# pyg-team/pytorch_geometric

Hardware: NVIDIA H100
Metric: edges/sec (GCNConv fwd+bwd) (higher is better)
Workload: dtype f32

## Files before the change

include/b200mp.h:

```cpp
#ifndef B200MP_H_
#define B200MP_H_

#include <stdint.h>

#ifdef __cplusplus
extern "C" {
#endif

#define B200MP_VERSION "0.1.0"

enum { B200MP_F32 = 0, B200MP_BF16 = 1 };
enum { B200MP_I32 = 0, B200MP_I64 = 1 };
enum { B200MP_SUM = 0, B200MP_MEAN = 1, B200MP_MIN = 2, B200MP_MAX = 3, B200MP_MUL = 4 };
enum {
    B200MP_OK = 0,
    B200MP_ERR_INVALID_ARG = -1,
    B200MP_ERR_UNSUPPORTED = -2,
    B200MP_ERR_CUDA = -3,
    B200MP_ERR_WORKSPACE = -4
};

const char* b200mp_version(void);
const char* b200mp_last_error(void);
int b200mp_device_info(int* sm_count, int* cc_major, int* cc_minor, int64_t* l2_bytes);
int b200mp_set_option(const char* name, int value);


int b200mp_degree(const void* index, int64_t n_index, int64_t n_nodes, void* deg, int idx_dtype,
                  void* stream);
int b200mp_index2ptr(const void* index_sorted, int64_t n_index, int64_t n_nodes, void* ptr,
                     int idx_dtype, void* stream);
int b200mp_ptr2index(const void* ptr, int64_t n_nodes, int64_t n_index, void* index,
                     int idx_dtype, void* stream);
int b200mp_index_stats(const void* index, int64_t n_index, int64_t* stats, int idx_dtype,
                       void* stream);
int64_t b200mp_sort_workspace_bytes(int64_t n_index, int64_t n_nodes, int idx_dtype);
int b200mp_sort_by_key(const void* keys, int64_t n_index, int64_t n_nodes, void* keys_sorted,
                       void* perm, void* ptr, void* workspace, int64_t workspace_bytes,
                       int idx_dtype, void* stream);
int b200mp_permute(const void* in, const void* perm, void* out, int64_t n, int elem_bytes,
                   int idx_dtype, void* stream);
int b200mp_convert_index(const void* in, int in_dtype, void* out, int out_dtype, int64_t n,
                         void* stream);
int64_t b200mp_self_loops_workspace_bytes(int64_t n_edges, int64_t n_nodes, int idx_dtype);
int b200mp_self_loops(const void* row, const void* col, const float* w_in, int64_t n_edges,
                      int64_t n_nodes, float fill_value, int mode, void* row_out, void* col_out,
                      float* w_out, int64_t* n_out_dev, void* workspace, int64_t workspace_bytes,
                      int idx_dtype, void* stream);
int b200mp_gcn_norm_csr(const void* rowptr, const void* src, const float* w, int64_t n_nodes,
                        int64_t n_edges, float* deg_inv_sqrt, float* w_out, int idx_dtype,
                        void* stream);

int b200mp_csr_plan_count(const void* rowptr, int64_t n_rows, int64_t chunk, int64_t* counts_dev,
                          int idx_dtype, void* stream);
int64_t b200mp_csr_plan_workspace_bytes(int64_t n_rows, int64_t n_long_rows, int idx_dtype);
int b200mp_csr_plan_fill(const void* rowptr, int64_t n_rows, int64_t chunk, int64_t n_long_rows,
                         int64_t* long_rows, int64_t* chunk_ptr, void* workspace,
                         int64_t workspace_bytes, int idx_dtype, void* stream);

int b200mp_spmm_csr(const void* rowptr, const void* col, const float* val, const void* x,
                    void* out, int64_t n_rows, int64_t n_cols, int64_t feat, int reduce,
                    const int64_t* long_rows, const int64_t* chunk_ptr, int64_t n_long_rows,
                    int64_t n_chunks, int64_t chunk, float* partials, const float* bias,
                    const void* x_halo, int64_t n_local_cols, int flags, const void* peer_ptrs,
                    int64_t peer_rows, const void* relu_mask, int idx_dtype, int val_dtype, void* stream);

int b200mp_segment_csr(const void* ptr, const void* src, void* out, int64_t n_rows, int64_t n_src,
                       int64_t feat, int reduce, const int64_t* long_rows, const int64_t* chunk_ptr,
                       int64_t n_long_rows, int64_t n_chunks, int64_t chunk, float* partials,
                       int idx_dtype, int val_dtype, void* stream);

int b200mp_minmax_ties(const void* rowptr, const void* col, const float* val, const void* x,
                       const void* out, float* ties, int64_t n_rows, int64_t feat,
                       int count_self_zero, int idx_dtype, int val_dtype, void* stream);
int b200mp_minmax_backward(const void* rowptr_t, const void* col_t, const float* val_t,
                           const void* x, const void* out, const void* grad_out, const float* ties,
                           void* grad_x, int64_t n_src, int64_t feat, int idx_dtype,
                           int val_dtype, void* stream);

int b200mp_sddmm_csr(const void* rowptr, const void* col, const void* a, const void* b, float* dot,
                     int64_t n_rows, int64_t feat, int idx_dtype, int val_dtype, void* stream);

int b200mp_edge_relu_csr(const void* rowptr, const void* col, const void* perm, const void* x,
                         const void* edge_rows, void* out, void* mask, int64_t n_rows, int64_t n_cols,
                         int64_t n_edges, int64_t feat, int reduce, const int64_t* long_rows,
                         const int64_t* chunk_ptr, int64_t n_long_rows, int64_t n_chunks, int64_t chunk,
                         float* partials, int idx_dtype, int val_dtype, void* stream);
int b200mp_edge_relu_backward_x(const void* rowptr_t, const void* col_t, const void* t2csr,
                                const float* val_t, const void* grad_out, const void* mask, void* grad_x,
                                int64_t n_src, int64_t feat, const int64_t* long_rows,
                                const int64_t* chunk_ptr, int64_t n_long_rows, int64_t n_chunks,
                                int64_t chunk, float* partials, int idx_dtype, int val_dtype, void* stream);
int b200mp_edge_relu_backward_edge(const void* rowptr, const void* perm, const void* grad_out,
                                   const void* mask, void* grad_edge_rows, int64_t n_rows, int64_t feat,
                                   int reduce, const int64_t* long_rows, const int64_t* chunk_ptr,
                                   int64_t n_long_rows, int64_t n_chunks, int64_t chunk, int idx_dtype,
                                   int val_dtype, void* stream);

int b200mp_gated_csr(const void* rowptr, const void* col, const void* k, const void* q, const void* v,
                     void* out, int64_t n_rows, int64_t n_cols, int64_t n_edges, int64_t feat, int64_t ld,
                     int reduce, const int64_t* long_rows, const int64_t* chunk_ptr, int64_t n_long_rows,
                     int64_t n_chunks, int64_t chunk, float* partials, int idx_dtype, int val_dtype,
                     void* stream);
int b200mp_gated_backward_dst(const void* rowptr, const void* col, const void* k, const void* q,
                              const void* v, const void* grad_out, void* grad_k, int64_t n_rows,
                              int64_t n_cols, int64_t n_edges, int64_t feat, int64_t ld, int reduce,
                              const int64_t* long_rows, const int64_t* chunk_ptr, int64_t n_long_rows,
                              int64_t n_chunks, int64_t chunk, float* partials, int idx_dtype,
                              int val_dtype, void* stream);
int b200mp_gated_backward_src(const void* rowptr_t, const void* col_t, const float* val_t, const void* k,
                              const void* q, const void* v, const void* grad_out, void* grad_q,
                              void* grad_v, int64_t n_src, int64_t n_dst, int64_t n_edges, int64_t feat,
                              int64_t ld, const int64_t* long_rows, const int64_t* chunk_ptr,
                              int64_t n_long_rows, int64_t n_chunks, int64_t chunk, float* partials,
                              int idx_dtype, int val_dtype, void* stream);

int b200mp_cg_csr(const void* rowptr, const void* col, const void* perm, const void* u, const void* v,
                  const void* c, void* out, int64_t n_rows, int64_t n_cols, int64_t n_edges, int64_t feat,
                  int64_t ld_u, int64_t ld_v, int reduce, const int64_t* long_rows,
                  const int64_t* chunk_ptr, int64_t n_long_rows, int64_t n_chunks, int64_t chunk,
                  float* partials, int idx_dtype, int val_dtype, void* stream);
int b200mp_cg_backward_dst(const void* rowptr, const void* col, const void* perm, const void* u,
                           const void* v, const void* c, const void* grad_out, void* grad_u, void* grad_c,
                           int64_t n_rows, int64_t n_cols, int64_t n_edges, int64_t feat, int64_t ld_u,
                           int64_t ld_v, int reduce, const int64_t* long_rows, const int64_t* chunk_ptr,
                           int64_t n_long_rows, int64_t n_chunks, int64_t chunk, float* partials,
                           int idx_dtype, int val_dtype, void* stream);
int b200mp_cg_backward_src(const void* rowptr_t, const void* col_t, const void* perm_t, const float* val_t,
                           const void* u, const void* v, const void* c, const void* grad_out, void* grad_v,
                           int64_t n_src, int64_t n_dst, int64_t n_edges, int64_t feat, int64_t ld_u,
                           int64_t ld_v, const int64_t* long_rows, const int64_t* chunk_ptr,
                           int64_t n_long_rows, int64_t n_chunks, int64_t chunk, float* partials,
                           int idx_dtype, int val_dtype, void* stream);

int b200mp_softmax_aggr_csr(const void* rowptr, const void* col, const void* perm, const void* x,
                            const void* edge_rows, const float* t, void* out, float* lse, int64_t n_rows,
                            int64_t n_cols, int64_t n_edges, int64_t feat, int message, float eps, int t_mode,
                            const int64_t* long_rows, const int64_t* chunk_ptr, int64_t n_long_rows,
                            int64_t n_chunks, int64_t chunk, float* partials, int idx_dtype, int val_dtype,
                            void* stream);
int64_t b200mp_softmax_aggr_workspace(int64_t n_rows, int64_t n_chunks, int64_t feat);
int b200mp_softmax_aggr_backward_dst(const void* rowptr, const void* col, const void* perm, const void* x,
                                     const void* edge_rows, const float* t, const void* out, const float* lse,
                                     const void* grad_out, void* grad_edge_rows, float* grad_t, float* workspace,
                                     int64_t n_rows, int64_t n_cols, int64_t n_edges, int64_t feat, int message,
                                     float eps, int t_mode, int semi_grad, const int64_t* long_rows,
                                     const int64_t* chunk_ptr, int64_t n_long_rows, int64_t n_chunks, int64_t chunk,
                                     int idx_dtype, int val_dtype, void* stream);
int b200mp_softmax_aggr_backward_src(const void* rowptr_t, const void* col_t, const void* perm_t, const void* x,
                                     const void* edge_rows, const float* t, const void* out, const float* lse,
                                     const void* grad_out, void* grad_x, int64_t n_src, int64_t n_dst,
                                     int64_t n_edges, int64_t feat, int message, float eps, int t_mode,
                                     int semi_grad, const int64_t* long_rows, const int64_t* chunk_ptr,
                                     int64_t n_long_rows, int64_t n_chunks, int64_t chunk, float* partials,
                                     int idx_dtype, int val_dtype, void* stream);

int b200mp_scatter_coo(const float* src, const void* index, float* out, float* count,
                       int64_t n_src, int64_t n_rows, int64_t feat, int reduce, int idx_dtype,
                       void* stream);
int b200mp_index_add_rows(const float* src, const void* index, float* out, int64_t n_src,
                          int64_t feat, int idx_dtype, void* stream);
int b200mp_gather_rows(const void* x, const void* index, const float* scale, void* out,
                       int64_t n_out, int64_t feat, int idx_dtype, int val_dtype, void* stream);

int b200mp_softmax_csr(const void* ptr, const float* src, float* out, int64_t n_rows,
                       int64_t n_src, int64_t heads, int idx_dtype, void* stream);
int b200mp_softmax_csr_backward(const void* ptr, const float* out, const float* grad_out,
                                float* grad_src, int64_t n_rows, int64_t n_src, int64_t heads,
                                int idx_dtype, void* stream);
int b200mp_softmax_edge_op(int op, const float* a, const float* b, const float* row, const void* dst_of_edge,
                           float* out, int64_t n_src, int64_t heads, int idx_dtype, void* stream);


int64_t b200mp_column_sum_parts(int64_t n_rows);
int b200mp_column_sum(const void* x, float* out, float* partials, int64_t n_parts, int64_t n_rows, int64_t feat,
                      int val_dtype, void* stream);

int b200mp_multi_aggr_mask_supported(int64_t feat, int val_dtype, int segment_mode);
int b200mp_multi_aggr_csr(const void* rowptr, const void* col, const void* x, void* out_sum, void* out_mean,
                          void* out_min, void* out_max, void* out_var, void* out_std, float* ties_min,
                          float* ties_max, void* hit_mask, int64_t n_rows, int64_t n_src, int64_t feat, int count_self_zero,
                          const int64_t* long_rows, const int64_t* chunk_ptr, int64_t n_long_rows,
                          int64_t n_chunks, int64_t chunk, float* partials, int idx_dtype, int val_dtype,
                          void* stream);
int b200mp_multi_aggr_prepare_backward(const void* rowptr, const void* g_sum, const void* g_mean,
                                       const void* g_var, const void* g_std, const void* g_min,
                                       const void* g_max, const void* mean, const void* std,
                                       const float* ties_min, const float* ties_max, float* term_a,
                                       float* term_b, float* gmin_out, float* gmax_out, int64_t n_rows,
                                       int64_t feat, int semi_grad, int idx_dtype, int val_dtype, void* stream);
int b200mp_multi_aggr_backward(const void* ptr, const void* idx, const void* x, const float* term_a,
                               const float* term_b, const void* out_min, const float* g_min,
                               const void* out_max, const float* g_max, const void* hit_mask, const void* t2csr,
                               void* grad_x, int64_t n_items, int64_t feat, int segment_mode, int idx_dtype,
                               int val_dtype, void* stream);

int b200mp_pna_epilogue(const void* rowptr, const void* x, const void* u, int64_t u_ld, const void* stat_sum,
                        const void* stat_min, const void* stat_max, const void* stat_var, const int32_t* aggr_host,
                        int n_aggr, const int32_t* scaler_host, int n_scaler, const float* avg_deg_lin,
                        const float* avg_deg_log, void* out, int64_t n_rows, int64_t towers, int64_t feat,
                        int stats_dtype, int idx_dtype, int val_dtype, void* stream);
int b200mp_pna_prologue(const void* rowptr, const void* grad_out, const void* u, int64_t u_ld, const void* stat_sum,
                        const void* stat_min, const void* stat_max, const void* stat_var, const float* ties_min,
                        const float* ties_max, const int32_t* aggr_host, int n_aggr, const int32_t* scaler_host,
                        int n_scaler, const float* avg_deg_lin, const float* avg_deg_log, float* term_a, float* term_b,
                        float* gmin, float* gmax, void* grad_u, int64_t gu_ld, void* grad_x, float* avg_part,
                        int64_t n_rows, int64_t towers, int64_t feat, int stats_dtype, int idx_dtype, int val_dtype,
                        void* stream);
int b200mp_pna_edge_stats(const void* rowptr, const void* col, const void* perm, const void* v, int64_t v_ld,
                          const void* c, float* stat_sum, float* stat_min, float* stat_max, float* stat_var,
                          float* ties_min, float* ties_max, int64_t n_rows, int64_t n_cols, int64_t n_edges,
                          int64_t width, const int64_t* long_rows, const int64_t* chunk_ptr, int64_t n_long_rows,
                          int64_t n_chunks, int64_t chunk, float* partials, int idx_dtype, int val_dtype, void* stream);
int b200mp_pna_edge_backward(const void* rowptr_t, const void* col_t, const void* perm_t, const void* v, int64_t v_ld,
                             const void* c, const float* term_a, const float* term_b, const float* stat_min,
                             const float* gmin, const float* stat_max, const float* gmax, void* grad_v, int64_t gv_ld,
                             void* grad_c, int64_t n_src, int64_t n_dst, int64_t n_edges, int64_t width, int idx_dtype,
                             int val_dtype, void* stream);

int b200mp_head_dot_supported(int64_t heads, int64_t chan, int val_dtype);
int64_t b200mp_head_dot_parts(int64_t n_rows, int64_t heads, int64_t chan, int val_dtype);
int b200mp_head_dot(const void* x, const float* att_a, const float* att_b, float* s_a, float* s_b, int64_t n_rows,
                    int64_t heads, int64_t chan, int val_dtype, void* stream);
int b200mp_head_dot_backward(const void* x, const float* att_a, const float* att_b, const float* g_a, const float* g_b,
                             const void* add, void* grad_x, float* part_a, float* part_b, int64_t n_parts,
                             int64_t n_rows, int64_t heads, int64_t chan, int val_dtype, void* stream);

int b200mp_gat_fused_csr(const void* rowptr, const void* col, const void* dst_of_edge, const void* xh,
                         const float* a_src, const float* a_dst, void* out, float* row_max,
                         float* row_den, float* alpha_out, int64_t n_rows, int64_t n_edges,
                         int64_t heads, int64_t chan, float slope, const int64_t* long_rows,
                         const int64_t* chunk_ptr, int64_t n_long_rows, int64_t n_chunks, int64_t chunk,
                         float* part_acc, float* part_ms, int idx_dtype, int val_dtype, void* stream);
int b200mp_gat_fused_csr_backward(const void* rowptr, const void* col, const void* dst_of_edge,
                                  const void* rowptr_t, const void* col_t, const void* t2csr,
                                  const void* xh, const float* a_src, const float* a_dst,
                                  const float* row_max, const float* row_den, const void* out,
                                  const void* grad_out, float* grad_pre, float* rowdot, void* grad_xh,
                                  float* grad_a_src, float* grad_a_dst, int64_t n_rows, int64_t n_src,
                                  int64_t n_edges, int64_t heads, int64_t chan, float slope,
                                  const int64_t* long_rows, const int64_t* chunk_ptr,
                                  int64_t n_long_rows, int64_t n_chunks, int64_t chunk, float* partials,
                                  int idx_dtype, int val_dtype, void* stream);

int b200mp_scatter_arg(const float* src, const void* index, const float* out, int64_t* arg, int64_t n_src,
                       int64_t n_rows, int64_t feat, int idx_dtype, void* stream);
int b200mp_spmm_csr_arg(const void* rowptr, const void* col, const float* val, const float* x, const float* out,
                        int64_t* arg, int64_t n_rows, int64_t feat, int64_t nnz, int idx_dtype, void* stream);

int b200mp_attn_supported(int64_t heads, int64_t chan, int val_dtype);
int b200mp_attn_csr_forward(int mode, const void* rowptr, const void* col, const void* v, const void* k,
                            const void* q, const float* s_src, const float* s_dst, const float* att,
                            const float* s_edge, int64_t v_stride, int64_t k_stride, int64_t q_stride,
                            void* out, float* row_max, float* row_den, float* alpha_out, int64_t n_rows,
                            int64_t n_edges, int64_t heads, int64_t chan, float slope, float scale,
                            const int64_t* long_rows, const int64_t* chunk_ptr, int64_t n_long_rows,
                            int64_t n_chunks, int64_t chunk, float* part_acc, float* part_ms, float dropout_p,
                            unsigned long long dropout_seed, const void* edge_feat, int idx_dtype, int val_dtype,
                            void* stream);
int64_t b200mp_attn_backward_partial_width(int mode, int64_t heads, int64_t chan, int transposed);
int64_t b200mp_attn_gatt_rows(void);
int b200mp_attn_csr_backward(int mode, const void* rowptr, const void* col, const void* rowptr_t,
                             const void* col_t, const void* t2csr, const void* v, const void* k, const void* q,
                             const float* s_src, const float* s_dst, const float* att, const float* s_edge,
                             int64_t v_stride, int64_t k_stride, int64_t q_stride, const float* row_max,
                             const float* row_den, const void* out, const void* grad_out, float* pair,
                             void* grad_v, void* grad_k, void* grad_q, float* grad_s_src, float* grad_s_dst,
                             float* grad_att, float* gatt_part, int64_t n_rows, int64_t n_src, int64_t n_edges,
                             int64_t heads, int64_t chan, float slope, float scale, const int64_t* long_rows,
                             const int64_t* chunk_ptr, int64_t n_long_rows, int64_t n_chunks, int64_t chunk,
                             float* partials, const int64_t* long_rows_t, const int64_t* chunk_ptr_t,
                             int64_t n_long_rows_t, int64_t n_chunks_t, float* partials_t, float dropout_p,
                             unsigned long long dropout_seed, const void* edge_feat, void* grad_edge_feat, int idx_dtype,
                             int val_dtype, void* stream);

int b200mp_split_tf32(const float* w, float* w_hi, float* w_lo, int64_t n, void* stream);
int b200mp_split_tf32_transposed(const float* w, float* wt_hi, float* wt_lo, int64_t rows, int64_t cols, void* stream);
int b200mp_linear_tf32x3(const float* x, const float* w_hi, const float* w_lo, float* y, int64_t m,
                         int64_t n, int64_t k, void* stream);
int b200mp_linear_grad_input_tf32x3(const float* g, const float* w_hi, const float* w_lo, float* gx,
                                    int64_t m, int64_t n, int64_t k, void* stream);
int64_t b200mp_linear_grad_weight_workspace_bytes(int64_t m, int64_t n, int64_t k);
int b200mp_linear_grad_weight_tf32x3(const float* g, const float* x, float* gw, int64_t m, int64_t n,
                                     int64_t k, void* workspace, int64_t workspace_bytes,
                                     void* stream);

int b200mp_gemm_pair_tf32x3(const float* a1, int64_t k1, const float* a2, int64_t k2, const float* b_hi,
                            const float* b_lo, int b_layout, const float* bias, int relu, float* c1, int64_t n1,
                            float* c2, int64_t n2, int64_t m, void* stream);

int b200mp_segment_matmul_tf32x3(const float* a, const int64_t* ptr, int64_t n_seg, const float* b_hi,
                                 const float* b_lo, int b_layout, float* c, int64_t m, int64_t k, int64_t n,
                                 void* stream);

#ifdef __cplusplus
}
#endif
#endif
```

pytorch_geometric_b200/_lib.py:

```python
from __future__ import annotations

import ctypes
import os
import re

from . import _build

_I64 = ctypes.c_int64
_INT = ctypes.c_int
_P = ctypes.c_void_p
_F = ctypes.c_float
_U64 = ctypes.c_uint64

_SIGS = {
    "b200mp_version": (ctypes.c_char_p, []),
    "b200mp_last_error": (ctypes.c_char_p, []),
    "b200mp_device_info": (_INT, [_P, _P, _P, _P]),
    "b200mp_set_option": (_INT, [ctypes.c_char_p, _INT]),
    "b200mp_degree": (_INT, [_P, _I64, _I64, _P, _INT, _P]),
    "b200mp_index2ptr": (_INT, [_P, _I64, _I64, _P, _INT, _P]),
    "b200mp_ptr2index": (_INT, [_P, _I64, _I64, _P, _INT, _P]),
    "b200mp_index_stats": (_INT, [_P, _I64, _P, _INT, _P]),
    "b200mp_sort_workspace_bytes": (_I64, [_I64, _I64, _INT]),
    "b200mp_sort_by_key": (_INT, [_P, _I64, _I64, _P, _P, _P, _P, _I64, _INT, _P]),
    "b200mp_permute": (_INT, [_P, _P, _P, _I64, _INT, _INT, _P]),
    "b200mp_convert_index": (_INT, [_P, _INT, _P, _INT, _I64, _P]),
    "b200mp_self_loops_workspace_bytes": (_I64, [_I64, _I64, _INT]),
    "b200mp_self_loops": (_INT, [_P, _P, _P, _I64, _I64, _F, _INT, _P, _P, _P, _P, _P, _I64, _INT, _P]),
    "b200mp_gcn_norm_csr": (_INT, [_P, _P, _P, _I64, _I64, _P, _P, _INT, _P]),
    "b200mp_csr_plan_count": (_INT, [_P, _I64, _I64, _P, _INT, _P]),
    "b200mp_csr_plan_workspace_bytes": (_I64, [_I64, _I64, _INT]),
    "b200mp_csr_plan_fill": (_INT, [_P, _I64, _I64, _I64, _P, _P, _P, _I64, _INT, _P]),
    "b200mp_spmm_csr": (_INT, [_P, _P, _P, _P, _P, _I64, _I64, _I64, _INT, _P, _P, _I64, _I64, _I64, _P,
                               _P, _P, _I64, _INT, _P, _I64, _P, _INT, _INT, _P]),
    "b200mp_segment_csr": (_INT, [_P, _P, _P, _I64, _I64, _I64, _INT, _P, _P, _I64, _I64, _I64, _P, _INT, _INT, _P]),
    "b200mp_minmax_ties": (_INT, [_P, _P, _P, _P, _P, _P, _I64, _I64, _INT, _INT, _INT, _P]),
    "b200mp_minmax_backward": (_INT, [_P, _P, _P, _P, _P, _P, _P, _P, _I64, _I64, _INT, _INT, _P]),
    "b200mp_sddmm_csr": (_INT, [_P, _P, _P, _P, _P, _I64, _I64, _INT, _INT, _P]),
    "b200mp_edge_relu_csr": (_INT, [_P] * 7 + [_I64] * 4 + [_INT, _P, _P, _I64, _I64, _I64, _P, _INT, _INT, _P]),
    "b200mp_edge_relu_backward_x": (_INT, [_P] * 7 + [_I64, _I64, _P, _P, _I64, _I64, _I64, _P, _INT, _INT, _P]),
    "b200mp_edge_relu_backward_edge": (_INT, [_P] * 5 + [_I64, _I64, _INT, _P, _P, _I64, _I64, _I64, _INT, _INT, _P]),
    "b200mp_gated_csr": (_INT, [_P] * 6 + [_I64] * 5 + [_INT, _P, _P, _I64, _I64, _I64, _P, _INT, _INT, _P]),
    "b200mp_gated_backward_dst": (_INT, [_P] * 7 + [_I64] * 5 + [_INT, _P, _P, _I64, _I64, _I64, _P, _INT, _INT, _P]),
    "b200mp_gated_backward_src": (_INT, [_P] * 9 + [_I64] * 5 + [_P, _P, _I64, _I64, _I64, _P, _INT, _INT, _P]),
    "b200mp_cg_csr": (_INT, [_P] * 7 + [_I64] * 6 + [_INT, _P, _P, _I64, _I64, _I64, _P, _INT, _INT, _P]),
    "b200mp_cg_backward_dst": (_INT, [_P] * 9 + [_I64] * 6 + [_INT, _P, _P, _I64, _I64, _I64, _P, _INT, _INT, _P]),
    "b200mp_cg_backward_src": (_INT, [_P] * 9 + [_I64] * 6 + [_P, _P, _I64, _I64, _I64, _P, _INT, _INT, _P]),
    "b200mp_softmax_aggr_csr": (_INT, [_P] * 8 + [_I64] * 4 + [_INT, _F, _INT, _P, _P, _I64, _I64, _I64, _P, _INT, _INT,
                                                                _P]),
    "b200mp_softmax_aggr_workspace": (_I64, [_I64, _I64, _I64]),
    "b200mp_softmax_aggr_backward_dst": (_INT, [_P] * 12 + [_I64] * 4 + [_INT, _F, _INT, _INT, _P, _P, _I64, _I64, _I64,
                                                                           _INT, _INT, _P]),
    "b200mp_softmax_aggr_backward_src": (_INT, [_P] * 10 + [_I64] * 4 + [_INT, _F, _INT, _INT, _P, _P, _I64, _I64, _I64,
                                                                           _P, _INT, _INT, _P]),
    "b200mp_scatter_coo": (_INT, [_P, _P, _P, _P, _I64, _I64, _I64, _INT, _INT, _P]),
    "b200mp_split_tf32": (_INT, [_P, _P, _P, _I64, _P]),
    "b200mp_split_tf32_transposed": (_INT, [_P, _P, _P, _I64, _I64, _P]),
    "b200mp_linear_tf32x3": (_INT, [_P, _P, _P, _P, _I64, _I64, _I64, _P]),
    "b200mp_linear_grad_input_tf32x3": (_INT, [_P, _P, _P, _P, _I64, _I64, _I64, _P]),
    "b200mp_linear_grad_weight_workspace_bytes": (_I64, [_I64, _I64, _I64]),
    "b200mp_linear_grad_weight_tf32x3": (_INT, [_P, _P, _P, _I64, _I64, _I64, _P, _I64, _P]),
    "b200mp_gemm_pair_tf32x3": (_INT, [_P, _I64, _P, _I64, _P, _P, _INT, _P, _INT, _P, _I64, _P, _I64, _I64, _P]),
    "b200mp_segment_matmul_tf32x3": (_INT, [_P, _P, _I64, _P, _P, _INT, _P, _I64, _I64, _I64, _P]),
    "b200mp_index_add_rows": (_INT, [_P, _P, _P, _I64, _I64, _INT, _P]),
    "b200mp_gather_rows": (_INT, [_P, _P, _P, _P, _I64, _I64, _INT, _INT, _P]),
    "b200mp_softmax_csr": (_INT, [_P, _P, _P, _I64, _I64, _I64, _INT, _P]),
    "b200mp_softmax_csr_backward": (_INT, [_P, _P, _P, _P, _I64, _I64, _I64, _INT, _P]),
    "b200mp_gat_fused_csr": (_INT, [_P] * 10 + [_I64, _I64, _I64, _I64, _F, _P, _P, _I64, _I64, _I64, _P, _P, _INT, _INT, _P]),
    "b200mp_gat_fused_csr_backward": (_INT, [_P] * 18 + [_I64, _I64, _I64, _I64, _I64, _F, _P, _P, _I64, _I64, _I64, _P,
                                              _INT, _INT, _P]),
    "b200mp_scatter_arg": (_INT, [_P, _P, _P, _P, _I64, _I64, _I64, _INT, _P]),
    "b200mp_spmm_csr_arg": (_INT, [_P, _P, _P, _P, _P, _P, _I64, _I64, _I64, _INT, _P]),
    "b200mp_attn_supported": (_INT, [_I64, _I64, _INT]),
    "b200mp_attn_csr_forward": (_INT, [_INT] + [_P] * 9 + [_I64] * 3 + [_P] * 4 + [_I64] * 4 + [_F, _F, _P, _P, _I64, _I64, _I64,
                                       _P, _P, _F, _U64, _P, _INT, _INT, _P]),
    "b200mp_attn_backward_partial_width": (_I64, [_INT, _I64, _I64, _INT]),
    "b200mp_attn_gatt_rows": (_I64, []),
    "b200mp_attn_csr_backward": (_INT, [_INT] + [_P] * 12 + [_I64] * 3 + [_P] * 12 + [_I64] * 5 + [_F, _F, _P, _P, _I64, _I64,
                                        _I64, _P, _P, _P, _I64, _I64, _P, _F, _U64, _P, _P, _INT, _INT, _P]),
    "b200mp_column_sum_parts": (_I64, [_I64]),
    "b200mp_column_sum": (_INT, [_P, _P, _P, _I64, _I64, _I64, _INT, _P]),
    "b200mp_softmax_edge_op": (_INT, [_INT, _P, _P, _P, _P, _P, _I64, _I64, _INT, _P]),
    "b200mp_multi_aggr_csr": (_INT, [_P] * 12 + [_I64, _I64, _I64, _INT, _P, _P, _I64, _I64, _I64, _P, _INT, _INT, _P]),
    "b200mp_multi_aggr_mask_supported": (_INT, [_I64, _INT, _INT]),
    "b200mp_head_dot_supported": (_INT, [_I64, _I64, _INT]),
    "b200mp_head_dot_parts": (_I64, [_I64, _I64, _I64, _INT]),
    "b200mp_head_dot": (_INT, [_P] * 5 + [_I64, _I64, _I64, _INT, _P]),
    "b200mp_head_dot_backward": (_INT, [_P] * 9 + [_I64, _I64, _I64, _I64, _INT, _P]),
    "b200mp_multi_aggr_prepare_backward": (_INT, [_P] * 15 + [_I64, _I64, _INT, _INT, _INT, _P]),
    "b200mp_multi_aggr_backward": (_INT, [_P] * 12 + [_I64, _I64, _INT, _INT, _INT, _P]),
    "b200mp_pna_epilogue": (_INT, [_P, _P, _P, _I64] + [_P] * 4 + [_P, _INT, _P, _INT, _P, _P, _P, _I64, _I64, _I64,
                                                                   _INT, _INT, _INT, _P]),
    "b200mp_pna_prologue": (_INT, [_P, _P, _P, _I64] + [_P] * 6 + [_P, _INT, _P, _INT] + [_P] * 7 + [_I64, _P, _P,
                                                                                               _I64, _I64, _I64,
                                                                                               _INT, _INT, _INT, _P]),
    "b200mp_pna_edge_stats": (_INT, [_P, _P, _P, _P, _I64] + [_P] * 7 + [_I64] * 4 + [_P, _P, _I64, _I64, _I64, _P, _INT,
                                                                                    _INT, _P]),
    "b200mp_pna_edge_backward": (_INT, [_P, _P, _P, _P, _I64] + [_P] * 8 + [_I64, _P] + [_I64] * 4 + [_INT, _INT, _P]),
}

_lib = None


def header_symbols() -> list[str]:
    with open(os.path.join(_build.INCLUDE, "b200mp.h")) as f:
        text = f.read()
    text = re.sub(r"/\*.*?\*/", "", text, flags=re.S)
    return sorted(set(re.findall(r"\b(b200mp_[a-z0-9_]+)\s*\(", text)))


def lib() -> ctypes.CDLL:
    global _lib
    if _lib is None:
        path = _build.LIB
        if _build.needs_build():
            try:
                path = _build.build()
            except Exception as exc:
                state = "is missing" if not os.path.exists(_build.LIB) else "is stale (sources changed since it was built)"
                raise RuntimeError(
                    f"pytorch_geometric_b200: libb200mp.so {state} and could not be rebuilt ({exc}); "
                    "there is no CPU / eager fallback.") from exc
        l = ctypes.CDLL(path)
        for name, (res, args) in _SIGS.items():
            fn = getattr(l, name)
            fn.restype = res
            fn.argtypes = args
        _lib = l
    return _lib


class B200MPError(RuntimeError):
    pass


def check(rc: int, what: str = "") -> None:
    if rc != 0:
        msg = lib().b200mp_last_error().decode()
        raise B200MPError(f"{what or 'b200mp'} failed (code {rc}): {msg}")
```

pytorch_geometric_b200/csrc/common.cuh:

```cuda
#pragma once

#include <cuda_bf16.h>
#include <cuda_runtime.h>
#include <stdint.h>

#include <cstdio>
#include <type_traits>

#include "../../include/b200mp.h"

namespace b200mp {

void set_error(const char* fmt, ...);

#define B200MP_CHECK_ARG(cond)                                                          \
    do {                                                                                \
        if (!(cond)) {                                                                  \
            ::b200mp::set_error("%s:%d: invalid argument: %s", __FILE__, __LINE__, #cond); \
            return B200MP_ERR_INVALID_ARG;                                              \
        }                                                                               \
    } while (0)

#define B200MP_CUDA(call)                                                                       \
    do {                                                                                        \
        cudaError_t e__ = (call);                                                               \
        if (e__ != cudaSuccess) {                                                               \
            ::b200mp::set_error("%s:%d: %s: %s", __FILE__, __LINE__, #call, cudaGetErrorString(e__)); \
            (void)cudaGetLastError();  \
            return B200MP_ERR_CUDA;                                                             \
        }                                                                                       \
    } while (0)

#define B200MP_LAUNCH_CHECK() B200MP_CUDA(cudaGetLastError())

constexpr int kSMs = 132;

inline int num_sms() {
    static int n = 0;
    if (n == 0) {
        int dev = 0;
        if (cudaGetDevice(&dev) != cudaSuccess ||
            cudaDeviceGetAttribute(&n, cudaDevAttrMultiProcessorCount, dev) != cudaSuccess || n <= 0)
            n = kSMs;
    }
    return n;
}

inline int64_t ceil_div(int64_t a, int64_t b) { return (a + b - 1) / b; }

template <typename F>
int dispatch_val_idx(int val_dtype, int idx_dtype, const char* what, F&& fn) {
    if (val_dtype == B200MP_F32 && idx_dtype == B200MP_I32) return fn(float{}, int32_t{});
    if (val_dtype == B200MP_F32 && idx_dtype == B200MP_I64) return fn(float{}, int64_t{});
    if (val_dtype == B200MP_BF16 && idx_dtype == B200MP_I32) return fn(__nv_bfloat16{}, int32_t{});
    if (val_dtype == B200MP_BF16 && idx_dtype == B200MP_I64) return fn(__nv_bfloat16{}, int64_t{});
    set_error("%s: unsupported dtype combination val=%d idx=%d", what, val_dtype, idx_dtype);
    return B200MP_ERR_UNSUPPORTED;
}

template <int MAX_VPL, typename F>
void lane_group_shape(int n_vec, F&& launch) {
    static_assert(MAX_VPL == 1 || MAX_VPL == 2 || MAX_VPL == 4, "VPL is 1, 2 or 4");
    using std::integral_constant;
    if (n_vec <= 1) launch(integral_constant<int, 1>{}, integral_constant<int, 1>{});
    else if (n_vec <= 2) launch(integral_constant<int, 2>{}, integral_constant<int, 1>{});
    else if (n_vec <= 4) launch(integral_constant<int, 4>{}, integral_constant<int, 1>{});
    else if (n_vec <= 8) launch(integral_constant<int, 8>{}, integral_constant<int, 1>{});
    else if (n_vec <= 16) launch(integral_constant<int, 16>{}, integral_constant<int, 1>{});
    else if constexpr (MAX_VPL == 1) launch(integral_constant<int, 32>{}, integral_constant<int, 1>{});
    else if (n_vec <= 32) launch(integral_constant<int, 32>{}, integral_constant<int, 1>{});
    else if constexpr (MAX_VPL == 2) launch(integral_constant<int, 32>{}, integral_constant<int, 2>{});
    else if (n_vec <= 64) launch(integral_constant<int, 32>{}, integral_constant<int, 2>{});
    else launch(integral_constant<int, 32>{}, integral_constant<int, 4>{});
}

template <int VPL>
constexpr int unroll_for_vpl() { return VPL >= 4 ? 1 : 4 / VPL; }

struct __align__(16) Vec16 {
    uint32_t w[4];
};

__device__ __forceinline__ Vec16 ldg_row16(const void* p) {
    Vec16 v;
    asm volatile("ld.global.nc.L1::no_allocate.v4.u32 {%0,%1,%2,%3}, [%4];"
                 : "=r"(v.w[0]), "=r"(v.w[1]), "=r"(v.w[2]), "=r"(v.w[3])
                 : "l"(p));
    return v;
}
__device__ __forceinline__ Vec16 ldg_stream16(const void* p) {
    Vec16 v;
    asm volatile("ld.global.cs.v4.u32 {%0,%1,%2,%3}, [%4];"
                 : "=r"(v.w[0]), "=r"(v.w[1]), "=r"(v.w[2]), "=r"(v.w[3])
                 : "l"(p));
    return v;
}
__device__ __forceinline__ void cp_async16(void* smem, const void* gmem) {
    asm volatile("cp.async.cg.shared.global [%0], [%1], 16;" ::"r"(static_cast<uint32_t>(__cvta_generic_to_shared(smem))), "l"(gmem) : "memory");
}
__device__ __forceinline__ void cp_async8(void* smem, const void* gmem) {
    asm volatile("cp.async.ca.shared.global [%0], [%1], 8;" ::"r"(static_cast<uint32_t>(__cvta_generic_to_shared(smem))), "l"(gmem) : "memory");
}
__device__ __forceinline__ void cp_async4(void* smem, const void* gmem) {
    asm volatile("cp.async.ca.shared.global [%0], [%1], 4;" ::"r"(static_cast<uint32_t>(__cvta_generic_to_shared(smem))), "l"(gmem) : "memory");
}
__device__ __forceinline__ void cp_async_commit() { asm volatile("cp.async.commit_group;" ::: "memory"); }
template <int N>
__device__ __forceinline__ void cp_async_wait() { asm volatile("cp.async.wait_group %0;" ::"n"(N) : "memory"); }
__device__ __forceinline__ void stg_stream16(void* p, const Vec16& v) {
    asm volatile("st.global.cs.v4.u32 [%0], {%1,%2,%3,%4};" ::"l"(p), "r"(v.w[0]), "r"(v.w[1]),
                 "r"(v.w[2]), "r"(v.w[3])
                 : "memory");
}

template <typename T>
struct ElemTraits;
template <>
struct ElemTraits<float> {
    static constexpr int kPerVec = 4;
    __device__ static __forceinline__ void unpack(const Vec16& v, float (&f)[4]) {
#pragma unroll
        for (int i = 0; i < 4; ++i) f[i] = __uint_as_float(v.w[i]);
    }
    __device__ static __forceinline__ Vec16 pack(const float (&f)[4]) {
        Vec16 v;
#pragma unroll
        for (int i = 0; i < 4; ++i) v.w[i] = __float_as_uint(f[i]);
        return v;
    }
    __device__ static __forceinline__ float to_float(float x) { return x; }
    __device__ static __forceinline__ float from_float(float x) { return x; }
};
template <>
struct ElemTraits<__nv_bfloat16> {
    static constexpr int kPerVec = 8;
    __device__ static __forceinline__ void unpack(const Vec16& v, float (&f)[8]) {
#pragma unroll
        for (int i = 0; i < 4; ++i) {
            f[2 * i] = __uint_as_float(v.w[i] << 16);
            f[2 * i + 1] = __uint_as_float(v.w[i] & 0xffff0000u);
        }
    }
    __device__ static __forceinline__ Vec16 pack(const float (&f)[8]) {
        Vec16 v;
#pragma unroll
        for (int i = 0; i < 4; ++i) {
            __nv_bfloat162 p = __floats2bfloat162_rn(f[2 * i], f[2 * i + 1]);
            v.w[i] = *reinterpret_cast<uint32_t*>(&p);
        }
        return v;
    }
    __device__ static __forceinline__ float to_float(__nv_bfloat16 x) { return __bfloat162float(x); }
    __device__ static __forceinline__ __nv_bfloat16 from_float(float x) { return __float2bfloat16_rn(x); }
};

template <typename T>
__device__ __forceinline__ float round_to(float v) {
    return ElemTraits<T>::to_float(ElemTraits<T>::from_float(v));
}

template <int EPV>
__device__ __forceinline__ void store_partial(float* p, const float (&acc)[EPV]) {
#pragma unroll
    for (int q = 0; q < EPV / 4; ++q)
        *reinterpret_cast<float4*>(p + 4 * q) = make_float4(acc[4 * q], acc[4 * q + 1], acc[4 * q + 2], acc[4 * q + 3]);
}

template <int RED>
__device__ __forceinline__ float red_identity() {
    if (RED == B200MP_MIN) return __int_as_float(0x7f800000);
    if (RED == B200MP_MAX) return __int_as_float(0xff800000);
    if (RED == B200MP_MUL) return 1.0f;
    return 0.0f;
}
template <int RED>
__device__ __forceinline__ float red_combine(float acc, float v) {
    if (RED == B200MP_MIN) return (v < acc || v != v) ? v : acc;
    if (RED == B200MP_MAX) return (v > acc || v != v) ? v : acc;
    if (RED == B200MP_MUL) return __fmul_rn(acc, v);
    return __fadd_rn(acc, v);
}

template <typename I>
__device__ __forceinline__ I ldg_idx(const I* p) {
    return __ldg(p);
}

inline bool aligned16(const void* p) { return (reinterpret_cast<uintptr_t>(p) & 15u) == 0; }

}
```

pytorch_geometric_b200/csrc/csr_dispatch.cuh:

```cuda
#pragma once

#include "csr_reduce.cuh"
#include "csr_tma.cuh"

namespace b200mp {

int get_option_spmm_impl();

template <typename T, typename I, int RED, bool GATHER>
int csr_reduce_variant(const I* rowptr, const I* col, const float* val, const T* x, T* out, int64_t n_rows,
                       int64_t feat, bool is_mean, bool inf_to_zero, LongRowPlan plan, const float* bias,
                       cudaStream_t stream) {
    if (n_rows == 0 || feat == 0) return B200MP_OK;
    const size_t row_bytes = static_cast<size_t>(feat) * sizeof(T);
    const bool tma_ok = row_bytes % 16 == 0 && row_bytes >= 512 && row_bytes <= 2048 && aligned16(x) &&
                        aligned16(plan.x2) && aligned16(out) && (plan.n_chunks == 0 || aligned16(plan.partials));
    const int impl = get_option_spmm_impl();
    if (tma_ok && impl == 2 && !plan.accumulate && !plan.peers)
        return csr_tma_launch<T, I, RED, GATHER>(rowptr, col, val, x, out, n_rows, feat, is_mean, inf_to_zero, plan,
                                                 bias, stream);
    return csr_reduce_dispatch<T, I, RED, GATHER>(rowptr, col, val, x, out, n_rows, feat, is_mean, inf_to_zero, plan,
                                                  bias, stream);
}

template <typename T, typename I, bool GATHER>
int csr_reduce_auto(const I* rowptr, const I* col, const float* val, const T* x, T* out, int64_t n_rows,
                    int64_t feat, int reduce, bool inf_to_zero, LongRowPlan plan, const float* bias,
                    cudaStream_t stream) {
    switch (reduce) {
        case B200MP_SUM:
            return csr_reduce_variant<T, I, B200MP_SUM, GATHER>(rowptr, col, val, x, out, n_rows, feat, false, false, plan, bias, stream);
        case B200MP_MEAN:
            return csr_reduce_variant<T, I, B200MP_SUM, GATHER>(rowptr, col, val, x, out, n_rows, feat, true, false, plan, bias, stream);
        case B200MP_MIN:
            return csr_reduce_variant<T, I, B200MP_MIN, GATHER>(rowptr, col, val, x, out, n_rows, feat, false, inf_to_zero, plan, bias, stream);
        case B200MP_MAX:
            return csr_reduce_variant<T, I, B200MP_MAX, GATHER>(rowptr, col, val, x, out, n_rows, feat, false, inf_to_zero, plan, bias, stream);
        default:
            set_error("csr_reduce: unsupported reduce %d", reduce);
            return B200MP_ERR_UNSUPPORTED;
    }
}

}
```

pytorch_geometric_b200/csrc/csr_reduce.cuh:

```cuda
#pragma once

#include "common.cuh"

namespace b200mp {

int get_option_spmm_tune();

struct LongRowPlan {
    const int64_t* long_rows;
    const int64_t* chunk_ptr;
    int64_t n_long;
    int64_t n_chunks;
    int64_t chunk;
    float* partials;
    const void* x2;
    int64_t split;
    int accumulate;
    const unsigned long long* peers;
    int64_t peer_rows;
    const void* relu_mask;
};

inline int make_plan(LongRowPlan& plan, const int64_t* long_rows, const int64_t* chunk_ptr, int64_t n_long_rows,
                     int64_t n_chunks, int64_t chunk, float* partials, bool needs_partials) {
    B200MP_CHECK_ARG(n_long_rows >= 0 && n_chunks >= 0);
    B200MP_CHECK_ARG(n_long_rows == 0 || (long_rows && chunk_ptr && chunk > 0 && (partials || !needs_partials)));
    plan = LongRowPlan{long_rows, chunk_ptr, n_long_rows, n_long_rows ? n_chunks : 0, chunk, partials,
                       nullptr, 0, 0, nullptr, 0, nullptr};
    return B200MP_OK;
}

__device__ __forceinline__ const char* row_base(const LongRowPlan& plan, const char* xb, const char* xb2, int64_t split,
                                                size_t row_bytes, int64_t c) {
    if (plan.peers) {
        const int64_t r = c / plan.peer_rows;
        return reinterpret_cast<const char*>(__ldg(plan.peers + r)) + static_cast<size_t>(c - r * plan.peer_rows) * row_bytes;
    }
    return (c < split ? xb : xb2) + static_cast<size_t>(c) * row_bytes;
}

template <typename I>
__device__ __forceinline__ bool decode_item(int64_t item, const I* __restrict__ rowptr, int64_t n_rows,
                                            const LongRowPlan& plan, int64_t& row, int64_t& begin,
                                            int64_t& end, bool& is_chunk) {
    if (item < plan.n_chunks) {
        int64_t lo = 0, hi = plan.n_long;
        while (hi - lo > 1) {
            const int64_t mid = (lo + hi) >> 1;
            if (__ldg(plan.chunk_ptr + mid) <= item) lo = mid; else hi = mid;
        }
        row = __ldg(plan.long_rows + lo);
        const int64_t k = item - __ldg(plan.chunk_ptr + lo);
        begin = static_cast<int64_t>(__ldg(rowptr + row)) + k * plan.chunk;
        const int64_t row_end = static_cast<int64_t>(__ldg(rowptr + row + 1));
        end = begin + plan.chunk < row_end ? begin + plan.chunk : row_end;
        is_chunk = true;
        return true;
    }
    row = item - plan.n_chunks;
    if (row >= n_rows) return false;
    begin = static_cast<int64_t>(__ldg(rowptr + row));
    end = static_cast<int64_t>(__ldg(rowptr + row + 1));
    is_chunk = false;
    if (plan.n_long > 0 && end - begin > plan.chunk) return false;
    return true;
}

template <int RED>
__device__ __forceinline__ float finalize(float acc, int64_t deg, bool is_mean, bool inf_to_zero) {
    if (RED == B200MP_SUM) {
        if (is_mean) acc = __fdiv_rn(acc, static_cast<float>(deg < 1 ? 1 : deg));
    } else if (RED == B200MP_MIN || RED == B200MP_MAX) {
        if (deg == 0) acc = 0.0f;
        if (inf_to_zero && isinf(acc)) acc = 0.0f;
    }
    return acc;
}

template <typename T, typename I, int G, int VPL, int RED, bool GATHER, int UNR_OVR = 0, int BLOCK = 256,
          int MINB = 1>
__global__ void __launch_bounds__(BLOCK, MINB)
csr_reduce_kernel(const I* __restrict__ rowptr, const I* __restrict__ col,
                  const float* __restrict__ val, const T* __restrict__ x, T* __restrict__ out,
                  int64_t n_rows, int n_vec, bool is_mean, bool inf_to_zero, LongRowPlan plan,
                  const float* __restrict__ bias) {
    constexpr int EPV = ElemTraits<T>::kPerVec;
    constexpr int UNR = UNR_OVR ? UNR_OVR : (VPL == 1 ? 8 : (VPL == 2 ? 4 : 2));
    const int lig = threadIdx.x & (G - 1);
    const int64_t item = (static_cast<int64_t>(blockIdx.x) * blockDim.x + threadIdx.x) / G;
    int64_t row, begin, end;
    bool is_chunk;
    const bool active = decode_item(item, rowptr, n_rows, plan, row, begin, end, is_chunk);
    if (G < 32 && !active) return;
    if (G == 32 && !active) return;
    const size_t row_bytes = static_cast<size_t>(n_vec) * 16;
    const char* xb = reinterpret_cast<const char*>(x);
    const char* xb2 = plan.x2 ? reinterpret_cast<const char*>(plan.x2) - static_cast<size_t>(plan.split) * row_bytes : xb;
    const int64_t split = plan.x2 ? plan.split : INT64_MAX;

    for (int vbase = 0; vbase < n_vec; vbase += G * VPL) {
        float acc[VPL][EPV];
#pragma unroll
        for (int k = 0; k < VPL; ++k)
#pragma unroll
            for (int i = 0; i < EPV; ++i) acc[k][i] = red_identity<RED>();
        bool vvalid[VPL];
#pragma unroll
        for (int k = 0; k < VPL; ++k) vvalid[k] = (vbase + lig + k * G) < n_vec;
        const size_t voff = static_cast<size_t>(vbase + lig) * 16;

        if (G == 32) {
            for (int64_t e0 = begin; e0 < end; e0 += 32) {
                const int n = static_cast<int>(end - e0 < 32 ? end - e0 : 32);
                int64_t c_l = 0;
                float w_l = 1.0f;
                if (lig < n) {
                    c_l = GATHER ? static_cast<int64_t>(ldg_idx(col + e0 + lig)) : (e0 + lig);
                    if (val) w_l = __ldg(val + e0 + lig);
                    c_l = static_cast<int64_t>(reinterpret_cast<uintptr_t>(row_base(plan, xb, xb2, split, row_bytes, c_l)));
                }
                for (int j = 0; j < n; j += UNR) {
                    Vec16 buf[UNR][VPL];
                    float w[UNR];
#pragma unroll
                    for (int u = 0; u < UNR; ++u) {
                        const int64_t c = __shfl_sync(0xffffffffu, c_l, (j + u) & 31);
                        w[u] = __shfl_sync(0xffffffffu, w_l, (j + u) & 31);
                        if (j + u < n) {
                            const char* p = reinterpret_cast<const char*>(static_cast<uintptr_t>(c)) + voff;
#pragma unroll
                            for (int k = 0; k < VPL; ++k)
                                if (vvalid[k]) buf[u][k] = ldg_row16(p + static_cast<size_t>(k) * G * 16);
                        }
                    }
#pragma unroll
                    for (int u = 0; u < UNR; ++u) {
                        if (j + u < n) {
#pragma unroll
                            for (int k = 0; k < VPL; ++k) {
                                if (vvalid[k]) {
                                    float f[EPV];
                                    ElemTraits<T>::unpack(buf[u][k], f);
#pragma unroll
                                    for (int i = 0; i < EPV; ++i) {
                                        const float m = val ? __fmul_rn(w[u], f[i]) : f[i];
                                        acc[k][i] = red_combine<RED>(acc[k][i], m);
                                    }
                                }
                            }
                        }
                    }
                }
            }
        } else {
            for (int64_t e = begin; e < end; e += UNR) {
                Vec16 buf[UNR][VPL];
                float w[UNR];
#pragma unroll
                for (int u = 0; u < UNR; ++u) {
                    w[u] = 1.0f;
                    if (e + u < end) {
                        const int64_t c = GATHER ? static_cast<int64_t>(ldg_idx(col + e + u)) : (e + u);
                        if (val) w[u] = __ldg(val + e + u);
                        if (vvalid[0]) buf[u][0] = ldg_row16(row_base(plan, xb, xb2, split, row_bytes, c) + voff);
                    }
                }
#pragma unroll
                for (int u = 0; u < UNR; ++u) {
                    if (e + u < end && vvalid[0]) {
                        float f[EPV];
                        ElemTraits<T>::unpack(buf[u][0], f);
#pragma unroll
                        for (int i = 0; i < EPV; ++i) {
                            const float m = val ? __fmul_rn(w[u], f[i]) : f[i];
                            acc[0][i] = red_combine<RED>(acc[0][i], m);
                        }
                    }
                }
            }
        }

        if (is_chunk) {
            float* pbase = plan.partials + static_cast<size_t>(item) * n_vec * EPV;
#pragma unroll
            for (int k = 0; k < VPL; ++k)
                if (vvalid[k]) store_partial<EPV>(pbase + static_cast<size_t>(vbase + lig + k * G) * EPV, acc[k]);
        } else {
            const int64_t deg = end - begin;
            char* ob = reinterpret_cast<char*>(out) + static_cast<size_t>(row) * row_bytes;
#pragma unroll
            for (int k = 0; k < VPL; ++k) {
                if (!vvalid[k]) continue;
                float f[EPV];
#pragma unroll
                for (int i = 0; i < EPV; ++i) f[i] = finalize<RED>(acc[k][i], deg, is_mean, inf_to_zero);
                if (bias) {
                    const float* bp = bias + static_cast<size_t>(vbase + lig + k * G) * EPV;
#pragma unroll
                    for (int i = 0; i < EPV; ++i) f[i] = __fadd_rn(f[i], __ldg(bp + i));
                }
                if (plan.accumulate) {
                    if (deg == 0 && !plan.relu_mask) continue;
                    float o[EPV];
                    ElemTraits<T>::unpack(*reinterpret_cast<const Vec16*>(ob + static_cast<size_t>(vbase + lig + k * G) * 16), o);
#pragma unroll
                    for (int i = 0; i < EPV; ++i) f[i] = deg == 0 ? o[i] : __fadd_rn(o[i], f[i]);
                    if (plan.relu_mask) {
                        float mk[EPV];
                        ElemTraits<T>::unpack(ldg_stream16(static_cast<const char*>(plan.relu_mask) + static_cast<size_t>(row) * row_bytes +
                                                           static_cast<size_t>(vbase + lig + k * G) * 16), mk);
#pragma unroll
                        for (int i = 0; i < EPV; ++i) f[i] = mk[i] > 0.0f ? f[i] : 0.0f;
                    }
                }
                stg_stream16(ob + static_cast<size_t>(vbase + lig + k * G) * 16, ElemTraits<T>::pack(f));
            }
        }
    }
}

template <typename T, typename I, int RED>
__global__ void __launch_bounds__(256)
csr_combine_kernel(const I* __restrict__ rowptr, T* __restrict__ out, int64_t feat, bool is_mean,
                   bool inf_to_zero, LongRowPlan plan, const float* __restrict__ bias) {
    const int64_t j = blockIdx.x;
    if (j >= plan.n_long) return;
    const int64_t row = plan.long_rows[j];
    const int64_t c0 = plan.chunk_ptr[j], c1 = plan.chunk_ptr[j + 1];
    const int64_t deg = static_cast<int64_t>(rowptr[row + 1]) - static_cast<int64_t>(rowptr[row]);
    for (int64_t f = threadIdx.x; f < feat; f += blockDim.x) {
        float acc = red_identity<RED>();
        for (int64_t c = c0; c < c1; ++c) acc = red_combine<RED>(acc, plan.partials[c * feat + f]);
        acc = finalize<RED>(acc, deg, is_mean, inf_to_zero);
        if (bias) acc = __fadd_rn(acc, bias[f]);
        if (plan.accumulate) acc = __fadd_rn(ElemTraits<T>::to_float(out[row * feat + f]), acc);
        if (plan.relu_mask && !(ElemTraits<T>::to_float(static_cast<const T*>(plan.relu_mask)[row * feat + f]) > 0.0f)) acc = 0.0f;
        out[row * feat + f] = ElemTraits<T>::from_float(acc);
    }
}

template <typename T, typename I, int RED, bool GATHER>
__global__ void __launch_bounds__(256)
csr_reduce_scalar_kernel(const I* __restrict__ rowptr, const I* __restrict__ col,
                         const float* __restrict__ val, const T* __restrict__ x, T* __restrict__ out,
                         int64_t n_rows, int64_t feat, int g, bool is_mean, bool inf_to_zero,
                         LongRowPlan plan, const float* __restrict__ bias) {
    const int lig = threadIdx.x & (g - 1);
    const int64_t item = (static_cast<int64_t>(blockIdx.x) * blockDim.x + threadIdx.x) / g;
    int64_t row, begin, end;
    bool is_chunk;
    if (!decode_item(item, rowptr, n_rows, plan, row, begin, end, is_chunk)) return;
    for (int64_t f = lig; f < feat; f += g) {
        float acc = red_identity<RED>();
        for (int64_t e = begin; e < end; e += 4) {
            float v[4], w[4];
#pragma unroll
            for (int u = 0; u < 4; ++u) {
                w[u] = 1.0f;
                v[u] = 0.0f;
                if (e + u < end) {
                    const int64_t c = GATHER ? static_cast<int64_t>(ldg_idx(col + e + u)) : (e + u);
                    if (val) w[u] = __ldg(val + e + u);
                    v[u] = ElemTraits<T>::to_float((plan.x2 && c >= plan.split)
                                                       ? static_cast<const T*>(plan.x2)[(c - plan.split) * feat + f]
                                                       : x[c * feat + f]);
                }
            }
#pragma unroll
            for (int u = 0; u < 4; ++u)
                if (e + u < end) acc = red_combine<RED>(acc, val ? __fmul_rn(w[u], v[u]) : v[u]);
        }
        if (is_chunk)
            plan.partials[item * feat + f] = acc;
        else {
            acc = finalize<RED>(acc, end - begin, is_mean, inf_to_zero);
            if (bias) acc = __fadd_rn(acc, bias[f]);
            if (plan.accumulate) {
                if (end == begin && !plan.relu_mask) continue;
                const float o = ElemTraits<T>::to_float(out[row * feat + f]);
                acc = end == begin ? o : __fadd_rn(o, acc);
                if (plan.relu_mask && !(ElemTraits<T>::to_float(static_cast<const T*>(plan.relu_mask)[row * feat + f]) > 0.0f)) acc = 0.0f;
            }
            out[row * feat + f] = ElemTraits<T>::from_float(acc);
        }
    }
}

template <typename T, typename I, int RED, bool GATHER, int G, int VPL>
inline void launch_vec(const I* rowptr, const I* col, const float* val, const T* x, T* out,
                       int64_t n_rows, int n_vec, bool is_mean, bool inf_to_zero,
                       const LongRowPlan& plan, const float* bias, cudaStream_t stream) {
    const int64_t items = plan.n_chunks + n_rows;
    if (items == 0) return;
#define B200MP_LAUNCH_TUNED(UNR_, BLOCK_, MINB_)                                                           \
    csr_reduce_kernel<T, I, G, VPL, RED, GATHER, UNR_, BLOCK_, MINB_>                                      \
        <<<static_cast<unsigned>(ceil_div(items, BLOCK_ / G)), BLOCK_, 0, stream>>>(                       \
            rowptr, col, val, x, out, n_rows, n_vec, is_mean, inf_to_zero, plan, bias)
    if (G == 32 && VPL == 2 && RED == B200MP_SUM && GATHER) {
        switch (get_option_spmm_tune()) {
            case 1: B200MP_LAUNCH_TUNED(4, 256, 1); return;
            case 2: B200MP_LAUNCH_TUNED(4, 256, 4); return;
            case 3: B200MP_LAUNCH_TUNED(1, 256, 8); return;
            default: break;
        }
    }
    if (sizeof(T) == 4) B200MP_LAUNCH_TUNED(unroll_for_vpl<VPL>(), 128, 12);
    else B200MP_LAUNCH_TUNED(unroll_for_vpl<VPL>(), 128, 8);
#undef B200MP_LAUNCH_TUNED
}

template <typename T, typename I, int RED, bool GATHER>
int csr_reduce_dispatch(const I* rowptr, const I* col, const float* val, const T* x, T* out,
                        int64_t n_rows, int64_t feat, bool is_mean, bool inf_to_zero,
                        LongRowPlan plan, const float* bias, cudaStream_t stream) {
    if (n_rows == 0 || feat == 0) return B200MP_OK;
    const size_t row_bytes = static_cast<size_t>(feat) * sizeof(T);
    const bool vec_ok = (row_bytes % 16 == 0) && aligned16(x) && aligned16(out) && aligned16(plan.x2) &&
                        aligned16(plan.relu_mask) && (plan.n_chunks == 0 || aligned16(plan.partials));
    if (vec_ok) {
        const int n_vec = static_cast<int>(row_bytes / 16);
        lane_group_shape<4>(n_vec, [&](auto G, auto VPL) {
            launch_vec<T, I, RED, GATHER, G(), VPL()>(rowptr, col, val, x, out, n_rows, n_vec, is_mean, inf_to_zero,
                                                      plan, bias, stream);
        });
    } else {
        int g = 1;
        while (g < 32 && g < feat) g <<= 1;
        const int64_t items = plan.n_chunks + n_rows;
        const int64_t blocks = ceil_div(items, 256 / g);
        csr_reduce_scalar_kernel<T, I, RED, GATHER><<<static_cast<unsigned>(blocks), 256, 0, stream>>>(
            rowptr, col, val, x, out, n_rows, feat, g, is_mean, inf_to_zero, plan, bias);
    }
    B200MP_LAUNCH_CHECK();
    if (plan.n_long > 0) {
        csr_combine_kernel<T, I, RED><<<static_cast<unsigned>(plan.n_long), 256, 0, stream>>>(
            rowptr, out, feat, is_mean, inf_to_zero, plan, bias);
        B200MP_LAUNCH_CHECK();
    }
    return B200MP_OK;
}

template <typename T, typename I, bool GATHER>
int csr_reduce_by_op(const I* rowptr, const I* col, const float* val, const T* x, T* out,
                     int64_t n_rows, int64_t feat, int reduce, bool inf_to_zero, LongRowPlan plan,
                     const float* bias, cudaStream_t stream) {
    switch (reduce) {
        case B200MP_SUM:
            return csr_reduce_dispatch<T, I, B200MP_SUM, GATHER>(rowptr, col, val, x, out, n_rows, feat, false, false, plan, bias, stream);
        case B200MP_MEAN:
            return csr_reduce_dispatch<T, I, B200MP_SUM, GATHER>(rowptr, col, val, x, out, n_rows, feat, true, false, plan, bias, stream);
        case B200MP_MIN:
            return csr_reduce_dispatch<T, I, B200MP_MIN, GATHER>(rowptr, col, val, x, out, n_rows, feat, false, inf_to_zero, plan, bias, stream);
        case B200MP_MAX:
            return csr_reduce_dispatch<T, I, B200MP_MAX, GATHER>(rowptr, col, val, x, out, n_rows, feat, false, inf_to_zero, plan, bias, stream);
        default:
            set_error("csr_reduce: unsupported reduce %d", reduce);
            return B200MP_ERR_UNSUPPORTED;
    }
}

}
```

pytorch_geometric_b200/csrc/spmm.cu:

```cuda
#include "csr_dispatch.cuh"

namespace b200mp {

template <typename T, typename I>
__global__ void __launch_bounds__(256)
minmax_ties_kernel(const I* __restrict__ rowptr, const I* __restrict__ col,
                   const float* __restrict__ val, const T* __restrict__ x, const T* __restrict__ out,
                   float* __restrict__ ties, int64_t n_rows, int64_t feat, int g, bool count_self_zero) {
    const int lig = threadIdx.x & (g - 1);
    const int64_t row = (static_cast<int64_t>(blockIdx.x) * blockDim.x + threadIdx.x) / g;
    if (row >= n_rows) return;
    const int64_t begin = rowptr[row], end = rowptr[row + 1];
    for (int64_t f = lig; f < feat; f += g) {
        const float o = ElemTraits<T>::to_float(out[row * feat + f]);
        float cnt = (count_self_zero && o == 0.0f) ? 1.0f : 0.0f;
        for (int64_t e = begin; e < end; e += 4) {
            float v[4];
#pragma unroll
            for (int u = 0; u < 4; ++u) {
                v[u] = 0.f;
                if (e + u < end) {
                    const int64_t c = col[e + u];
                    const float xv = ElemTraits<T>::to_float(x[c * feat + f]);
                    v[u] = ElemTraits<T>::to_float(ElemTraits<T>::from_float(val ? __fmul_rn(__ldg(val + e + u), xv) : xv));
                }
            }
#pragma unroll
            for (int u = 0; u < 4; ++u)
                if (e + u < end && v[u] == o) cnt += 1.0f;
        }
        ties[row * feat + f] = cnt;
    }
}

template <typename T, typename I>
__global__ void __launch_bounds__(256)
minmax_backward_kernel(const I* __restrict__ rowptr_t, const I* __restrict__ col_t,
                       const float* __restrict__ val_t, const T* __restrict__ x,
                       const T* __restrict__ out, const T* __restrict__ grad_out,
                       const float* __restrict__ ties, T* __restrict__ grad_x, int64_t n_src,
                       int64_t feat, int g) {
    const int lig = threadIdx.x & (g - 1);
    const int64_t j = (static_cast<int64_t>(blockIdx.x) * blockDim.x + threadIdx.x) / g;
    if (j >= n_src) return;
    const int64_t begin = rowptr_t[j], end = rowptr_t[j + 1];
    for (int64_t f = lig; f < feat; f += g) {
        const float xv = ElemTraits<T>::to_float(x[j * feat + f]);
        float acc = 0.0f;
        for (int64_t e = begin; e < end; ++e) {
            const int64_t d = col_t[e];
            const float w = val_t ? __ldg(val_t + e) : 1.0f;
            const float m = ElemTraits<T>::to_float(ElemTraits<T>::from_float(val_t ? __fmul_rn(w, xv) : xv));
            const float o = ElemTraits<T>::to_float(out[d * feat + f]);
            if (m == o) {
                const float gd = __fdiv_rn(ElemTraits<T>::to_float(grad_out[d * feat + f]), ties[d * feat + f]);
                acc = __fadd_rn(acc, val_t ? __fmul_rn(w, gd) : gd);
            }
        }
        grad_x[j * feat + f] = ElemTraits<T>::from_float(acc);
    }
}

template <typename T, typename I>
__global__ void __launch_bounds__(256)
sddmm_kernel(const I* __restrict__ rowptr, const I* __restrict__ col, const T* __restrict__ a,
             const T* __restrict__ b, float* __restrict__ dot, int64_t n_rows, int64_t feat) {
    const int lane = threadIdx.x & 31;
    const int64_t row = (static_cast<int64_t>(blockIdx.x) * blockDim.x + threadIdx.x) >> 5;
    if (row >= n_rows) return;
    const int64_t begin = rowptr[row], end = rowptr[row + 1];
    const T* ar = a + row * feat;
    for (int64_t e = begin; e < end; e += 2) {
        const bool has1 = e + 1 < end;
        const T* b0 = b + static_cast<int64_t>(col[e]) * feat;
        const T* b1 = has1 ? b + static_cast<int64_t>(col[e + 1]) * feat : b0;
        float s0 = 0.f, s1 = 0.f;
        for (int64_t f = lane; f < feat; f += 32) {
            const float av = ElemTraits<T>::to_float(ar[f]);
            s0 = fmaf(av, ElemTraits<T>::to_float(b0[f]), s0);
            s1 = fmaf(av, ElemTraits<T>::to_float(b1[f]), s1);
        }
#pragma unroll
        for (int o = 16; o > 0; o >>= 1) {
            s0 += __shfl_xor_sync(0xffffffffu, s0, o);
            s1 += __shfl_xor_sync(0xffffffffu, s1, o);
        }
        if (lane == 0) {
            dot[e] = s0;
            if (has1) dot[e + 1] = s1;
        }
    }
}

inline int group_width(int64_t feat) {
    int g = 1;
    while (g < 32 && g < feat) g <<= 1;
    return g;
}

}

using namespace b200mp;

extern "C" int b200mp_spmm_csr(const void* rowptr, const void* col, const float* val, const void* x,
                               void* out, int64_t n_rows, int64_t n_cols, int64_t feat, int reduce,
                               const int64_t* long_rows, const int64_t* chunk_ptr,
                               int64_t n_long_rows, int64_t n_chunks, int64_t chunk, float* partials,
                               const float* bias, const void* x_halo, int64_t n_local_cols, int flags,
                               const void* peer_ptrs, int64_t peer_rows, const void* relu_mask, int idx_dtype,
                               int val_dtype, void* stream) {
    B200MP_CHECK_ARG(n_rows >= 0 && n_cols >= 0 && feat >= 0);
    B200MP_CHECK_ARG((flags & ~1) == 0 && (!(flags & 1) || (reduce == B200MP_SUM && !bias)));
    B200MP_CHECK_ARG(!relu_mask || (flags & 1));
    LongRowPlan plan;
    if (int rc = make_plan(plan, long_rows, chunk_ptr, n_long_rows, n_chunks, chunk, partials, true)) return rc;
    if (n_rows == 0 || feat == 0) return B200MP_OK;
    B200MP_CHECK_ARG(rowptr && out);
    B200MP_CHECK_ARG(x || n_cols == 0 || peer_ptrs);
    B200MP_CHECK_ARG(!peer_ptrs || (peer_rows > 0 && !x_halo && (feat * (val_dtype == B200MP_BF16 ? 2 : 4)) % 16 == 0));
    B200MP_CHECK_ARG(!peer_ptrs || (aligned16(x) && aligned16(out) && aligned16(relu_mask) &&
                                    (n_long_rows == 0 || aligned16(partials))));
    B200MP_CHECK_ARG(!x_halo || (n_local_cols >= 0 && n_local_cols <= n_cols));
    plan.x2 = x_halo;
    plan.split = x_halo ? n_local_cols : 0;
    plan.accumulate = flags & 1;
    plan.peers = static_cast<const unsigned long long*>(peer_ptrs);
    plan.peer_rows = peer_ptrs ? peer_rows : 0;
    plan.relu_mask = relu_mask;
    return dispatch_val_idx(val_dtype, idx_dtype, "spmm_csr", [&](auto tv, auto ti) {
        using T = decltype(tv);
        using I = decltype(ti);
        return csr_reduce_auto<T, I, true>(static_cast<const I*>(rowptr), static_cast<const I*>(col), val,
                                            static_cast<const T*>(x), static_cast<T*>(out), n_rows, feat, reduce,
                                            false, plan, bias, static_cast<cudaStream_t>(stream));
    });
}

extern "C" int b200mp_minmax_ties(const void* rowptr, const void* col, const float* val, const void* x,
                                  const void* out, float* ties, int64_t n_rows, int64_t feat,
                                  int count_self_zero, int idx_dtype, int val_dtype, void* stream) {
    B200MP_CHECK_ARG(n_rows >= 0 && feat >= 0);
    if (n_rows == 0 || feat == 0) return B200MP_OK;
    B200MP_CHECK_ARG(rowptr && out && ties);
    return dispatch_val_idx(val_dtype, idx_dtype, "minmax_ties", [&](auto tv, auto ti) {
        using T = decltype(tv);
        using I = decltype(ti);
        const int g = group_width(feat);
        minmax_ties_kernel<T, I><<<static_cast<unsigned>(ceil_div(n_rows, 256 / g)), 256, 0,
                                   static_cast<cudaStream_t>(stream)>>>(
            static_cast<const I*>(rowptr), static_cast<const I*>(col), val, static_cast<const T*>(x),
            static_cast<const T*>(out), ties, n_rows, feat, g, count_self_zero != 0);
        B200MP_LAUNCH_CHECK();
        return B200MP_OK;
    });
}

extern "C" int b200mp_minmax_backward(const void* rowptr_t, const void* col_t, const float* val_t,
                                      const void* x, const void* out, const void* grad_out,
                                      const float* ties, void* grad_x, int64_t n_src, int64_t feat,
                                      int idx_dtype, int val_dtype, void* stream) {
    B200MP_CHECK_ARG(n_src >= 0 && feat >= 0);
    if (n_src == 0 || feat == 0) return B200MP_OK;
    B200MP_CHECK_ARG(rowptr_t && x && grad_x);
    return dispatch_val_idx(val_dtype, idx_dtype, "minmax_backward", [&](auto tv, auto ti) {
        using T = decltype(tv);
        using I = decltype(ti);
        const int g = group_width(feat);
        minmax_backward_kernel<T, I><<<static_cast<unsigned>(ceil_div(n_src, 256 / g)), 256, 0,
                                       static_cast<cudaStream_t>(stream)>>>(
            static_cast<const I*>(rowptr_t), static_cast<const I*>(col_t), val_t, static_cast<const T*>(x),
            static_cast<const T*>(out), static_cast<const T*>(grad_out), ties, static_cast<T*>(grad_x), n_src,
            feat, g);
        B200MP_LAUNCH_CHECK();
        return B200MP_OK;
    });
}

extern "C" int b200mp_sddmm_csr(const void* rowptr, const void* col, const void* a, const void* b,
                                float* dot, int64_t n_rows, int64_t feat, int idx_dtype, int val_dtype,
                                void* stream) {
    B200MP_CHECK_ARG(n_rows >= 0 && feat >= 0);
    if (n_rows == 0) return B200MP_OK;
    B200MP_CHECK_ARG(rowptr && dot);
    return dispatch_val_idx(val_dtype, idx_dtype, "sddmm_csr", [&](auto tv, auto ti) {
        using T = decltype(tv);
        using I = decltype(ti);
        sddmm_kernel<T, I><<<static_cast<unsigned>(ceil_div(n_rows, 8)), 256, 0, static_cast<cudaStream_t>(stream)>>>(
            static_cast<const I*>(rowptr), static_cast<const I*>(col), static_cast<const T*>(a),
            static_cast<const T*>(b), dot, n_rows, feat);
        B200MP_LAUNCH_CHECK();
        return B200MP_OK;
    });
}
```

pytorch_geometric_b200/csrc/structure.cu:

```cuda
#include <cub/cub.cuh>
#include <thrust/iterator/counting_iterator.h>

#include "common.cuh"

namespace b200mp {

constexpr int kThreads = 256;
inline unsigned grid_for(int64_t n, int per_block = kThreads) {
    int64_t b = ceil_div(n, per_block);
    return static_cast<unsigned>(b < 1 ? 1 : b);
}

template <typename I>
__global__ void degree_kernel(const I* __restrict__ index, int64_t n, I* __restrict__ deg) {
    const int64_t e = static_cast<int64_t>(blockIdx.x) * blockDim.x + threadIdx.x;
    if (e >= n) return;
    if (sizeof(I) == 8)
        atomicAdd(reinterpret_cast<unsigned long long*>(deg + index[e]), 1ull);
    else
        atomicAdd(reinterpret_cast<unsigned int*>(deg + index[e]), 1u);
}

template <typename I>
__global__ void index2ptr_kernel(const I* __restrict__ index, int64_t n, int64_t n_nodes, I* __restrict__ ptr) {
    const int64_t e = static_cast<int64_t>(blockIdx.x) * blockDim.x + threadIdx.x;
    if (e > n) return;
    const int64_t prev = e == 0 ? -1 : static_cast<int64_t>(index[e - 1]);
    const int64_t cur = e == n ? n_nodes : static_cast<int64_t>(index[e]);
    for (int64_t i = prev + 1; i <= cur; ++i) ptr[i] = static_cast<I>(e);
}

template <typename I>
__device__ __forceinline__ int64_t row_of_edge(const I* __restrict__ ptr, int64_t n_nodes, int64_t e) {
    int64_t lo = 0, hi = n_nodes;
    while (hi - lo > 1) {
        const int64_t mid = (lo + hi) >> 1;
        if (static_cast<int64_t>(__ldg(ptr + mid)) <= e) lo = mid; else hi = mid;
    }
    return lo;
}

template <typename I>
__global__ void ptr2index_kernel(const I* __restrict__ ptr, int64_t n_nodes, int64_t n, I* __restrict__ index) {
    const int64_t e = static_cast<int64_t>(blockIdx.x) * blockDim.x + threadIdx.x;
    if (e >= n) return;
    index[e] = static_cast<I>(row_of_edge(ptr, n_nodes, e));
}

template <typename I>
__global__ void index_stats_kernel(const I* __restrict__ index, int64_t n, long long* __restrict__ stats) {
    long long mn = LLONG_MAX, mx = LLONG_MIN;
    int unsorted = 0;
    for (int64_t e = static_cast<int64_t>(blockIdx.x) * blockDim.x + threadIdx.x; e < n;
         e += static_cast<int64_t>(gridDim.x) * blockDim.x) {
        const long long v = index[e];
        mn = v < mn ? v : mn;
        mx = v > mx ? v : mx;
        if (e > 0 && static_cast<long long>(index[e - 1]) > v) unsorted = 1;
    }
    typedef cub::BlockReduce<long long, kThreads> BR;
    __shared__ typename BR::TempStorage tmp;
    mn = BR(tmp).Reduce(mn, cub::Min());
    __syncthreads();
    mx = BR(tmp).Reduce(mx, cub::Max());
    __syncthreads();
    const long long us = BR(tmp).Reduce(static_cast<long long>(unsorted), cub::Max());
    if (threadIdx.x == 0) {
        atomicMin(stats + 0, mn);
        atomicMax(stats + 1, mx);
        if (us) atomicMin(stats + 2, 0ll);
    }
}
__global__ void index_stats_init(long long* stats, int64_t n) {
    stats[0] = n ? LLONG_MAX : 0;
    stats[1] = n ? LLONG_MIN : -1;
    stats[2] = 1;
}

template <typename I>
__global__ void iota_kernel(I* __restrict__ out, int64_t n) {
    const int64_t i = static_cast<int64_t>(blockIdx.x) * blockDim.x + threadIdx.x;
    if (i < n) out[i] = static_cast<I>(i);
}

template <typename E, typename I>
__global__ void permute_kernel(const E* __restrict__ in, const I* __restrict__ perm, E* __restrict__ out, int64_t n) {
    const int64_t i = static_cast<int64_t>(blockIdx.x) * blockDim.x + threadIdx.x;
    if (i < n) out[i] = in[perm[i]];
}

template <typename A, typename B>
__global__ void convert_kernel(const A* __restrict__ in, B* __restrict__ out, int64_t n) {
    const int64_t i = static_cast<int64_t>(blockIdx.x) * blockDim.x + threadIdx.x;
    if (i < n) out[i] = static_cast<B>(in[i]);
}

inline int bits_for(int64_t n_nodes) {
    int b = 1;
    while (b < 63 && (int64_t(1) << b) < n_nodes) ++b;
    return b;
}
inline size_t align_up(size_t x, size_t a = 256) { return (x + a - 1) / a * a; }

template <typename I>
size_t sort_temp_bytes(int64_t n, int64_t n_nodes) {
    size_t t = 0;
    cub::DeviceRadixSort::SortPairs(nullptr, t, static_cast<const I*>(nullptr), static_cast<I*>(nullptr),
                                    static_cast<const I*>(nullptr), static_cast<I*>(nullptr), n, 0,
                                    bits_for(n_nodes));
    return t;
}

template <typename I>
int sort_typed(const void* keys, int64_t n, int64_t n_nodes, void* keys_sorted, void* perm, void* ptr,
               void* workspace, int64_t ws_bytes, cudaStream_t stream) {
    const size_t arr = align_up(sizeof(I) * static_cast<size_t>(n));
    size_t temp = sort_temp_bytes<I>(n, n_nodes);
    const size_t need = arr * 2 + align_up(temp);
    if (static_cast<size_t>(ws_bytes) < need) {
        set_error("sort_by_key: workspace %lld < %zu", static_cast<long long>(ws_bytes), need);
        return B200MP_ERR_WORKSPACE;
    }
    char* ws = static_cast<char*>(workspace);
    I* iota = reinterpret_cast<I*>(ws);
    I* kout = keys_sorted ? static_cast<I*>(keys_sorted) : reinterpret_cast<I*>(ws + arr);
    void* tmp = ws + 2 * arr;
    if (n > 0) {
        iota_kernel<I><<<grid_for(n), kThreads, 0, stream>>>(iota, n);
        B200MP_LAUNCH_CHECK();
        B200MP_CUDA(cub::DeviceRadixSort::SortPairs(tmp, temp, static_cast<const I*>(keys), kout, iota,
                                                    static_cast<I*>(perm), n, 0, bits_for(n_nodes), stream));
    }
    if (ptr) {
        index2ptr_kernel<I><<<grid_for(n + 1), kThreads, 0, stream>>>(kout, n, n_nodes, static_cast<I*>(ptr));
        B200MP_LAUNCH_CHECK();
    }
    return B200MP_OK;
}

template <typename I>
struct NotLoop {
    const I* row;
    const I* col;
    __device__ __forceinline__ bool operator()(const int64_t& e) const { return row[e] != col[e]; }
};

template <typename I>
__global__ void self_loops_write_kernel(const I* __restrict__ row, const I* __restrict__ col,
                                        const float* __restrict__ w_in, const int64_t* __restrict__ kept,
                                        const int64_t* __restrict__ n_kept_dev, int64_t n_nodes,
                                        float fill, I* __restrict__ row_out, I* __restrict__ col_out,
                                        float* __restrict__ w_out, int64_t* __restrict__ n_out_dev) {
    const int64_t n_kept = *n_kept_dev;
    const int64_t i = static_cast<int64_t>(blockIdx.x) * blockDim.x + threadIdx.x;
    if (i == 0) *n_out_dev = n_kept + n_nodes;
    if (i < n_kept) {
        const int64_t e = kept[i];
        row_out[i] = row[e];
        col_out[i] = col[e];
        if (w_in) w_out[i] = w_in[e];
    } else if (i < n_kept + n_nodes) {
        const int64_t v = i - n_kept;
        row_out[i] = static_cast<I>(v);
        col_out[i] = static_cast<I>(v);
        if (w_in) w_out[i] = fill;
    }
}
template <typename I>
__global__ void loop_last_edge_kernel(const I* __restrict__ row, const I* __restrict__ col, int64_t n_edges,
                                      long long* __restrict__ last) {
    const int64_t e = static_cast<int64_t>(blockIdx.x) * blockDim.x + threadIdx.x;
    if (e < n_edges && row[e] == col[e]) atomicMax(last + row[e], static_cast<long long>(e));
}
__global__ void fill_ll_kernel(long long* p, int64_t n, long long v) {
    const int64_t i = static_cast<int64_t>(blockIdx.x) * blockDim.x + threadIdx.x;
    if (i < n) p[i] = v;
}
__global__ void loop_weight_kernel(const float* __restrict__ w_in, const long long* __restrict__ last,
                                   const int64_t* __restrict__ n_kept_dev, int64_t n_nodes,
                                   float* __restrict__ w_out) {
    const int64_t v = static_cast<int64_t>(blockIdx.x) * blockDim.x + threadIdx.x;
    if (v < n_nodes && last[v] >= 0) w_out[*n_kept_dev + v] = w_in[last[v]];
}

template <typename I>
size_t select_temp_bytes(int64_t n) {
    size_t t = 0;
    thrust::counting_iterator<int64_t> it(0);
    NotLoop<I> pred{nullptr, nullptr};
    cub::DeviceSelect::If(nullptr, t, it, static_cast<int64_t*>(nullptr), static_cast<int64_t*>(nullptr), n, pred);
    return t;
}

template <typename I>
int self_loops_typed(const void* row_, const void* col_, const float* w_in, int64_t n_edges, int64_t n_nodes,
                     float fill, int mode, void* row_out, void* col_out, float* w_out, int64_t* n_out_dev,
                     void* workspace, int64_t ws_bytes, cudaStream_t stream) {
    const I* row = static_cast<const I*>(row_);
    const I* col = static_cast<const I*>(col_);
    size_t temp = select_temp_bytes<I>(n_edges);
    const size_t kept_b = align_up(sizeof(int64_t) * static_cast<size_t>(n_edges));
    const size_t last_b = align_up(sizeof(long long) * static_cast<size_t>(n_nodes));
    const size_t need = kept_b + last_b + 256 + align_up(temp);
    if (static_cast<size_t>(ws_bytes) < need) {
        set_error("self_loops: workspace %lld < %zu", static_cast<long long>(ws_bytes), need);
        return B200MP_ERR_WORKSPACE;
    }
    char* ws = static_cast<char*>(workspace);
    int64_t* kept = reinterpret_cast<int64_t*>(ws);
    long long* last = reinterpret_cast<long long*>(ws + kept_b);
    int64_t* n_kept = reinterpret_cast<int64_t*>(ws + kept_b + last_b);
    void* tmp = ws + kept_b + last_b + 256;
    thrust::counting_iterator<int64_t> it(0);
    NotLoop<I> pred{row, col};
    B200MP_CUDA(cub::DeviceSelect::If(tmp, temp, it, kept, n_kept, n_edges, pred, stream));
    self_loops_write_kernel<I><<<grid_for(n_edges + n_nodes), kThreads, 0, stream>>>(
        row, col, w_in, kept, n_kept, n_nodes, fill, static_cast<I*>(row_out), static_cast<I*>(col_out), w_out,
        n_out_dev);
    B200MP_LAUNCH_CHECK();
    if (w_in && mode == 0 && n_nodes > 0) {
        fill_ll_kernel<<<grid_for(n_nodes), kThreads, 0, stream>>>(last, n_nodes, -1ll);
        if (n_edges > 0) loop_last_edge_kernel<I><<<grid_for(n_edges), kThreads, 0, stream>>>(row, col, n_edges, last);
        loop_weight_kernel<<<grid_for(n_nodes), kThreads, 0, stream>>>(w_in, last, n_kept, n_nodes, w_out);
        B200MP_LAUNCH_CHECK();
    }
    return B200MP_OK;
}

template <typename I>
__global__ void gcn_deg_kernel(const I* __restrict__ rowptr, const float* __restrict__ w, int64_t n_nodes,
                               float* __restrict__ dinv) {
    const int64_t i = static_cast<int64_t>(blockIdx.x) * blockDim.x + threadIdx.x;
    if (i >= n_nodes) return;
    const int64_t b = rowptr[i], e = rowptr[i + 1];
    float deg;
    if (w) {
        deg = 0.0f;
        for (int64_t k = b; k < e; ++k) deg = __fadd_rn(deg, __ldg(w + k));
    } else {
        deg = static_cast<float>(e - b);
    }
    float d = powf(deg, -0.5f);
    if (isinf(d)) d = 0.0f;
    dinv[i] = d;
}
template <typename I>
__global__ void gcn_weight_kernel(const I* __restrict__ rowptr, const I* __restrict__ src,
                                  const float* __restrict__ w, const float* __restrict__ dinv, int64_t n_nodes,
                                  int64_t n_edges, float* __restrict__ w_out) {
    const int64_t e = static_cast<int64_t>(blockIdx.x) * blockDim.x + threadIdx.x;
    if (e >= n_edges) return;
    const int64_t dst = row_of_edge(rowptr, n_nodes, e);
    const float we = w ? w[e] : 1.0f;
    w_out[e] = __fmul_rn(__fmul_rn(dinv[src[e]], we), dinv[dst]);
}

template <typename I>
__global__ void plan_count_kernel(const I* __restrict__ rowptr, int64_t n_rows, int64_t chunk,
                                  unsigned long long* __restrict__ counts) {
    const int64_t i = static_cast<int64_t>(blockIdx.x) * blockDim.x + threadIdx.x;
    if (i >= n_rows) return;
    const int64_t deg = static_cast<int64_t>(rowptr[i + 1]) - static_cast<int64_t>(rowptr[i]);
    if (deg > chunk) {
        atomicAdd(counts + 0, 1ull);
        atomicAdd(counts + 1, static_cast<unsigned long long>((deg + chunk - 1) / chunk));
    }
}
template <typename I>
struct IsLong {
    const I* rowptr;
    int64_t chunk;
    __device__ __forceinline__ bool operator()(const int64_t& i) const {
        return static_cast<int64_t>(rowptr[i + 1]) - static_cast<int64_t>(rowptr[i]) > chunk;
    }
};
template <typename I>
__global__ void plan_chunks_kernel(const I* __restrict__ rowptr, const int64_t* __restrict__ long_rows,
                                   int64_t n_long, int64_t chunk, int64_t* __restrict__ nchunks) {
    const int64_t j = static_cast<int64_t>(blockIdx.x) * blockDim.x + threadIdx.x;
    if (j > n_long) return;
    if (j == n_long) { nchunks[j] = 0; return; }
    const int64_t r = long_rows[j];
    const int64_t deg = static_cast<int64_t>(rowptr[r + 1]) - static_cast<int64_t>(rowptr[r]);
    nchunks[j] = (deg + chunk - 1) / chunk;
}

}

using namespace b200mp;

#define IDX_DISPATCH(EXPR32, EXPR64)                                        \
    do {                                                                    \
        if (idx_dtype == B200MP_I32) { EXPR32; }                            \
        else if (idx_dtype == B200MP_I64) { EXPR64; }                       \
        else { set_error("bad idx_dtype %d", idx_dtype); return B200MP_ERR_UNSUPPORTED; } \
    } while (0)

extern "C" int b200mp_degree(const void* index, int64_t n_index, int64_t n_nodes, void* deg, int idx_dtype,
                             void* stream) {
    B200MP_CHECK_ARG(n_index >= 0 && n_nodes >= 0);
    B200MP_CHECK_ARG(deg || n_nodes == 0);
    cudaStream_t s = static_cast<cudaStream_t>(stream);
    const size_t isz = idx_dtype == B200MP_I64 ? 8 : 4;
    if (n_nodes) B200MP_CUDA(cudaMemsetAsync(deg, 0, isz * n_nodes, s));
    if (n_index == 0) return B200MP_OK;
    B200MP_CHECK_ARG(index);
    IDX_DISPATCH((degree_kernel<int32_t><<<grid_for(n_index), kThreads, 0, s>>>(static_cast<const int32_t*>(index), n_index, static_cast<int32_t*>(deg))),
                 (degree_kernel<int64_t><<<grid_for(n_index), kThreads, 0, s>>>(static_cast<const int64_t*>(index), n_index, static_cast<int64_t*>(deg))));
    B200MP_LAUNCH_CHECK();
    return B200MP_OK;
}

extern "C" int b200mp_index2ptr(const void* index_sorted, int64_t n_index, int64_t n_nodes, void* ptr,
                                int idx_dtype, void* stream) {
    B200MP_CHECK_ARG(n_index >= 0 && n_nodes >= 0 && ptr);
    cudaStream_t s = static_cast<cudaStream_t>(stream);
    IDX_DISPATCH((index2ptr_kernel<int32_t><<<grid_for(n_index + 1), kThreads, 0, s>>>(static_cast<const int32_t*>(index_sorted), n_index, n_nodes, static_cast<int32_t*>(ptr))),
                 (index2ptr_kernel<int64_t><<<grid_for(n_index + 1), kThreads, 0, s>>>(static_cast<const int64_t*>(index_sorted), n_index, n_nodes, static_cast<int64_t*>(ptr))));
    B200MP_LAUNCH_CHECK();
    return B200MP_OK;
}

extern "C" int b200mp_ptr2index(const void* ptr, int64_t n_nodes, int64_t n_index, void* index, int idx_dtype,
                                void* stream) {
    B200MP_CHECK_ARG(n_index >= 0 && n_nodes >= 0 && ptr);
    if (n_index == 0) return B200MP_OK;
    B200MP_CHECK_ARG(index);
    cudaStream_t s = static_cast<cudaStream_t>(stream);
    IDX_DISPATCH((ptr2index_kernel<int32_t><<<grid_for(n_index), kThreads, 0, s>>>(static_cast<const int32_t*>(ptr), n_nodes, n_index, static_cast<int32_t*>(index))),
                 (ptr2index_kernel<int64_t><<<grid_for(n_index), kThreads, 0, s>>>(static_cast<const int64_t*>(ptr), n_nodes, n_index, static_cast<int64_t*>(index))));
    B200MP_LAUNCH_CHECK();
    return B200MP_OK;
}

extern "C" int b200mp_index_stats(const void* index, int64_t n_index, int64_t* stats, int idx_dtype,
                                  void* stream) {
    B200MP_CHECK_ARG(n_index >= 0 && stats);
    cudaStream_t s = static_cast<cudaStream_t>(stream);
    long long* st = reinterpret_cast<long long*>(stats);
    index_stats_init<<<1, 1, 0, s>>>(st, n_index);
    if (n_index > 0) {
        B200MP_CHECK_ARG(index);
        int64_t blocks = ceil_div(n_index, kThreads);
        if (blocks > num_sms() * 8) blocks = num_sms() * 8;
        IDX_DISPATCH((index_stats_kernel<int32_t><<<static_cast<unsigned>(blocks), kThreads, 0, s>>>(static_cast<const int32_t*>(index), n_index, st)),
                     (index_stats_kernel<int64_t><<<static_cast<unsigned>(blocks), kThreads, 0, s>>>(static_cast<const int64_t*>(index), n_index, st)));
    }
    B200MP_LAUNCH_CHECK();
    return B200MP_OK;
}

extern "C" int64_t b200mp_sort_workspace_bytes(int64_t n_index, int64_t n_nodes, int idx_dtype) {
    if (n_index < 0 || n_nodes < 0) return B200MP_ERR_INVALID_ARG;
    const size_t isz = idx_dtype == B200MP_I64 ? 8 : 4;
    const size_t arr = align_up(isz * static_cast<size_t>(n_index));
    const size_t temp = idx_dtype == B200MP_I64 ? sort_temp_bytes<int64_t>(n_index, n_nodes)
                                                : sort_temp_bytes<int32_t>(n_index, n_nodes);
    return static_cast<int64_t>(arr * 2 + align_up(temp) + 256);
}

extern "C" int b200mp_sort_by_key(const void* keys, int64_t n_index, int64_t n_nodes, void* keys_sorted,
                                  void* perm, void* ptr, void* workspace, int64_t workspace_bytes,
                                  int idx_dtype, void* stream) {
    B200MP_CHECK_ARG(n_index >= 0 && n_nodes >= 0);
    B200MP_CHECK_ARG(n_index == 0 || (keys && perm && workspace));
    cudaStream_t s = static_cast<cudaStream_t>(stream);
    if (idx_dtype == B200MP_I32)
        return sort_typed<int32_t>(keys, n_index, n_nodes, keys_sorted, perm, ptr, workspace, workspace_bytes, s);
    if (idx_dtype == B200MP_I64)
        return sort_typed<int64_t>(keys, n_index, n_nodes, keys_sorted, perm, ptr, workspace, workspace_bytes, s);
    set_error("bad idx_dtype %d", idx_dtype);
    return B200MP_ERR_UNSUPPORTED;
}

extern "C" int b200mp_permute(const void* in, const void* perm, void* out, int64_t n, int elem_bytes,
                              int idx_dtype, void* stream) {
    B200MP_CHECK_ARG(n >= 0);
    if (n == 0) return B200MP_OK;
    B200MP_CHECK_ARG(in && perm && out);
    B200MP_CHECK_ARG(elem_bytes == 4 || elem_bytes == 8);
    cudaStream_t s = static_cast<cudaStream_t>(stream);
    if (elem_bytes == 4) {
        IDX_DISPATCH((permute_kernel<uint32_t, int32_t><<<grid_for(n), kThreads, 0, s>>>(static_cast<const uint32_t*>(in), static_cast<const int32_t*>(perm), static_cast<uint32_t*>(out), n)),
                     (permute_kernel<uint32_t, int64_t><<<grid_for(n), kThreads, 0, s>>>(static_cast<const uint32_t*>(in), static_cast<const int64_t*>(perm), static_cast<uint32_t*>(out), n)));
    } else {
        IDX_DISPATCH((permute_kernel<uint64_t, int32_t><<<grid_for(n), kThreads, 0, s>>>(static_cast<const uint64_t*>(in), static_cast<const int32_t*>(perm), static_cast<uint64_t*>(out), n)),
                     (permute_kernel<uint64_t, int64_t><<<grid_for(n), kThreads, 0, s>>>(static_cast<const uint64_t*>(in), static_cast<const int64_t*>(perm), static_cast<uint64_t*>(out), n)));
    }
    B200MP_LAUNCH_CHECK();
    return B200MP_OK;
}

extern "C" int b200mp_convert_index(const void* in, int in_dtype, void* out, int out_dtype, int64_t n,
                                    void* stream) {
    B200MP_CHECK_ARG(n >= 0);
    if (n == 0) return B200MP_OK;
    B200MP_CHECK_ARG(in && out);
    cudaStream_t s = static_cast<cudaStream_t>(stream);
    if (in_dtype == B200MP_I64 && out_dtype == B200MP_I32)
        convert_kernel<int64_t, int32_t><<<grid_for(n), kThreads, 0, s>>>(static_cast<const int64_t*>(in), static_cast<int32_t*>(out), n);
    else if (in_dtype == B200MP_I32 && out_dtype == B200MP_I64)
        convert_kernel<int32_t, int64_t><<<grid_for(n), kThreads, 0, s>>>(static_cast<const int32_t*>(in), static_cast<int64_t*>(out), n);
    else if (in_dtype == out_dtype && (in_dtype == B200MP_I32 || in_dtype == B200MP_I64))
        B200MP_CUDA(cudaMemcpyAsync(out, in, (in_dtype == B200MP_I64 ? 8 : 4) * static_cast<size_t>(n), cudaMemcpyDeviceToDevice, s));
    else {
        set_error("convert_index: bad dtypes %d -> %d", in_dtype, out_dtype);
        return B200MP_ERR_UNSUPPORTED;
    }
    B200MP_LAUNCH_CHECK();
    return B200MP_OK;
}

extern "C" int64_t b200mp_self_loops_workspace_bytes(int64_t n_edges, int64_t n_nodes, int idx_dtype) {
    if (n_edges < 0 || n_nodes < 0) return B200MP_ERR_INVALID_ARG;
    const size_t temp = idx_dtype == B200MP_I64 ? select_temp_bytes<int64_t>(n_edges) : select_temp_bytes<int32_t>(n_edges);
    return static_cast<int64_t>(align_up(8 * static_cast<size_t>(n_edges)) + align_up(8 * static_cast<size_t>(n_nodes)) + 256 + align_up(temp) + 256);
}

extern "C" int b200mp_self_loops(const void* row, const void* col, const float* w_in, int64_t n_edges,
                                 int64_t n_nodes, float fill_value, int mode, void* row_out, void* col_out,
                                 float* w_out, int64_t* n_out_dev, void* workspace, int64_t workspace_bytes,
                                 int idx_dtype, void* stream) {
    B200MP_CHECK_ARG(n_edges >= 0 && n_nodes >= 0 && n_out_dev && workspace);
    B200MP_CHECK_ARG(n_edges == 0 || (row && col));
    B200MP_CHECK_ARG(n_edges + n_nodes == 0 || (row_out && col_out));
    B200MP_CHECK_ARG(!w_in || w_out);
    B200MP_CHECK_ARG(mode == 0 || mode == 1);
    cudaStream_t s = static_cast<cudaStream_t>(stream);
    if (idx_dtype == B200MP_I32)
        return self_loops_typed<int32_t>(row, col, w_in, n_edges, n_nodes, fill_value, mode, row_out, col_out, w_out, n_out_dev, workspace, workspace_bytes, s);
    if (idx_dtype == B200MP_I64)
        return self_loops_typed<int64_t>(row, col, w_in, n_edges, n_nodes, fill_value, mode, row_out, col_out, w_out, n_out_dev, workspace, workspace_bytes, s);
    set_error("bad idx_dtype %d", idx_dtype);
    return B200MP_ERR_UNSUPPORTED;
}

extern "C" int b200mp_gcn_norm_csr(const void* rowptr, const void* src, const float* w, int64_t n_nodes,
                                   int64_t n_edges, float* deg_inv_sqrt, float* w_out, int idx_dtype,
                                   void* stream) {
    B200MP_CHECK_ARG(n_nodes >= 0 && n_edges >= 0);
    if (n_nodes == 0) return B200MP_OK;
    B200MP_CHECK_ARG(rowptr && deg_inv_sqrt);
    B200MP_CHECK_ARG(n_edges == 0 || (src && w_out));
    cudaStream_t s = static_cast<cudaStream_t>(stream);
    IDX_DISPATCH(({
                     gcn_deg_kernel<int32_t><<<grid_for(n_nodes), kThreads, 0, s>>>(static_cast<const int32_t*>(rowptr), w, n_nodes, deg_inv_sqrt);
                     if (n_edges) gcn_weight_kernel<int32_t><<<grid_for(n_edges), kThreads, 0, s>>>(static_cast<const int32_t*>(rowptr), static_cast<const int32_t*>(src), w, deg_inv_sqrt, n_nodes, n_edges, w_out);
                 }),
                 ({
                     gcn_deg_kernel<int64_t><<<grid_for(n_nodes), kThreads, 0, s>>>(static_cast<const int64_t*>(rowptr), w, n_nodes, deg_inv_sqrt);
                     if (n_edges) gcn_weight_kernel<int64_t><<<grid_for(n_edges), kThreads, 0, s>>>(static_cast<const int64_t*>(rowptr), static_cast<const int64_t*>(src), w, deg_inv_sqrt, n_nodes, n_edges, w_out);
                 }));
    B200MP_LAUNCH_CHECK();
    return B200MP_OK;
}

extern "C" int b200mp_csr_plan_count(const void* rowptr, int64_t n_rows, int64_t chunk, int64_t* counts_dev,
                                     int idx_dtype, void* stream) {
    B200MP_CHECK_ARG(n_rows >= 0 && chunk > 0 && counts_dev);
    cudaStream_t s = static_cast<cudaStream_t>(stream);
    B200MP_CUDA(cudaMemsetAsync(counts_dev, 0, 16, s));
    if (n_rows == 0) return B200MP_OK;
    B200MP_CHECK_ARG(rowptr);
    unsigned long long* c = reinterpret_cast<unsigned long long*>(counts_dev);
    IDX_DISPATCH((plan_count_kernel<int32_t><<<grid_for(n_rows), kThreads, 0, s>>>(static_cast<const int32_t*>(rowptr), n_rows, chunk, c)),
                 (plan_count_kernel<int64_t><<<grid_for(n_rows), kThreads, 0, s>>>(static_cast<const int64_t*>(rowptr), n_rows, chunk, c)));
    B200MP_LAUNCH_CHECK();
    return B200MP_OK;
}

namespace b200mp {
template <typename I>
size_t plan_temp_bytes(int64_t n_rows, int64_t n_long) {
    size_t t1 = 0, t2 = 0;
    thrust::counting_iterator<int64_t> it(0);
    IsLong<I> pred{nullptr, 1};
    cub::DeviceSelect::If(nullptr, t1, it, static_cast<int64_t*>(nullptr), static_cast<int64_t*>(nullptr), n_rows, pred);
    cub::DeviceScan::ExclusiveSum(nullptr, t2, static_cast<int64_t*>(nullptr), static_cast<int64_t*>(nullptr), n_long + 1);
    return t1 > t2 ? t1 : t2;
}
template <typename I>
int plan_fill_typed(const void* rowptr_, int64_t n_rows, int64_t chunk, int64_t n_long, int64_t* long_rows,
                    int64_t* chunk_ptr, void* workspace, int64_t ws_bytes, cudaStream_t s) {
    const I* rowptr = static_cast<const I*>(rowptr_);
    size_t temp = plan_temp_bytes<I>(n_rows, n_long);
    const size_t nch_b = align_up(8 * static_cast<size_t>(n_long + 1));
    if (static_cast<size_t>(ws_bytes) < nch_b + 256 + align_up(temp)) {
        set_error("csr_plan_fill: workspace too small");
        return B200MP_ERR_WORKSPACE;
    }
    char* ws = static_cast<char*>(workspace);
    int64_t* nchunks = reinterpret_cast<int64_t*>(ws);
    int64_t* n_sel = reinterpret_cast<int64_t*>(ws + nch_b);
    void* tmp = ws + nch_b + 256;
    thrust::counting_iterator<int64_t> it(0);
    IsLong<I> pred{rowptr, chunk};
    size_t t = temp;
    B200MP_CUDA(cub::DeviceSelect::If(tmp, t, it, long_rows, n_sel, n_rows, pred, s));
    plan_chunks_kernel<I><<<grid_for(n_long + 1), kThreads, 0, s>>>(rowptr, long_rows, n_long, chunk, nchunks);
    B200MP_LAUNCH_CHECK();
    t = temp;
    B200MP_CUDA(cub::DeviceScan::ExclusiveSum(tmp, t, nchunks, chunk_ptr, n_long + 1, s));
    return B200MP_OK;
}
}

extern "C" int64_t b200mp_csr_plan_workspace_bytes(int64_t n_rows, int64_t n_long_rows, int idx_dtype) {
    if (n_rows < 0 || n_long_rows < 0) return B200MP_ERR_INVALID_ARG;
    const size_t temp = idx_dtype == B200MP_I64 ? plan_temp_bytes<int64_t>(n_rows, n_long_rows)
                                                : plan_temp_bytes<int32_t>(n_rows, n_long_rows);
    return static_cast<int64_t>(align_up(8 * static_cast<size_t>(n_long_rows + 1)) + 256 + align_up(temp) + 256);
}

extern "C" int b200mp_csr_plan_fill(const void* rowptr, int64_t n_rows, int64_t chunk, int64_t n_long_rows,
                                    int64_t* long_rows, int64_t* chunk_ptr, void* workspace,
                                    int64_t workspace_bytes, int idx_dtype, void* stream) {
    B200MP_CHECK_ARG(n_rows >= 0 && chunk > 0 && n_long_rows >= 0);
    if (n_long_rows == 0) return B200MP_OK;
    B200MP_CHECK_ARG(rowptr && long_rows && chunk_ptr && workspace);
    cudaStream_t s = static_cast<cudaStream_t>(stream);
    if (idx_dtype == B200MP_I32)
        return plan_fill_typed<int32_t>(rowptr, n_rows, chunk, n_long_rows, long_rows, chunk_ptr, workspace, workspace_bytes, s);
    if (idx_dtype == B200MP_I64)
        return plan_fill_typed<int64_t>(rowptr, n_rows, chunk, n_long_rows, long_rows, chunk_ptr, workspace, workspace_bytes, s);
    set_error("bad idx_dtype %d", idx_dtype);
    return B200MP_ERR_UNSUPPORTED;
}
```

pytorch_geometric_b200/functional.py:

```python
from __future__ import annotations

from typing import Optional

import torch
from torch import Tensor

from . import ops
from .graph import CSRGraph


class _Aggregate(torch.autograd.Function):
    @staticmethod
    def forward(ctx, x: Tensor, edge_weight: Optional[Tensor], graph: CSRGraph, reduce: str):
        val = graph.val
        if edge_weight is not None:
            val = graph.to_csr_order(edge_weight.detach().float().contiguous().view(-1))
        out = ops.spmm_csr(graph.rowptr, graph.col, val, x, graph.num_dst, reduce, graph.plan)
        ctx.graph, ctx.reduce = graph, reduce
        ctx.has_ew = edge_weight is not None
        need_x = reduce in ("min", "max") or (ctx.has_ew and edge_weight.requires_grad)
        ctx.save_for_backward(x if need_x else None, out if reduce in ("min", "max") else None, val)
        return out

    @staticmethod
    def backward(ctx, grad_out: Tensor):
        graph, reduce = ctx.graph, ctx.reduce
        x, out, val = ctx.saved_tensors
        grad_out = grad_out.contiguous()
        graph.build_transpose()
        gx = gw = None
        val_t = None
        if val is not None:
            val_t = graph.val_t if (not ctx.has_ew and graph.val_t is not None) else \
                graph.to_csc_order(graph.from_csr_order(val))
        if ctx.needs_input_grad[0]:
            if reduce in ("sum", "add"):
                gx = ops.spmm_csr(graph.rowptr_t, graph.col_t, val_t, grad_out, graph.num_src, "sum", graph.plan_t)
            elif reduce == "mean":
                mv = graph.mean_val_t()
                if val_t is not None:
                    mv = mv * val_t
                gx = ops.spmm_csr(graph.rowptr_t, graph.col_t, mv, grad_out, graph.num_src, "sum", graph.plan_t)
            else:
                ties = ops.minmax_ties(graph.rowptr, graph.col, val, x, out, count_self_zero=True)
                gx = ops.minmax_backward(graph.rowptr_t, graph.col_t, val_t, x, out, grad_out, ties)
        if ctx.has_ew and ctx.needs_input_grad[1]:
            if reduce not in ("sum", "add", "mean"):
                raise NotImplementedError("gradient wrt edge_weight is implemented for sum/mean only")
            g = grad_out
            dot = ops.sddmm_csr(graph.rowptr, graph.col, g, x)
            if reduce == "mean":
                inv = 1.0 / graph.in_degree().clamp(min=1).to(torch.float32)
                dot = dot * ops.gather_rows(inv.view(-1, 1), graph.dst_csr).view(-1)
            gw = graph.from_csr_order(dot)
        return gx, gw, None, None


def aggregate(graph: CSRGraph, x: Tensor, reduce: str = "sum", edge_weight: Optional[Tensor] = None) -> Tensor:
    if reduce not in ("sum", "add", "mean", "min", "max"):
        raise ValueError(f"Encountered invalid `reduce` argument '{reduce}'")
    if x.dim() == 1:
        return aggregate(graph, x.view(-1, 1), reduce, edge_weight).view(-1)
    if x.dim() > 2:
        shape = x.shape[1:]
        return aggregate(graph, x.reshape(x.size(0), -1), reduce, edge_weight).view((graph.num_dst, ) + shape)
    if x.size(0) != graph.num_src:
        raise ValueError(f"x has {x.size(0)} rows but the graph has {graph.num_src} source nodes")
    return _Aggregate.apply(x, edge_weight, graph, reduce)


class _AggregateEdgeReLU(torch.autograd.Function):

    @staticmethod
    def forward(ctx, x: Tensor, edge_rows: Tensor, graph: CSRGraph, reduce: str):
        want_mask = ctx.needs_input_grad[0] or ctx.needs_input_grad[1]
        out, mask = ops.edge_relu_csr(graph.rowptr, graph.col, graph.perm, x, edge_rows, graph.num_dst, reduce,
                                      graph.plan, want_mask=want_mask)
        ctx.graph, ctx.reduce = graph, reduce
        ctx.save_for_backward(mask)
        return out

    @staticmethod
    def backward(ctx, grad_out: Tensor):
        mask, = ctx.saved_tensors
        graph, reduce = ctx.graph, ctx.reduce
        gx = ga = None
        if ctx.needs_input_grad[0]:
            graph.build_transpose()
            val_t = graph.mean_val_t() if reduce == "mean" else None
            gx = ops.edge_relu_backward_x(graph.rowptr_t, graph.col_t, graph.t2csr, val_t, grad_out, mask, graph.num_src,
                                          graph.plan_t)
        if ctx.needs_input_grad[1]:
            ga = ops.edge_relu_backward_edge(graph.rowptr, graph.perm, grad_out, mask, graph.num_edges, reduce, graph.plan)
        return gx, ga, None, None


def aggregate_edge_relu(graph: CSRGraph, x: Tensor, edge_rows: Tensor, reduce: str = "sum") -> Tensor:
    if reduce not in ("sum", "add", "mean"):
        raise ValueError(f"aggregate_edge_relu reduces by sum or mean, got '{reduce}'")
    if edge_rows.dtype != x.dtype:
        raise TypeError(f"edge_rows ({edge_rows.dtype}) and x ({x.dtype}) must share a dtype")
    if tuple(edge_rows.shape) != (graph.num_edges, ) + tuple(x.shape[1:]):
        raise ValueError(f"edge_rows must have shape {(graph.num_edges, ) + tuple(x.shape[1:])}, "
                         f"got {tuple(edge_rows.shape)}")
    if x.dim() == 1:
        return aggregate_edge_relu(graph, x.view(-1, 1), edge_rows.view(-1, 1), reduce).view(-1)
    if x.size(0) != graph.num_src:
        raise ValueError(f"x has {x.size(0)} rows but the graph has {graph.num_src} source nodes")
    shape = x.shape[1:]
    x2 = x.reshape(x.size(0), -1)
    out = _AggregateEdgeReLU.apply(x2, edge_rows.reshape(graph.num_edges, x2.size(1)), graph,
                                   "mean" if reduce == "mean" else "sum")
    return out.view((graph.num_dst, ) + tuple(shape))


class _AggregateGated(torch.autograd.Function):

    @staticmethod
    def forward(ctx, k: Tensor, q: Tensor, v: Optional[Tensor], graph: CSRGraph, reduce: str):
        F = k.size(1)
        qq, vv = (q, v) if v is not None else (q[:, :F], q[:, F:])
        out = ops.gated_csr(graph.rowptr, graph.col, k, qq, vv, graph.num_dst, reduce, graph.plan)
        ctx.graph, ctx.reduce, ctx.split = graph, reduce, v is None
        ctx.save_for_backward(k, q, v)
        return out

    @staticmethod
    def backward(ctx, grad_out: Tensor):
        k, q, v = ctx.saved_tensors
        graph, reduce = ctx.graph, ctx.reduce
        F = k.size(1)
        qq, vv = (q[:, :F], q[:, F:]) if ctx.split else (q, v)
        gk = gq = gv = None
        if ctx.needs_input_grad[0]:
            gk = ops.gated_backward_dst(graph.rowptr, graph.col, k, qq, vv, grad_out, reduce, graph.plan)
        if ctx.needs_input_grad[1] or ctx.needs_input_grad[2]:
            graph.build_transpose()
            val_t = graph.mean_val_t() if reduce == "mean" else None
            gq = torch.empty_like(q)
            gv = None if ctx.split else torch.empty_like(v)
            ops.gated_backward_src(graph.rowptr_t, graph.col_t, val_t, k, qq, vv, grad_out,
                                   gq[:, :F] if ctx.split else gq, gq[:, F:] if ctx.split else gv, graph.plan_t)
        return gk, gq, gv, None, None


def _gated_check(graph: CSRGraph, k: Tensor, q: Tensor, reduce: str, name: str) -> None:
    if reduce not in ("sum", "add", "mean"):
        raise ValueError(f"{name} reduces by sum or mean, got '{reduce}'")
    if q.dtype != k.dtype:
        raise TypeError(f"q ({q.dtype}) and k ({k.dtype}) must share a dtype")
    if k.size(0) != graph.num_dst:
        raise ValueError(f"k has {k.size(0)} rows but the graph has {graph.num_dst} destination nodes")
    if q.size(0) != graph.num_src:
        raise ValueError(f"q has {q.size(0)} rows but the graph has {graph.num_src} source nodes")


def aggregate_gated(graph: CSRGraph, k: Tensor, q: Tensor, v: Tensor, reduce: str = "sum") -> Tensor:
    _gated_check(graph, k, q, reduce, "aggregate_gated")
    if v.dtype != k.dtype:
        raise TypeError(f"v ({v.dtype}) and k ({k.dtype}) must share a dtype")
    if q.shape[1:] != k.shape[1:] or v.shape != q.shape:
        raise ValueError(f"q and v must have shape {(graph.num_src, ) + tuple(k.shape[1:])}, "
                         f"got {tuple(q.shape)} and {tuple(v.shape)}")
    if k.dim() == 1:
        return aggregate_gated(graph, k.view(-1, 1), q.view(-1, 1), v.view(-1, 1), reduce).view(-1)
    shape = k.shape[1:]
    k2 = k.reshape(k.size(0), -1).contiguous()
    q2 = q.reshape(q.size(0), -1).contiguous()
    v2 = v.reshape(v.size(0), -1).contiguous()
    out = _AggregateGated.apply(k2, q2, v2, graph, "mean" if reduce == "mean" else "sum")
    return out.view((graph.num_dst, ) + tuple(shape))


def aggregate_gated_qv(graph: CSRGraph, k: Tensor, qv: Tensor, reduce: str = "sum") -> Tensor:
    _gated_check(graph, k, qv, reduce, "aggregate_gated_qv")
    if k.dim() != 2 or qv.dim() != 2 or qv.size(1) != 2 * k.size(1):
        raise ValueError(f"k must be [num_dst, F] and qv [num_src, 2F], got {tuple(k.shape)} and {tuple(qv.shape)}")
    return _AggregateGated.apply(k.contiguous(), qv.contiguous(), None, graph, "mean" if reduce == "mean" else "sum")


class _AggregateCG(torch.autograd.Function):

    @staticmethod
    def forward(ctx, u: Tensor, v: Optional[Tensor], c: Optional[Tensor], graph: CSRGraph, reduce: str):
        W = u.size(1) // (2 if v is None else 1)
        uu, vv = (u, v) if v is not None else (u[:, :W], u[:, W:])
        out = ops.cg_csr(graph.rowptr, graph.col, graph.perm, uu, vv, c, graph.num_dst, reduce, graph.plan)
        ctx.graph, ctx.reduce, ctx.packed = graph, reduce, v is None
        ctx.save_for_backward(u, v, c)
        return out

    @staticmethod
    def backward(ctx, grad_out: Tensor):
        u, v, c = ctx.saved_tensors
        graph, reduce, packed = ctx.graph, ctx.reduce, ctx.packed
        W = u.size(1) // (2 if packed else 1)
        uu, vv = (u[:, :W], u[:, W:]) if packed else (u, v)
        need_u, need_c = ctx.needs_input_grad[0], ctx.needs_input_grad[2]
        need_v = need_u if packed else ctx.needs_input_grad[1]
        grad_out = grad_out.contiguous()
        gu = gv = gc = None
        gu_dst = gv_dst = None
        if packed:
            if need_u or need_c:
                full = torch.empty_like(u)
                gu_dst, gv_dst = full[:, :W], full[:, W:]
                gu = full if need_u else None
        else:
            if need_u or need_c:
                gu_dst = torch.empty_like(u)
                gu = gu_dst if need_u else None
        if need_u or need_c:
            gc = ops.cg_backward_dst(graph.rowptr, graph.col, graph.perm, uu, vv, c, grad_out, gu_dst, need_c, reduce,
                                     graph.plan)
        if need_v:
            graph.build_transpose()
            if gc is not None:
                sums = ops.spmm_csr(graph.rowptr_t, graph.perm_t, None, gc, graph.num_src, "sum", graph.plan_t)
                if packed:
                    gv_dst.copy_(sums)
                else:
                    gv = sums
            else:
                if not packed:
                    gv = gv_dst = torch.empty_like(v)
                val_t = graph.mean_val_t() if reduce == "mean" else None
                ops.cg_backward_src(graph.rowptr_t, graph.col_t, graph.perm_t, val_t, uu, vv, c, grad_out, gv_dst,
                                    graph.plan_t)
        return gu, gv, gc, None, None


def _cg_check(graph: CSRGraph, u: Tensor, c: Optional[Tensor], reduce: str, width: int, name: str) -> None:
    if reduce not in ("sum", "add", "mean"):
        raise ValueError(f"{name} reduces by sum or mean, got '{reduce}'")
    if u.dim() != 2 or u.size(1) % width:
        raise ValueError(f"{name}: u must be a [num_dst, {width}F] tensor, got {tuple(u.shape)}")
    if u.size(0) != graph.num_dst:
        raise ValueError(f"u has {u.size(0)} rows but the graph has {graph.num_dst} destination nodes")
    F = u.size(1) // width
    if c is not None and (tuple(c.shape) != (graph.num_edges, 2 * F) or c.dtype != u.dtype):
        raise ValueError(f"c must be a [{graph.num_edges}, {2 * F}] tensor of u's dtype, got {tuple(c.shape)} {c.dtype}")


def aggregate_cg(graph: CSRGraph, u: Tensor, v: Tensor, c: Optional[Tensor] = None, reduce: str = "sum") -> Tensor:
    _cg_check(graph, u, c, reduce, 2, "aggregate_cg")
    if v.dtype != u.dtype or v.shape != (graph.num_src, u.size(1)):
        raise ValueError(f"v must be a [{graph.num_src}, {u.size(1)}] tensor of u's dtype, got {tuple(v.shape)} {v.dtype}")
    return _AggregateCG.apply(u.contiguous(), v.contiguous(), None if c is None else c.contiguous(), graph,
                              "mean" if reduce == "mean" else "sum")


def aggregate_cg_uv(graph: CSRGraph, uv: Tensor, c: Optional[Tensor] = None, reduce: str = "sum") -> Tensor:
    _cg_check(graph, uv, c, reduce, 4, "aggregate_cg_uv")
    if graph.num_src != graph.num_dst:
        raise ValueError(f"aggregate_cg_uv needs as many sources as destinations, got {graph.num_src} and {graph.num_dst}")
    return _AggregateCG.apply(uv.contiguous(), None, None if c is None else c.contiguous(), graph,
                              "mean" if reduce == "mean" else "sum")


class _SoftmaxAggregate(torch.autograd.Function):

    @staticmethod
    def forward(ctx, x, a, t, where, eps: float, message: str, semi_grad: bool, want_lse: bool):
        rowptr, col, perm, plan, n_edges, _ = where
        out, lse = ops.softmax_aggr_csr(rowptr, col, perm, x, a, t, rowptr.numel() - 1, n_edges, message, eps, plan,
                                        want_lse)
        ctx.where, ctx.eps, ctx.message, ctx.semi = where, eps, message, semi_grad
        ctx.save_for_backward(x, a, t, out, lse)
        return out

    @staticmethod
    def backward(ctx, grad_out: Tensor):
        x, a, t, out, lse = ctx.saved_tensors
        rowptr, col, perm, plan, n_edges, graph = ctx.where
        need_x, need_a, need_t = ctx.needs_input_grad[:3]
        need_t = need_t and not ctx.semi
        gx = ga = gt = None
        if need_a or need_t:
            ga, gt = ops.softmax_aggr_backward_dst(rowptr, col, perm, x, a, t, out, lse, grad_out, n_edges, ctx.message,
                                                   ctx.eps, ctx.semi, need_a, need_t, plan)
            if gt is not None:
                gt = gt.sum().view(1) if t.numel() == 1 else gt
        if need_x:
            graph.build_transpose()
            if ga is not None:
                gx = ops.spmm_csr(graph.rowptr_t, graph.perm_t, None, ga, graph.num_src, "sum", graph.plan_t)
            else:
                gx = ops.softmax_aggr_backward_src(graph.rowptr_t, graph.col_t, graph.perm_t, x, a, t, out, lse,
                                                   grad_out, ctx.message, ctx.eps, ctx.semi, graph.plan_t)
        return gx, ga, gt, None, None, None, None, None


def softmax_aggregate(graph, x: Optional[Tensor], a: Optional[Tensor] = None, t=1.0, eps: float = 0.0,
                      message: str = "identity", semi_grad: bool = False) -> Tensor:
    if isinstance(graph, CSRGraph):
        where = (graph.rowptr, graph.col, graph.perm, graph.plan, graph.num_edges, graph)
        if x is not None and x.size(0) != graph.num_src:
            raise ValueError(f"x has {x.size(0)} rows but the graph has {graph.num_src} source nodes")
    else:
        if x is not None:
            raise ValueError("a (ptr, plan) message layout takes the messages as `a`, not x")
        ptr, plan = graph
        where = (ptr, None, None, plan, a.size(0), None)
    ref = x if x is not None else a
    if ref is None or ref.dim() != 2:
        raise ValueError("softmax_aggregate takes two-dimensional x or a")
    if isinstance(t, Tensor):
        tt = t.reshape(-1).float().contiguous()
        if tt.numel() not in (1, ref.size(1)):
            raise ValueError(f"t must have 1 or {ref.size(1)} elements, got {t.numel()}")
    elif float(t) == 1.0:
        tt = None
    else:
        tt = torch.full((1, ), float(t), dtype=torch.float32, device=ref.device)
    x = None if x is None else x.contiguous()
    a = None if a is None else a.contiguous()
    want_lse = torch.is_grad_enabled() and any(v is not None and v.requires_grad for v in (x, a, tt))
    return _SoftmaxAggregate.apply(x, a, tt, where, float(eps), message, bool(semi_grad), want_lse)


class _PNAAggregate(torch.autograd.Function):

    @staticmethod
    def forward(ctx, x: Tensor, uv: Tensor, c: Optional[Tensor], avg_lin: Tensor, avg_log: Tensor, graph: CSRGraph,
                aggrs: tuple, scalers: tuple):
        N, T, F = x.shape
        W = T * F
        u, v = uv[:, :W], uv[:, W:]
        lin32 = avg_lin.detach().reshape(1).float().contiguous()
        log32 = avg_log.detach().reshape(1).float().contiguous()
        need_grad = any(ctx.needs_input_grad[:5])
        vv = None
        if c is None:
            vv = v.contiguous()
            res = ops.multi_aggr_csr(graph.rowptr, graph.col, vv, graph.num_dst, ops._pna_need(aggrs), graph.plan,
                                     with_ties=need_grad, count_self_zero=False)
        else:
            res = ops.pna_edge_stats(graph.rowptr, graph.col, graph.perm, v, c, graph.num_dst, aggrs, graph.plan,
                                     with_ties=need_grad)
        out = ops.pna_epilogue(graph.rowptr, x.reshape(N, W), u, res, aggrs, scalers, lin32, log32, T)
        ctx.graph, ctx.aggrs, ctx.scalers, ctx.shape = graph, aggrs, scalers, (N, T, F)
        ctx.keys, ctx.avg_dtypes = tuple(res), (avg_lin.dtype, avg_log.dtype)
        ctx.save_for_backward(uv, vv, c, lin32, log32, *res.values())
        return out

# ... 381 lines not shown
```

pytorch_geometric_b200/graph.py:

```python
from __future__ import annotations

from typing import Optional

import torch
from torch import Tensor

from . import ops

DEFAULT_CHUNK = 512
_INT32_MAX = 2**31 - 1


class CSRGraph:
    def __init__(self, src: Tensor, dst: Tensor, num_src: int, num_dst: int,
                 edge_weight: Optional[Tensor] = None, chunk: int = DEFAULT_CHUNK,
                 idx_dtype: Optional[torch.dtype] = None):
        if not src.is_cuda:
            raise RuntimeError("CSRGraph lives on a CUDA device (no CPU fallback)")
        E = src.numel()
        if idx_dtype is None:
            idx_dtype = torch.int32 if max(num_src, num_dst, E) < _INT32_MAX else torch.int64
        self.idx_dtype = idx_dtype
        self.num_src, self.num_dst, self.num_edges = int(num_src), int(num_dst), int(E)
        self.chunk = int(chunk)
        self.device = src.device
        self._src = ops.convert_index(src.contiguous(), idx_dtype)
        self._dst = ops.convert_index(dst.contiguous(), idx_dtype)
        _, self.perm, self.rowptr = ops.sort_by_key(self._dst, self.num_dst, want_sorted=False)
        self.col = ops.permute(self._src, self.perm)
        self.val = None if edge_weight is None else ops.permute(edge_weight.detach().float().contiguous(), self.perm)
        self.plan = ops.LongRowPlan(self.rowptr, self.chunk)
        self._t_built = False
        self.perm_t = self.rowptr_t = self.col_t = self.val_t = self.plan_t = None
        self._mean_val_t = None
        self._inv_perm = None
        self._inv_perm_t = None
        self._dst_csr = None
        self._t2csr = None

    @classmethod
    def from_edge_index(cls, edge_index: Tensor, num_nodes: Optional[int] = None,
                        edge_weight: Optional[Tensor] = None, num_src: Optional[int] = None,
                        num_dst: Optional[int] = None, **kw) -> "CSRGraph":
        if edge_index.dim() != 2 or edge_index.size(0) != 2:
            raise ValueError("edge_index must have shape [2, E]")
        if num_nodes is None and (num_src is None or num_dst is None):
            _, mx, _ = ops.index_stats(edge_index.reshape(-1)) if edge_index.numel() else (0, -1, True)
            num_nodes = mx + 1
        return cls(edge_index[0], edge_index[1], num_src if num_src is not None else num_nodes,
                   num_dst if num_dst is not None else num_nodes, edge_weight, **kw)

    @classmethod
    def from_csr(cls, rowptr: Tensor, col: Tensor, num_src: int, edge_weight: Optional[Tensor] = None,
                 transposed: Optional[tuple] = None, chunk: int = DEFAULT_CHUNK,
                 idx_dtype: Optional[torch.dtype] = None, bounded_degree: bool = False) -> "CSRGraph":
        if not rowptr.is_cuda:
            raise RuntimeError("CSRGraph lives on a CUDA device (no CPU fallback)")
        g = object.__new__(cls)
        E, n_dst = col.numel(), rowptr.numel() - 1
        if idx_dtype is None:
            idx_dtype = torch.int32 if max(num_src, n_dst, E) < _INT32_MAX else torch.int64
        g.idx_dtype = idx_dtype
        g.num_src, g.num_dst, g.num_edges = int(num_src), int(n_dst), int(E)
        g.chunk, g.device = int(chunk), rowptr.device
        g.rowptr = ops.convert_index(rowptr.contiguous(), idx_dtype)
        g.col = ops.convert_index(col.contiguous(), idx_dtype)
        g.perm = None
        g._src, g._dst = g.col, None
        g.val = None if edge_weight is None else edge_weight.detach().float().contiguous()
        g._bounded = bool(bounded_degree)
        g.plan = ops.LongRowPlan.empty(g.chunk) if bounded_degree else ops.LongRowPlan(g.rowptr, g.chunk)
        g._t_built = False
        g.perm_t = g.rowptr_t = g.col_t = g.val_t = g.plan_t = None
        g._mean_val_t = g._inv_perm = g._inv_perm_t = g._dst_csr = g._t2csr = None
        if transposed is not None:
            rowptr_t, col_t, perm_t = transposed
            g.rowptr_t = ops.convert_index(rowptr_t.contiguous(), idx_dtype)
            g.col_t = ops.convert_index(col_t.contiguous(), idx_dtype)
            g.perm_t = ops.convert_index(perm_t.contiguous(), idx_dtype)
            g.plan_t = ops.LongRowPlan(g.rowptr_t, g.chunk)
            g._t_built = True
            if g.val is not None:
                g.val_t = ops.permute(g.val, g.perm_t)
        return g

    def build_transpose(self) -> None:
        if self._t_built:
            return
        if self._dst is None:
            self._dst = self.dst_csr
        _, self.perm_t, self.rowptr_t = ops.sort_by_key(self._src, self.num_src, want_sorted=False)
        self.col_t = ops.permute(self._dst, self.perm_t)
        self.plan_t = ops.LongRowPlan(self.rowptr_t, self.chunk)
        self._t_built = True
        if self.val is not None:
            self.val_t = self.to_csc_order(self.from_csr_order(self.val))

    def trim(self, num_dst: int, num_src: int, num_edges: int) -> "CSRGraph":
        if self.perm is not None:
            raise ValueError("trim() needs a graph adopted with from_csr (edge order == CSR order)")
        if not (0 <= num_dst <= self.num_dst and 0 <= num_src <= self.num_src and 0 <= num_edges <= self.num_edges):
            raise ValueError("trim(): sizes must not exceed the graph's")
        g = object.__new__(CSRGraph)
        g.idx_dtype, g.chunk, g.device = self.idx_dtype, self.chunk, self.device
        g.num_src, g.num_dst, g.num_edges = int(num_src), int(num_dst), int(num_edges)
        g.rowptr = self.rowptr[:num_dst + 1].clamp(max=num_edges)
        g.col = self.col[:num_edges]
        g.perm = None
        g._src, g._dst = g.col, None
        g.val = None if self.val is None else self.val[:num_edges]
        g._bounded = getattr(self, "_bounded", False)
        g.plan = ops.LongRowPlan.empty(g.chunk) if g._bounded else ops.LongRowPlan(g.rowptr, g.chunk)
        g._t_built = False
        g.perm_t = g.rowptr_t = g.col_t = g.val_t = g.plan_t = None
        g._mean_val_t = g._inv_perm = g._inv_perm_t = g._dst_csr = g._t2csr = None
        return g

    def to_csr_order(self, per_edge: Tensor) -> Tensor:
        if self.perm is None:
            return per_edge.contiguous()
        return ops.permute(per_edge.contiguous(), self.perm)

    def to_csc_order(self, per_edge: Tensor) -> Tensor:
        self.build_transpose()
        return ops.permute(per_edge.contiguous(), self.perm_t)

    def _inverse(self, perm: Tensor) -> Tensor:
        inv = torch.empty_like(perm)
        inv[perm.long()] = torch.arange(perm.numel(), device=perm.device, dtype=perm.dtype)
        return inv

    def from_csr_order(self, per_edge_csr: Tensor) -> Tensor:
        if self.perm is None:
            return per_edge_csr.contiguous()
        if self._inv_perm is None:
            self._inv_perm = self._inverse(self.perm)
        return ops.permute(per_edge_csr.contiguous(), self._inv_perm)

    def from_csc_order(self, per_edge_csc: Tensor) -> Tensor:
        self.build_transpose()
        if self._inv_perm_t is None:
            self._inv_perm_t = self._inverse(self.perm_t)
        return ops.permute(per_edge_csc.contiguous(), self._inv_perm_t)

    def to_csr_order_rows(self, per_edge: Tensor) -> Tensor:
        if self.perm is None:
            return per_edge.contiguous()
        return ops.gather_rows(per_edge.contiguous(), self.perm)

    def from_csr_order_rows(self, per_edge_csr: Tensor) -> Tensor:
        if self.perm is None:
            return per_edge_csr.contiguous()
        if self._inv_perm is None:
            self._inv_perm = self._inverse(self.perm)
        return ops.gather_rows(per_edge_csr.contiguous(), self._inv_perm)

    @property
    def t2csr(self) -> Tensor:
        if getattr(self, "_t2csr", None) is None:
            self.build_transpose()
            if self.perm is None:
                self._t2csr = self.perm_t
            else:
                if self._inv_perm is None:
                    self._inv_perm = self._inverse(self.perm)
                self._t2csr = ops.permute(self._inv_perm, self.perm_t)
        return self._t2csr

    @property
    def dst_csr(self) -> Tensor:
        if self._dst_csr is None:
            self._dst_csr = ops.ptr2index(self.rowptr, self.num_edges)
        return self._dst_csr

    def in_degree(self) -> Tensor:
        return self.rowptr[1:] - self.rowptr[:-1]

    def mean_val_t(self) -> Tensor:
        if self._mean_val_t is None:
            self.build_transpose()
            inv = 1.0 / self.in_degree().clamp(min=1).to(torch.float32)
            self._mean_val_t = ops.gather_rows(inv.view(-1, 1), self.col_t).view(-1)
        return self._mean_val_t

    def with_values(self, val_csr: Optional[Tensor]) -> "CSRGraph":
        g = object.__new__(CSRGraph)
        g.__dict__.update(self.__dict__)
        g.val = val_csr
        g.val_t = None
        if val_csr is not None and self._t_built:
            g.val_t = g.to_csc_order(g.from_csr_order(val_csr))
        return g

    def nbytes(self) -> int:
        n = 0
        for t in (self.rowptr, self.col, self.perm, self.val, self.rowptr_t, self.col_t, self.perm_t, self.val_t,
                  self._src, self._dst):
            if t is not None:
                n += t.numel() * t.element_size()
        return n

    def __repr__(self) -> str:
        return (f"CSRGraph(num_src={self.num_src}, num_dst={self.num_dst}, num_edges={self.num_edges}, "
                f"idx={self.idx_dtype}, long_rows={self.plan.n_long}, chunks={self.plan.n_chunks})")


_GRAPH_CACHE: "dict" = {}
_GRAPH_CACHE_EDGES = 600_000_000


def _cache_put(key, holders, graph) -> None:
    _GRAPH_CACHE[key] = (holders, graph)
    total = sum(g.num_edges for _, g in _GRAPH_CACHE.values())
    while total > _GRAPH_CACHE_EDGES and len(_GRAPH_CACHE) > 1:
        k0 = next(iter(_GRAPH_CACHE))
        total -= _GRAPH_CACHE.pop(k0)[1].num_edges


def cached_graph(edge_index: Tensor, num_src: int, num_dst: int, flow: str = "source_to_target", loops: Optional[str] = None,
                 loop_nodes: Optional[int] = None, edge_type: Optional[Tensor] = None,
                 num_relations: Optional[int] = None) -> CSRGraph:
    if edge_index.dim() != 2 or edge_index.size(0) != 2:
        raise ValueError("edge_index must have shape [2, E]")
    key = (edge_index.data_ptr(), edge_index.numel(), edge_index._version, int(num_src), int(num_dst), flow, loops, loop_nodes,
           None if edge_type is None else (edge_type.data_ptr(), edge_type._version), num_relations)
    hit = _GRAPH_CACHE.get(key)
    if hit is not None:
        return hit[1]
    ei = edge_index
    if loops == "gat":
        from . import utils as U
        ei = U.remove_then_add_self_loops(edge_index, int(loop_nodes if loop_nodes is not None else min(num_src, num_dst)))
    src, dst = (ei[0], ei[1]) if flow == "source_to_target" else (ei[1], ei[0])
    if edge_type is not None:
        dst = dst.to(torch.int64) * int(num_relations) + edge_type.to(torch.int64)
    g = CSRGraph(src, dst, num_src, num_dst)
    _cache_put(key, (edge_index, edge_type), g)
    return g


def clear_graph_cache() -> None:
    _GRAPH_CACHE.clear()
```

pytorch_geometric_b200/nn/conv.py:

```python
from __future__ import annotations

import math
from typing import Optional, Union

import torch
import torch.nn.functional as F
from torch import Tensor

from .. import dense
from .. import functional as Fn
from .. import ops
from .. import utils as U
from ..graph import CSRGraph, cached_graph

Adj = Union[Tensor, CSRGraph]


def glorot_(w: Tensor) -> Tensor:
    a = math.sqrt(6.0 / (w.size(-2) + w.size(-1)))
    with torch.no_grad():
        return w.uniform_(-a, a)


class _Lin(torch.nn.Module):

    def __init__(self, in_channels: int, out_channels: int, bias: bool = True):
        super().__init__()
        self.weight = torch.nn.Parameter(torch.empty(out_channels, in_channels))
        self.bias = torch.nn.Parameter(torch.zeros(out_channels)) if bias else None
        glorot_(self.weight)

    def forward(self, x: Tensor) -> Tensor:
        return dense.linear(x, self.weight, self.bias)


def _w(mod):
    return None if mod is None else mod.weight


class _BiasAggregate(torch.autograd.Function):

    @staticmethod
    def forward(ctx, x: Tensor, bias: Tensor, graph: CSRGraph):
        ctx.graph = graph
        return ops.spmm_csr(graph.rowptr, graph.col, graph.val, x, graph.num_dst, "sum", graph.plan, bias=bias)

    @staticmethod
    def backward(ctx, grad_out: Tensor):
        graph = ctx.graph
        grad_out = grad_out.contiguous()
        gx = gb = None
        if ctx.needs_input_grad[0]:
            graph.build_transpose()
            gx = ops.spmm_csr(graph.rowptr_t, graph.col_t, graph.val_t, grad_out, graph.num_src, "sum", graph.plan_t)
        if ctx.needs_input_grad[1]:
            gb = ops.column_sum(grad_out)
        return gx, gb, None


def gcn_conv(x: Tensor, graph: CSRGraph, weight: Tensor, bias: Optional[Tensor]) -> Tensor:
    xw = dense.linear(x, weight)
    if bias is not None:
        return _BiasAggregate.apply(xw, bias, graph)
    return Fn.aggregate(graph, xw, "sum")


class _SageFused(torch.autograd.Function):

    @staticmethod
    def forward(ctx, x: Tensor, w_l: Tensor, b_l: Optional[Tensor], w_r: Tensor, graph: CSRGraph, aggr: str, relu: bool,
                input_is_relu: bool, grad_masked_by_consumer: bool):
        x = x.contiguous()
        agg = ops.spmm_csr(graph.rowptr, graph.col, graph.val, x, graph.num_dst, aggr, graph.plan)
        w_hi, w_lo = dense.split_tf32(torch.cat([w_l.detach(), w_r.detach()], dim=1))
        y, _ = dense.gemm_pair(agg, x, w_hi, w_lo, 0, w_l.size(0), bias=None if b_l is None else b_l.detach(), relu=relu)
        ctx.graph, ctx.aggr, ctx.relu, ctx.has_bias = graph, aggr, relu, b_l is not None
        ctx.input_is_relu, ctx.premasked = input_is_relu, grad_masked_by_consumer
        ctx.save_for_backward(x, agg, w_hi, w_lo, y if (relu and not grad_masked_by_consumer) else None)
        return y

    @staticmethod
    def backward(ctx, g: Tensor):
        x, agg, w_hi, w_lo, y = ctx.saved_tensors
        graph = ctx.graph
        g = g.contiguous()
        if ctx.relu and not ctx.premasked:
            g = g * (y > 0)
        k = x.size(1)
        gx = gwl = gwr = gb = None
        if ctx.needs_input_grad[0]:
            ga, gx = dense.gemm_pair(g, None, w_hi, w_lo, 1, k, k)
            graph.build_transpose()
            val_t = graph.mean_val_t() if ctx.aggr == "mean" else graph.val_t
            ops.spmm_csr(graph.rowptr_t, graph.col_t, val_t, ga, graph.num_src, "sum", graph.plan_t, out=gx, accumulate=True,
                         relu_mask=x if ctx.input_is_relu else None)
        if ctx.needs_input_grad[1]:
            gwl = dense._mm_tn(g, agg)
        if ctx.needs_input_grad[3]:
            gwr = dense._mm_tn(g, x)
        if ctx.has_bias and ctx.needs_input_grad[2]:
            gb = ops.column_sum(g)
        return gx, gwl, gb, gwr, None, None, None, None, None


def _sage_fusable(x_src: Tensor, x_dst: Optional[Tensor], graph: CSRGraph, aggr: str, w_l: Tensor, w_r: Optional[Tensor]) -> bool:
    k, n = x_src.size(1), w_l.size(0)
    return (x_dst is x_src and w_r is not None and aggr in ("mean", "sum", "add") and graph.val is None
            and graph.num_src == graph.num_dst and x_src.is_cuda and x_src.dtype == torch.float32 and w_l.dtype == torch.float32
            and dense.get_backend() == "tf32x3" and k % 128 == 0 and n % 128 == 0 and w_l.size(1) == k and w_r.size(1) == k
            and x_src.size(0) > 0)


def sage_conv(x_src: Tensor, x_dst: Optional[Tensor], graph: CSRGraph, aggr: str, w_l: Tensor, b_l: Optional[Tensor],
              w_r: Optional[Tensor], normalize: bool = False, relu: bool = False, input_is_relu: bool = False,
              grad_masked_by_consumer: bool = False) -> Tensor:
    if _sage_fusable(x_src, x_dst, graph, aggr, w_l, w_r):
        out = _SageFused.apply(x_src, w_l, b_l, w_r, graph, "sum" if aggr == "add" else aggr, relu, input_is_relu,
                               grad_masked_by_consumer and relu)
    else:
        agg = Fn.aggregate(graph, x_src, aggr)
        if w_r is not None and x_dst is not None:
            out = dense.linear_pair(agg, w_l, x_dst, w_r, b_l, relu=relu)
        else:
            out = dense.linear(agg, w_l, b_l, relu=relu)
    if normalize:
        out = F.normalize(out, p=2.0, dim=-1)
    return out


def graph_conv(x_src: Tensor, x_dst: Optional[Tensor], graph: CSRGraph, aggr: str, w_rel: Tensor, b_rel: Optional[Tensor],
               w_root: Tensor, edge_weight: Optional[Tensor] = None) -> Tensor:
    agg = Fn.aggregate(graph, x_src, aggr, edge_weight)
    if x_dst is not None:
        return dense.linear_pair(agg, w_rel, x_dst, w_root, b_rel)
    return dense.linear(agg, w_rel, b_rel)


def gin_aggregate(x_src: Tensor, x_dst: Optional[Tensor], graph: CSRGraph, eps) -> Tensor:
    out = Fn.aggregate(graph, x_src, "sum")
    if x_dst is not None:
        out = out + (1 + eps) * x_dst
    return out


class _HeadDot(torch.autograd.Function):

    @staticmethod
    def forward(ctx, xh, att_a, att_b, H, C):
        s_a, s_b = ops.head_dot(xh, att_a, att_b, H, C)
        ctx.save_for_backward(xh, att_a, att_b)
        ctx.hc = (H, C)
        return s_a, s_b

    @staticmethod
    def backward(ctx, g_a, g_b):
        xh, att_a, att_b = ctx.saved_tensors
        H, C = ctx.hc
        if g_a is None:
            g_a = torch.zeros(xh.size(0), H, dtype=torch.float32, device=xh.device)
        if att_b is not None and g_b is None:
            g_b = torch.zeros(xh.size(0), H, dtype=torch.float32, device=xh.device)
        gx, ga, gb = ops.head_dot_backward(xh, att_a, att_b, g_a, g_b if att_b is not None else None, None, H, C,
                                           ctx.needs_input_grad[0])
        ga = ga.view_as(att_a).to(att_a.dtype) if ctx.needs_input_grad[1] else None
        gb = gb.view_as(att_b).to(att_b.dtype) if att_b is not None and ctx.needs_input_grad[2] else None
        return gx, ga, gb, None, None


def _head_dot(xh: Tensor, att: Tensor, H: int, C: int, att2: Optional[Tensor] = None):
    if ops.head_dot_supported(xh, H, C):
        s_a, s_b = _HeadDot.apply(xh, att, att2, H, C)
        return s_a if att2 is None else (s_a, s_b)
    x3 = xh.view(-1, H, C).float()
    s_a = (x3 * att.view(1, H, C).float()).sum(dim=-1)
    return s_a if att2 is None else (s_a, (x3 * att2.view(1, H, C).float()).sum(dim=-1))


def _finish_heads(out: Tensor, H: int, C: int, concat: bool, res: Optional[Tensor], bias: Optional[Tensor]) -> Tensor:
    if not concat:
        out = out.view(-1, H, C).mean(dim=1)
    if res is not None:
        out = out + res
    if bias is not None:
        out = out + bias.to(out.dtype)
    return out


def gat_conv(xh_src: Tensor, xh_dst: Optional[Tensor], graph: CSRGraph, att_src: Tensor, att_dst: Optional[Tensor], H: int,
             C: int, negative_slope: float = 0.2, concat: bool = True, res: Optional[Tensor] = None,
             bias: Optional[Tensor] = None, s_edge: Optional[Tensor] = None, return_alpha: bool = False,
             dropout_p: float = 0.0):
    if att_dst is None:
        a_src = _head_dot(xh_src, att_src, H, C)
        a_dst = a_src.new_zeros(graph.num_dst, H)
    elif xh_dst is None:
        a_src, a_dst = _head_dot(xh_src, att_src, H, C, att_dst)
    else:
        a_src = _head_dot(xh_src, att_src, H, C)
        a_dst = _head_dot(xh_dst, att_dst, H, C)
    r = Fn.attention("gat", graph, H, C, v=xh_src, s_src=a_src, s_dst=a_dst, s_edge=s_edge, negative_slope=negative_slope,
                     return_alpha=return_alpha, dropout_p=dropout_p)
    out, alpha = r if return_alpha else (r, None)
    out = _finish_heads(out, H, C, concat, res, bias)
    return (out, alpha) if return_alpha else out


def gatv2_conv(x_l: Tensor, x_r: Tensor, graph: CSRGraph, att: Tensor, H: int, C: int, negative_slope: float = 0.2,
               concat: bool = True, res: Optional[Tensor] = None, bias: Optional[Tensor] = None, return_alpha: bool = False,
               dropout_p: float = 0.0, e_feat: Optional[Tensor] = None):
    r = Fn.attention("gatv2", graph, H, C, v=x_l, q=x_r, att=att.reshape(-1), negative_slope=negative_slope,
                     return_alpha=return_alpha, dropout_p=dropout_p, e_feat=e_feat)
    out, alpha = r if return_alpha else (r, None)
    out = _finish_heads(out, H, C, concat, res, bias)
    return (out, alpha) if return_alpha else out


def transformer_conv(query: Tensor, kv: Tensor, graph: CSRGraph, H: int, C: int, concat: bool = True,
                     x_skip: Optional[Tensor] = None, w_beta: Optional[Tensor] = None, return_alpha: bool = False,
                     dropout_p: float = 0.0, e_feat: Optional[Tensor] = None):
    r = Fn.attention("dot", graph, H, C, q=query, kv=kv, scale=1.0 / math.sqrt(C), return_alpha=return_alpha,
                     dropout_p=dropout_p, e_feat=e_feat)
    out, alpha = r if return_alpha else (r, None)
    if not concat:
        out = out.view(-1, H, C).mean(dim=1)
    if x_skip is not None:
        if w_beta is not None:
            beta = F.linear(torch.cat([out, x_skip, out - x_skip], dim=-1), w_beta).sigmoid()
            out = beta * x_skip + (1 - beta) * out
        else:
            out = out + x_skip
    return (out, alpha) if return_alpha else out


def rgcn_weight(weight: Tensor, comp: Optional[Tensor], num_relations: int, in_channels: int, out_channels: int,
                num_blocks: Optional[int]) -> Tensor:
    if comp is not None:
        return (comp @ weight.view(weight.size(0), -1)).view(num_relations, in_channels, out_channels)
    if num_blocks is not None:
        R, B, ci, co = weight.shape
        return torch.stack([torch.block_diag(*weight[r]) for r in range(R)])
    return weight


def rgcn_conv(x: Tensor, graph: CSRGraph, weight: Tensor, root: Optional[Tensor], bias: Optional[Tensor], aggr: str = "mean"):
    N = x.size(0)
    R, Fi, Fo = weight.shape
    h = Fn.aggregate(graph, x, aggr).view(N, R * Fi)
    w = weight.reshape(R * Fi, Fo)
    if root is not None:
        return dense.matmul_pair(h, w, x, root, bias)
    out = dense.matmul(h, w)
    return out if bias is None else out + bias.to(out.dtype)


def _src_dst(edge_index: Tensor, flow: str):
    return (edge_index[0], edge_index[1]) if flow == "source_to_target" else (edge_index[1], edge_index[0])


def _plain_graph(edge_index: Adj, num_src: int, num_dst: int, flow: str = "source_to_target") -> CSRGraph:
    if isinstance(edge_index, CSRGraph):
        return edge_index
    return cached_graph(edge_index, num_src, num_dst, flow=flow)


class GCNConv(torch.nn.Module):
    def __init__(self, in_channels: int, out_channels: int, improved: bool = False, cached: bool = False,
                 add_self_loops: Optional[bool] = None, normalize: bool = True, bias: bool = True, **kwargs):
        super().__init__()
        if add_self_loops is None:
            add_self_loops = normalize
        if add_self_loops and not normalize:
            raise ValueError(f"'{self.__class__.__name__}' does not support adding self-loops to the graph when no "
                             f"on-the-fly normalization is applied")
        self.in_channels, self.out_channels = in_channels, out_channels
        self.improved, self.cached = improved, cached
        self.add_self_loops, self.normalize = add_self_loops, normalize
        self.flow = kwargs.get("flow", "source_to_target")
        self.lin = _Lin(in_channels, out_channels, bias=False)
        self.bias = torch.nn.Parameter(torch.zeros(out_channels)) if bias else None
        self._cached_graph: Optional[CSRGraph] = None

    def reset_parameters(self):
        glorot_(self.lin.weight)
        if self.bias is not None:
            torch.nn.init.zeros_(self.bias)
        self._cached_graph = None

    def graph_for(self, edge_index: Adj, edge_weight: Optional[Tensor], num_nodes: int) -> CSRGraph:
        if isinstance(edge_index, CSRGraph):
            return edge_index
        if self._cached_graph is not None:
            return self._cached_graph
        if self.normalize:
            g = U.gcn_norm_graph(edge_index, edge_weight, num_nodes, self.improved, self.add_self_loops, self.flow)
        else:
            src, dst = _src_dst(edge_index, self.flow)
            g = CSRGraph(src, dst, num_nodes, num_nodes, edge_weight)
        if self.cached:
            self._cached_graph = g
        return g

    def forward(self, x: Tensor, edge_index: Adj, edge_weight: Optional[Tensor] = None) -> Tensor:
        if isinstance(x, (tuple, list)):
            raise ValueError(f"'{self.__class__.__name__}' received a tuple of node features as input while "
                             "this layer does not support bipartite message passing. Please try other layers "
                             "such as 'SAGEConv' or 'GraphConv' instead")
        return gcn_conv(x, self.graph_for(edge_index, edge_weight, x.size(0)), self.lin.weight, self.bias)

    def __repr__(self) -> str:
        return f"{self.__class__.__name__}({self.in_channels}, {self.out_channels})"


def _pair(x):
    return (x, x) if isinstance(x, Tensor) else (x[0], x[1])


def _num_dst(x, size):
    if x[1] is not None:
        return x[1].size(0)
    return size[1] if size is not None and size[1] is not None else x[0].size(0)


class SAGEConv(torch.nn.Module):
    def __init__(self, in_channels, out_channels: int, aggr: str = "mean", normalize: bool = False,
                 root_weight: bool = True, project: bool = False, bias: bool = True, **kwargs):
        super().__init__()
        if isinstance(in_channels, int):
            in_channels = (in_channels, in_channels)
        if aggr not in ("mean", "sum", "add", "max", "min"):
            raise ValueError(f"aggr='{aggr}' is not on the fused path")
        self.in_channels, self.out_channels = in_channels, out_channels
        self.aggr, self.normalize, self.root_weight, self.project = aggr, normalize, root_weight, project
        self.flow = kwargs.get("flow", "source_to_target")
        if project:
            self.lin = _Lin(in_channels[0], in_channels[0], bias=True)
        self.lin_l = _Lin(in_channels[0], out_channels, bias=bias)
        if root_weight:
            self.lin_r = _Lin(in_channels[1], out_channels, bias=False)

    def forward(self, x, edge_index: Adj, size=None) -> Tensor:
        x = _pair(x)
        if self.project and hasattr(self, "lin"):
            x = (self.lin(x[0]).relu(), x[1])
        graph = _plain_graph(edge_index, x[0].size(0), _num_dst(x, size), self.flow)
        return sage_conv(x[0], x[1], graph, self.aggr, self.lin_l.weight, self.lin_l.bias,
                         self.lin_r.weight if self.root_weight else None, self.normalize)

    def __repr__(self) -> str:
        return f"{self.__class__.__name__}({self.in_channels}, {self.out_channels}, aggr={self.aggr})"


class GraphConv(torch.nn.Module):
    def __init__(self, in_channels, out_channels: int, aggr: str = "add", bias: bool = True, **kwargs):
        super().__init__()
        if isinstance(in_channels, int):
            in_channels = (in_channels, in_channels)
        if aggr not in ("mean", "sum", "add", "max", "min"):
            raise ValueError(f"aggr='{aggr}' is not on the fused path")
        self.in_channels, self.out_channels, self.aggr = in_channels, out_channels, aggr
        self.flow = kwargs.get("flow", "source_to_target")
        self.lin_rel = _Lin(in_channels[0], out_channels, bias=bias)
        self.lin_root = _Lin(in_channels[1], out_channels, bias=False)

    def forward(self, x, edge_index: Adj, edge_weight: Optional[Tensor] = None, size=None) -> Tensor:
        x = _pair(x)
        graph = _plain_graph(edge_index, x[0].size(0), _num_dst(x, size), self.flow)
        return graph_conv(x[0], x[1], graph, self.aggr, self.lin_rel.weight, self.lin_rel.bias, self.lin_root.weight,
                          edge_weight)

    def __repr__(self) -> str:
        return f"{self.__class__.__name__}({self.in_channels[0]}, {self.out_channels})"


class GINConv(torch.nn.Module):
    def __init__(self, nn: torch.nn.Module, eps: float = 0.0, train_eps: bool = False, **kwargs):
        super().__init__()
        self.nn = nn
        self.initial_eps = eps
        self.flow = kwargs.get("flow", "source_to_target")
        if train_eps:
            self.eps = torch.nn.Parameter(torch.full((1, ), float(eps)))
        else:
            self.register_buffer("eps", torch.full((1, ), float(eps)))

    def forward(self, x, edge_index: Adj, size=None) -> Tensor:
        x = _pair(x)
        graph = _plain_graph(edge_index, x[0].size(0), _num_dst(x, size), self.flow)
        return self.nn(gin_aggregate(x[0], x[1], graph, self.eps))

    def __repr__(self) -> str:
        return f"{self.__class__.__name__}(nn={self.nn})"


class GINEConv(torch.nn.Module):

    def __init__(self, nn: torch.nn.Module, eps: float = 0.0, train_eps: bool = False, edge_dim: Optional[int] = None,
                 **kwargs):
        super().__init__()
# ... 542 lines not shown
```

pytorch_geometric_b200/ops.py:

```python
from __future__ import annotations

import ctypes
from typing import Optional, Tuple

import torch
from torch import Tensor

from ._lib import check, lib

F32, BF16 = 0, 1
I32, I64 = 0, 1
REDUCE = {"sum": 0, "add": 0, "mean": 1, "min": 2, "amin": 2, "max": 3, "amax": 3, "mul": 4}


class _Launches:
    count = 0


LAUNCHES = _Launches()


class _Profile:

    def __init__(self):
        self.enabled = False
        self.events = {}

    def reset(self, enabled: bool = False):
        self.enabled = enabled
        self.events = {}

    def begin(self, name: str):
        if not self.enabled:
            return None
        e0 = torch.cuda.Event(enable_timing=True)
        e1 = torch.cuda.Event(enable_timing=True)
        e0.record()
        self.events.setdefault(name, []).append((e0, e1))
        return e1

    def summary(self) -> dict:
        torch.cuda.synchronize()
        out = {}
        for k, v in self.events.items():
            each = [a.elapsed_time(b) for a, b in v]
            out[k] = {"ms_total": sum(each), "calls": len(each), "ms_each": each}
        return out


PROFILE = _Profile()


def _timed(name: str, n_kernels: int, fn, *args):
    LAUNCHES.count += n_kernels
    end = PROFILE.begin(name)
    rc = fn(*args)
    if end is not None:
        end.record()
    check(rc, name)


def _stream() -> int:
    return torch.cuda.current_stream().cuda_stream


def _p(t: Optional[Tensor]):
    return None if t is None else t.data_ptr()


def _cuda(*ts: Optional[Tensor]) -> None:
    for t in ts:
        if t is not None and not t.is_cuda:
            raise RuntimeError("pytorch_geometric_b200 ops run on CUDA tensors only (no CPU fallback); "
                               f"got a tensor on {t.device}")


def _idt(t: Tensor) -> int:
    if t.dtype == torch.int32:
        return I32
    if t.dtype == torch.int64:
        return I64
    raise TypeError(f"index tensors must be int32 or int64, got {t.dtype}")


def _vdt(t: Tensor) -> int:
    if t.dtype == torch.float32:
        return F32
    if t.dtype == torch.bfloat16:
        return BF16
    raise TypeError(f"feature tensors must be float32 or bfloat16, got {t.dtype}")


def _same_idx(*ts: Optional[Tensor]) -> int:
    ds = {t.dtype for t in ts if t is not None}
    if len(ds) != 1:
        raise TypeError(f"index tensors of one call must share a dtype, got {ds}")
    return _idt(next(t for t in ts if t is not None))


def _ws(nbytes: int, device) -> Tensor:
    return torch.empty(max(int(nbytes), 256), dtype=torch.uint8, device=device)


def degree(index: Tensor, num_nodes: int) -> Tensor:
    _cuda(index)
    index = index.contiguous()
    deg = torch.empty(num_nodes, dtype=index.dtype, device=index.device)
    check(lib().b200mp_degree(_p(index), index.numel(), num_nodes, _p(deg), _idt(index), _stream()), "degree")
    return deg


def index2ptr(index: Tensor, size: int) -> Tensor:
    _cuda(index)
    index = index.contiguous()
    ptr = torch.empty(size + 1, dtype=index.dtype, device=index.device)
    check(lib().b200mp_index2ptr(_p(index), index.numel(), size, _p(ptr), _idt(index), _stream()), "index2ptr")
    return ptr


def ptr2index(ptr: Tensor, output_size: Optional[int] = None) -> Tensor:
    _cuda(ptr)
    ptr = ptr.contiguous()
    n = int(ptr[-1]) if output_size is None else int(output_size)
    index = torch.empty(n, dtype=ptr.dtype, device=ptr.device)
    check(lib().b200mp_ptr2index(_p(ptr), ptr.numel() - 1, n, _p(index), _idt(ptr), _stream()), "ptr2index")
    return index


def index_stats(index: Tensor) -> Tuple[int, int, bool]:
    _cuda(index)
    index = index.contiguous()
    st = torch.empty(3, dtype=torch.int64, device=index.device)
    check(lib().b200mp_index_stats(_p(index), index.numel(), _p(st), _idt(index), _stream()), "index_stats")
    mn, mx, srt = st.tolist()
    return mn, mx, bool(srt)


def sort_by_key(keys: Tensor, num_nodes: int, want_sorted: bool = True,
                want_ptr: bool = True) -> Tuple[Optional[Tensor], Tensor, Optional[Tensor]]:
    _cuda(keys)
    keys = keys.contiguous()
    n = keys.numel()
    it = _idt(keys)
    ws = _ws(lib().b200mp_sort_workspace_bytes(n, num_nodes, it), keys.device)
    ks = torch.empty_like(keys) if want_sorted else None
    perm = torch.empty_like(keys)
    ptr = torch.empty(num_nodes + 1, dtype=keys.dtype, device=keys.device) if want_ptr else None
    check(lib().b200mp_sort_by_key(_p(keys), n, num_nodes, _p(ks), _p(perm), _p(ptr), _p(ws), ws.numel(), it,
                                   _stream()), "sort_by_key")
    return ks, perm, ptr


def permute(src: Tensor, perm: Tensor) -> Tensor:
    _cuda(src, perm)
    src, perm = src.contiguous(), perm.contiguous()
    out = torch.empty(perm.numel(), dtype=src.dtype, device=src.device)
    check(lib().b200mp_permute(_p(src), _p(perm), _p(out), perm.numel(), src.element_size(), _idt(perm),
                               _stream()), "permute")
    return out


def convert_index(index: Tensor, dtype: torch.dtype) -> Tensor:
    _cuda(index)
    if index.dtype == dtype:
        return index
    index = index.contiguous()
    out = torch.empty(index.shape, dtype=dtype, device=index.device)
    check(lib().b200mp_convert_index(_p(index), _idt(index), _p(out), _idt(out), index.numel(), _stream()),
          "convert_index")
    return out


def self_loops(row: Tensor, col: Tensor, weight: Optional[Tensor], num_nodes: int, fill_value: float = 1.0,
               mode: int = 0) -> Tuple[Tensor, Tensor, Optional[Tensor]]:
    _cuda(row, col, weight)
    row, col = row.contiguous(), col.contiguous()
    it = _same_idx(row, col)
    E = row.numel()
    if weight is not None:
        weight = weight.contiguous().float()
    ws = _ws(lib().b200mp_self_loops_workspace_bytes(E, num_nodes, it), row.device)
    r2 = torch.empty(E + num_nodes, dtype=row.dtype, device=row.device)
    c2 = torch.empty_like(r2)
    w2 = torch.empty(E + num_nodes, dtype=torch.float32, device=row.device) if weight is not None else None
    n_out = torch.empty(1, dtype=torch.int64, device=row.device)
    check(lib().b200mp_self_loops(_p(row), _p(col), _p(weight), E, num_nodes, float(fill_value), mode, _p(r2),
                                  _p(c2), _p(w2), _p(n_out), _p(ws), ws.numel(), it, _stream()), "self_loops")
    n = int(n_out.item())
    return r2[:n], c2[:n], (w2[:n] if w2 is not None else None)


def gcn_norm_csr(rowptr: Tensor, src: Tensor, weight: Optional[Tensor]) -> Tuple[Tensor, Tensor]:
    _cuda(rowptr, src, weight)
    it = _same_idx(rowptr, src)
    N, E = rowptr.numel() - 1, src.numel()
    dinv = torch.empty(N, dtype=torch.float32, device=rowptr.device)
    w_out = torch.empty(E, dtype=torch.float32, device=rowptr.device)
    check(lib().b200mp_gcn_norm_csr(_p(rowptr), _p(src), _p(weight), N, E, _p(dinv), _p(w_out), it, _stream()),
          "gcn_norm_csr")
    return dinv, w_out


class LongRowPlan:

    __slots__ = ("long_rows", "chunk_ptr", "n_long", "n_chunks", "chunk", "_partials")

    def __init__(self, rowptr: Tensor, chunk: int):
        _cuda(rowptr)
        it = _idt(rowptr)
        n_rows = rowptr.numel() - 1
        counts = torch.empty(2, dtype=torch.int64, device=rowptr.device)
        check(lib().b200mp_csr_plan_count(_p(rowptr), n_rows, chunk, _p(counts), it, _stream()), "csr_plan_count")
        self.n_long, self.n_chunks = (int(v) for v in counts.tolist())
        self.chunk = int(chunk)
        self.long_rows = self.chunk_ptr = None
        self._partials = None
        if self.n_long:
            self.long_rows = torch.empty(self.n_long, dtype=torch.int64, device=rowptr.device)
            self.chunk_ptr = torch.empty(self.n_long + 1, dtype=torch.int64, device=rowptr.device)
            ws = _ws(lib().b200mp_csr_plan_workspace_bytes(n_rows, self.n_long, it), rowptr.device)
            check(lib().b200mp_csr_plan_fill(_p(rowptr), n_rows, chunk, self.n_long, _p(self.long_rows),
                                             _p(self.chunk_ptr), _p(ws), ws.numel(), it, _stream()),
                  "csr_plan_fill")

    @classmethod
    def empty(cls, chunk: int = 512) -> "LongRowPlan":
        p = object.__new__(cls)
        p.n_long = p.n_chunks = 0
        p.chunk = int(chunk)
        p.long_rows = p.chunk_ptr = p._partials = None
        return p

    def partials(self, feat: int, device) -> Optional[Tensor]:
        if not self.n_long:
            return None
        need = self.n_chunks * feat
        if self._partials is None or self._partials.numel() < need:
            self._partials = torch.empty(need, dtype=torch.float32, device=device)
        return self._partials


def spmm_csr(rowptr: Tensor, col: Tensor, val: Optional[Tensor], x: Tensor, n_rows: int, reduce: str = "sum",
             plan: Optional[LongRowPlan] = None, out: Optional[Tensor] = None,
             bias: Optional[Tensor] = None, x_halo: Optional[Tensor] = None, accumulate: bool = False,
             peer_ptrs: Optional[int] = None, peer_rows: int = 0, relu_mask: Optional[Tensor] = None) -> Tensor:
    _cuda(rowptr, col, val, x)
    if x.dim() != 2:
        raise ValueError("spmm_csr expects a 2-D feature matrix")
    x = x.contiguous()
    it = _same_idx(rowptr, col)
    if val is not None and (val.dtype != torch.float32 or not val.is_contiguous()):
        val = val.contiguous().float()
    F = x.size(1)
    if out is None:
        out = torch.empty(n_rows, F, dtype=x.dtype, device=x.device)
    if plan is not None and plan.n_long:
        part = plan.partials(F, x.device)
        args = (_p(plan.long_rows), _p(plan.chunk_ptr), plan.n_long, plan.n_chunks, plan.chunk, _p(part))
    else:
        args = (None, None, 0, 0, 0, None)
    if bias is not None:
        _cuda(bias)
        if bias.dtype != torch.float32 or not bias.is_contiguous():
            bias = bias.detach().float().contiguous()
        if bias.numel() != F:
            raise ValueError("bias must have one entry per feature")
    if relu_mask is not None:
        _cuda(relu_mask)
        if not accumulate or relu_mask.dtype != x.dtype or tuple(relu_mask.shape) != (n_rows, F) or not relu_mask.is_contiguous():
            raise ValueError("relu_mask needs accumulate=True and a contiguous [n_rows, F] tensor of x's dtype")
    n_cols, n_local = x.size(0), 0
    if x_halo is not None:
        _cuda(x_halo)
        if x_halo.dtype != x.dtype or x_halo.dim() != 2 or x_halo.size(1) != F or not x_halo.is_contiguous():
            raise ValueError("x_halo must be a contiguous [n_halo, F] tensor of x's dtype")
        n_local, n_cols = x.size(0), x.size(0) + x_halo.size(0)
    _timed("spmm_csr", 2 if args[2] else 1, lib().b200mp_spmm_csr, _p(rowptr), _p(col), _p(val), _p(x), _p(out),
           n_rows, n_cols, F, REDUCE[reduce], *args, _p(bias), _p(x_halo), n_local, int(bool(accumulate)),
           peer_ptrs, int(peer_rows), _p(relu_mask), it, _vdt(x), _stream())
    return out


SEGMENT_PLAN_MIN_ROWS = 1 << 16
SEGMENT_CHUNK = 512


_PLAN_CACHE: "dict" = {}
_PLAN_CACHE_MAX = 32


def segment_plan(ptr: Tensor, n_src: int) -> Optional["LongRowPlan"]:
    if n_src < SEGMENT_PLAN_MIN_ROWS:
        return None
    import weakref
    key = id(ptr)
    hit = _PLAN_CACHE.get(key)
    if hit is not None and hit[0]() is ptr and hit[1] == ptr._version:
        return hit[2]
    plan = LongRowPlan(ptr, SEGMENT_CHUNK)
    plan = plan if plan.n_long else None
    if len(_PLAN_CACHE) >= _PLAN_CACHE_MAX:
        for k in [k for k, v in _PLAN_CACHE.items() if v[0]() is None] or list(_PLAN_CACHE)[:1]:
            _PLAN_CACHE.pop(k, None)
    try:
        _PLAN_CACHE[key] = (weakref.ref(ptr), ptr._version, plan)
    except TypeError:
        pass
    return plan


def segment_csr(src: Tensor, ptr: Tensor, reduce: str = "sum", plan: Optional["LongRowPlan"] = None) -> Tensor:
    _cuda(src, ptr)
    src = src.contiguous()
    n_rows = ptr.numel() - 1
    flat = src.view(src.size(0), -1)
    out = torch.empty((n_rows, flat.size(1)), dtype=src.dtype, device=src.device)
    pargs, _ = _plan_args(plan, flat.size(1), src.device)
    _timed("segment_csr", 2 if pargs[2] else 1, lib().b200mp_segment_csr, _p(ptr), _p(flat), _p(out), n_rows,
           flat.size(0), flat.size(1), REDUCE[reduce], *pargs, _idt(ptr), _vdt(src), _stream())
    return out.view((n_rows, ) + tuple(src.shape[1:]))


def minmax_ties(rowptr: Tensor, col: Tensor, val: Optional[Tensor], x: Tensor, out: Tensor,
                count_self_zero: bool = True) -> Tensor:
    _cuda(rowptr, col, val, x, out)
    it = _same_idx(rowptr, col)
    ties = torch.empty(out.shape, dtype=torch.float32, device=out.device)
    check(lib().b200mp_minmax_ties(_p(rowptr), _p(col), _p(val), _p(x), _p(out), _p(ties), out.size(0),
                                   out.size(1), int(count_self_zero), it, _vdt(x), _stream()), "minmax_ties")
    return ties


def minmax_backward(rowptr_t: Tensor, col_t: Tensor, val_t: Optional[Tensor], x: Tensor, out: Tensor,
                    grad_out: Tensor, ties: Tensor) -> Tensor:
    _cuda(rowptr_t, col_t, val_t, x, out, grad_out, ties)
    it = _same_idx(rowptr_t, col_t)
    gx = torch.empty_like(x)
    check(lib().b200mp_minmax_backward(_p(rowptr_t), _p(col_t), _p(val_t), _p(x), _p(out), _p(grad_out),
                                       _p(ties), _p(gx), x.size(0), x.size(1), it, _vdt(x), _stream()),
          "minmax_backward")
    return gx


def sddmm_csr(rowptr: Tensor, col: Tensor, a: Tensor, b: Tensor) -> Tensor:
    _cuda(rowptr, col, a, b)
    it = _same_idx(rowptr, col)
    a, b = a.contiguous(), b.contiguous()
    dot = torch.empty(col.numel(), dtype=torch.float32, device=a.device)
    check(lib().b200mp_sddmm_csr(_p(rowptr), _p(col), _p(a), _p(b), _p(dot), rowptr.numel() - 1, a.size(1), it,
                                 _vdt(a), _stream()), "sddmm_csr")
    return dot


def edge_relu_csr(rowptr: Tensor, col: Tensor, perm: Optional[Tensor], x: Tensor, edge_rows: Tensor, n_rows: int,
                  reduce: str = "sum", plan: Optional[LongRowPlan] = None,
                  want_mask: bool = False) -> Tuple[Tensor, Optional[Tensor]]:
    _cuda(rowptr, col, perm, x, edge_rows)
    if reduce not in ("sum", "add", "mean"):
        raise ValueError(f"edge_relu_csr reduces by sum or mean, not '{reduce}'")
    x, edge_rows = x.contiguous(), edge_rows.contiguous()
    E, F = col.numel(), x.size(1)
    if edge_rows.dtype != x.dtype or tuple(edge_rows.shape) != (E, F):
        raise ValueError(f"edge_rows must be a [{E}, {F}] tensor of x's dtype, got {tuple(edge_rows.shape)} {edge_rows.dtype}")
    it = _same_idx(rowptr, col, perm)
    out = torch.empty(n_rows, F, dtype=x.dtype, device=x.device)
    mask = torch.empty(E, (F + 7) // 8, dtype=torch.uint8, device=x.device) if want_mask else None
    pargs, _ = _plan_args(plan, F, x.device)
    _timed("edge_relu_csr", 2 if pargs[2] else 1, lib().b200mp_edge_relu_csr, _p(rowptr), _p(col), _p(perm), _p(x),
           _p(edge_rows), _p(out), _p(mask), n_rows, x.size(0), E, F, REDUCE[reduce], *pargs, it, _vdt(x), _stream())
    return out, mask


def edge_relu_backward_x(rowptr_t: Tensor, col_t: Tensor, t2csr: Tensor, val_t: Optional[Tensor], grad_out: Tensor,
                         mask: Tensor, n_src: int, plan_t: Optional[LongRowPlan] = None) -> Tensor:
    _cuda(rowptr_t, col_t, t2csr, val_t, grad_out, mask)
    grad_out = grad_out.contiguous()
    it = _same_idx(rowptr_t, col_t, t2csr)
    F = grad_out.size(1)
    grad_x = torch.empty(n_src, F, dtype=grad_out.dtype, device=grad_out.device)
    pargs, _ = _plan_args(plan_t, F, grad_out.device)
    _timed("edge_relu_backward_x", 2 if pargs[2] else 1, lib().b200mp_edge_relu_backward_x, _p(rowptr_t), _p(col_t),
           _p(t2csr), _p(val_t), _p(grad_out), _p(mask), _p(grad_x), n_src, F, *pargs, it, _vdt(grad_out), _stream())
    return grad_x


def edge_relu_backward_edge(rowptr: Tensor, perm: Optional[Tensor], grad_out: Tensor, mask: Tensor, n_edges: int,
                            reduce: str = "sum", plan: Optional[LongRowPlan] = None) -> Tensor:
    _cuda(rowptr, perm, grad_out, mask)
    grad_out = grad_out.contiguous()
    it = _same_idx(rowptr, perm)
    F = grad_out.size(1)
    grad = torch.empty(n_edges, F, dtype=grad_out.dtype, device=grad_out.device)
    if n_edges == 0:
        return grad
    pargs = (_p(plan.long_rows), _p(plan.chunk_ptr), plan.n_long, plan.n_chunks, plan.chunk) \
        if plan is not None and plan.n_long else (None, None, 0, 0, 0)
    _timed("edge_relu_backward_edge", 1, lib().b200mp_edge_relu_backward_edge, _p(rowptr), _p(perm), _p(grad_out),
           _p(mask), _p(grad), rowptr.numel() - 1, F, REDUCE[reduce], *pargs, it, _vdt(grad_out), _stream())
    return grad


def _gated_rows(k: Tensor, q: Tensor, v: Tensor) -> int:
    F = k.size(1)
    if k.dim() != 2 or not k.is_contiguous():
        raise ValueError("k must be a contiguous 2-D tensor")
    for name, t in (("q", q), ("v", v)):
        if t.dim() != 2 or t.size(1) != F or t.dtype != k.dtype or (t.size(0) > 0 and t.stride(1) != 1):
            raise ValueError(f"{name} must be a [N, {F}] tensor of k's dtype with unit feature stride, "
                             f"got {tuple(t.shape)} {t.dtype}")
    if q.size(0) != v.size(0) or q.stride(0) != v.stride(0) or q.stride(0) < F:
        raise ValueError(f"q and v must have the same rows and one row stride >= {F}, got strides "
                         f"{q.stride()} and {v.stride()}")
    return q.stride(0)


def gated_csr(rowptr: Tensor, col: Tensor, k: Tensor, q: Tensor, v: Tensor, n_rows: int, reduce: str = "sum",
              plan: Optional[LongRowPlan] = None) -> Tensor:
    _cuda(rowptr, col, k, q, v)
    if reduce not in ("sum", "add", "mean"):
        raise ValueError(f"gated_csr reduces by sum or mean, not '{reduce}'")
    ld = _gated_rows(k, q, v)
    it = _same_idx(rowptr, col)
    F = k.size(1)
    out = torch.empty(n_rows, F, dtype=k.dtype, device=k.device)
    pargs, _ = _plan_args(plan, F, k.device)
    _timed("gated_csr", 2 if pargs[2] else 1, lib().b200mp_gated_csr, _p(rowptr), _p(col), _p(k), _p(q), _p(v),
           _p(out), n_rows, q.size(0), col.numel(), F, ld, REDUCE[reduce], *pargs, it, _vdt(k), _stream())
    return out


def gated_backward_dst(rowptr: Tensor, col: Tensor, k: Tensor, q: Tensor, v: Tensor, grad_out: Tensor,
                       reduce: str = "sum", plan: Optional[LongRowPlan] = None) -> Tensor:
    _cuda(rowptr, col, k, q, v, grad_out)
    ld = _gated_rows(k, q, v)
    grad_out = grad_out.contiguous()
    it = _same_idx(rowptr, col)
    F = k.size(1)
    grad_k = torch.empty_like(k)
    pargs, _ = _plan_args(plan, F, k.device)
    _timed("gated_backward_dst", 2 if pargs[2] else 1, lib().b200mp_gated_backward_dst, _p(rowptr), _p(col), _p(k),
           _p(q), _p(v), _p(grad_out), _p(grad_k), k.size(0), q.size(0), col.numel(), F, ld, REDUCE[reduce], *pargs,
           it, _vdt(k), _stream())
    return grad_k


def gated_backward_src(rowptr_t: Tensor, col_t: Tensor, val_t: Optional[Tensor], k: Tensor, q: Tensor, v: Tensor,
                       grad_out: Tensor, grad_q: Tensor, grad_v: Tensor,
                       plan_t: Optional[LongRowPlan] = None) -> Tuple[Tensor, Tensor]:
    _cuda(rowptr_t, col_t, val_t, k, q, v, grad_out, grad_q, grad_v)
    ld = _gated_rows(k, q, v)
    if _gated_rows(k, grad_q, grad_v) != ld or grad_q.size(0) != q.size(0):
        raise ValueError("grad_q and grad_v must have the shape and row stride of q and v")
    grad_out = grad_out.contiguous()
    it = _same_idx(rowptr_t, col_t)
    F = k.size(1)
    pargs, _ = _plan_args(plan_t, 2 * F, k.device)
    _timed("gated_backward_src", 2 if pargs[2] else 1, lib().b200mp_gated_backward_src, _p(rowptr_t), _p(col_t),
           _p(val_t), _p(k), _p(q), _p(v), _p(grad_out), _p(grad_q), _p(grad_v), q.size(0), k.size(0), col_t.numel(),
           F, ld, *pargs, it, _vdt(k), _stream())
    return grad_q, grad_v


def _cg_rows(u: Tensor, v: Tensor, c: Optional[Tensor], n_edges: int) -> int:
    if u.dim() != 2 or u.size(1) % 2:
        raise ValueError(f"u must be a [N, 2F] tensor, got {tuple(u.shape)}")
    F = u.size(1) // 2
    for name, t in (("u", u), ("v", v)):
        if t.dim() != 2 or t.size(1) != 2 * F or t.dtype != u.dtype or (t.size(0) > 0 and t.stride(1) != 1) \
                or (t.size(0) > 1 and t.stride(0) < 2 * F):
            raise ValueError(f"{name} must be a [N, {2 * F}] tensor of u's dtype with unit feature stride, "
                             f"got {tuple(t.shape)} {t.dtype} strides {t.stride()}")
    if c is not None and (tuple(c.shape) != (n_edges, 2 * F) or c.dtype != u.dtype or not c.is_contiguous()):
        raise ValueError(f"c must be a contiguous [{n_edges}, {2 * F}] tensor of u's dtype, got {tuple(c.shape)} {c.dtype}")
    return F


def _ld(t: Tensor) -> int:
    return t.stride(0) if t.size(0) > 1 else t.size(1)


def cg_csr(rowptr: Tensor, col: Tensor, perm: Optional[Tensor], u: Tensor, v: Tensor, c: Optional[Tensor],
           n_rows: int, reduce: str = "sum", plan: Optional[LongRowPlan] = None) -> Tensor:
    _cuda(rowptr, col, perm, u, v, c)
    if reduce not in ("sum", "add", "mean"):
        raise ValueError(f"cg_csr reduces by sum or mean, not '{reduce}'")
    F = _cg_rows(u, v, c, col.numel())
    it = _same_idx(rowptr, col, perm)
    out = torch.empty(n_rows, F, dtype=u.dtype, device=u.device)
    pargs, _ = _plan_args(plan, F, u.device)
    _timed("cg_csr", 2 if pargs[2] else 1, lib().b200mp_cg_csr, _p(rowptr), _p(col), _p(perm), _p(u), _p(v), _p(c),
           _p(out), n_rows, v.size(0), col.numel(), F, _ld(u), _ld(v), REDUCE[reduce], *pargs, it, _vdt(u), _stream())
    return out


def cg_backward_dst(rowptr: Tensor, col: Tensor, perm: Optional[Tensor], u: Tensor, v: Tensor, c: Optional[Tensor],
                    grad_out: Tensor, grad_u: Tensor, want_grad_c: bool, reduce: str = "sum",
                    plan: Optional[LongRowPlan] = None) -> Optional[Tensor]:
    _cuda(rowptr, col, perm, u, v, c, grad_out, grad_u)
    F = _cg_rows(u, v, c, col.numel())
    if _cg_rows(grad_u, v, None, 0) != F or grad_u.size(0) != u.size(0) or _ld(grad_u) != _ld(u):
        raise ValueError("grad_u must have the shape and row stride of u")
    if want_grad_c and c is None:
        raise ValueError("grad_c is the gradient of c: want_grad_c needs c")
    grad_out = grad_out.contiguous()
    it = _same_idx(rowptr, col, perm)
    E = col.numel()
    grad_c = torch.empty(E, 2 * F, dtype=u.dtype, device=u.device) if want_grad_c else None
    pargs, _ = _plan_args(plan, 2 * F, u.device)
    _timed("cg_backward_dst", 2 if pargs[2] else 1, lib().b200mp_cg_backward_dst, _p(rowptr), _p(col), _p(perm), _p(u),
           _p(v), _p(c), _p(grad_out), _p(grad_u), _p(grad_c), u.size(0), v.size(0), E, F, _ld(u), _ld(v),
           REDUCE[reduce], *pargs, it, _vdt(u), _stream())
    return grad_c


def cg_backward_src(rowptr_t: Tensor, col_t: Tensor, perm_t: Tensor, val_t: Optional[Tensor], u: Tensor, v: Tensor,
                    c: Optional[Tensor], grad_out: Tensor, grad_v: Tensor,
                    plan_t: Optional[LongRowPlan] = None) -> Tensor:
    _cuda(rowptr_t, col_t, perm_t, val_t, u, v, c, grad_out, grad_v)
    E = col_t.numel()
    F = _cg_rows(u, v, c, E)
    if _cg_rows(u, grad_v, None, 0) != F or grad_v.size(0) != v.size(0) or _ld(grad_v) != _ld(v):
        raise ValueError("grad_v must have the shape and row stride of v")
    grad_out = grad_out.contiguous()
    it = _same_idx(rowptr_t, col_t, perm_t)
    pargs, _ = _plan_args(plan_t, 2 * F, u.device)
    _timed("cg_backward_src", 2 if pargs[2] else 1, lib().b200mp_cg_backward_src, _p(rowptr_t), _p(col_t), _p(perm_t),
           _p(val_t), _p(u), _p(v), _p(c), _p(grad_out), _p(grad_v), v.size(0), u.size(0), E, F, _ld(u), _ld(v),
           *pargs, it, _vdt(u), _stream())
    return grad_v


SOFTMAX_MESSAGES = {"identity": 0, "relu_eps": 1}


def _softmax_aggr_args(x: Optional[Tensor], a: Optional[Tensor], t: Optional[Tensor], message: str, n_edges: int):
    if message not in SOFTMAX_MESSAGES:
        raise ValueError(f"message must be one of {sorted(SOFTMAX_MESSAGES)}, got '{message}'")
    if message == "relu_eps" and x is None:
        raise ValueError("the relu_eps message needs x")
    if message == "identity" and (x is None) == (a is None):
        raise ValueError("the identity message takes exactly one of x and the edge rows")
    ref = x if x is not None else a
    F = ref.size(1)
    for name, v in (("x", x), ("edge rows", a)):
        if v is not None and (v.dim() != 2 or v.size(1) != F or v.dtype != ref.dtype or not v.is_contiguous()):
            raise ValueError(f"{name} must be a contiguous [N, {F}] tensor of dtype {ref.dtype}, got {tuple(v.shape)}")
    if a is not None and a.size(0) != n_edges:
        raise ValueError(f"edge rows must have {n_edges} rows, got {a.size(0)}")
    t_mode = 0
    if t is not None:
        if t.dtype != torch.float32 or not t.is_contiguous() or t.numel() not in (1, F):
            raise ValueError(f"t must be a contiguous float32 tensor of 1 or {F} elements, got {tuple(t.shape)} {t.dtype}")
        t_mode = 1 if t.numel() == 1 else 2
    return F, SOFTMAX_MESSAGES[message], t_mode


def softmax_aggr_csr(rowptr: Tensor, col: Optional[Tensor], perm: Optional[Tensor], x: Optional[Tensor],
                     a: Optional[Tensor], t: Optional[Tensor], n_rows: int, n_edges: int, message: str = "identity",
                     eps: float = 0.0, plan: Optional[LongRowPlan] = None,
                     want_lse: bool = False) -> Tuple[Tensor, Optional[Tensor]]:
    _cuda(rowptr, col, perm, x, a, t)
    F, msg, t_mode = _softmax_aggr_args(x, a, t, message, n_edges)
    it = _same_idx(rowptr, col, perm)
    ref = x if x is not None else a
    out = torch.empty(n_rows, F, dtype=ref.dtype, device=ref.device)
    lse = torch.empty(n_rows, F, dtype=torch.float32, device=ref.device) if want_lse else None
    pargs, _ = _plan_args(plan, 3 * F, ref.device)
    _timed("softmax_aggr_csr", 2 if pargs[2] else 1, lib().b200mp_softmax_aggr_csr, _p(rowptr), _p(col), _p(perm),
           _p(x), _p(a), _p(t), _p(out), _p(lse), n_rows, 0 if x is None else x.size(0), n_edges, F, msg, float(eps),
           t_mode, *pargs, it, _vdt(ref), _stream())
    return out, lse


def softmax_aggr_backward_dst(rowptr: Tensor, col: Optional[Tensor], perm: Optional[Tensor], x: Optional[Tensor],
                              a: Optional[Tensor], t: Optional[Tensor], out: Tensor, lse: Tensor, grad_out: Tensor,
                              n_edges: int, message: str, eps: float, semi_grad: bool, want_grad_a: bool,
                              want_grad_t: bool, plan: Optional[LongRowPlan] = None):
    _cuda(rowptr, col, perm, x, a, t, out, lse, grad_out)
    F, msg, t_mode = _softmax_aggr_args(x, a, t, message, n_edges)
    if want_grad_t and t is None:
        raise ValueError("grad_t needs t")
    it = _same_idx(rowptr, col, perm)
    grad_out = grad_out.contiguous()
# ... 537 lines not shown
```

Before: 888.5 million.

## Add degree-class L2 eviction hints for hot source rows in CSR SpMM

Precomputes a per-edge class byte from the source node's degree, plus a degree histogram, when the graph and its transpose are built. At launch time a class threshold is picked so the hottest rows fit in half of L2. A hinted kernel variant then loads those gathered feature rows with an evict_last policy, and loads the other rows and all index/value streams with evict_first. This aims to raise L2 hit rates for high-degree neighbours. The cost is an extra uint8 read per edge, per-graph preprocessing with a host sync for the histogram, and a fixed launch config that bypasses the existing tuning switch.

```diff
diff --git a/include/b200mp.h b/include/b200mp.h
--- a/include/b200mp.h
+++ b/include/b200mp.h
@@ -58,12 +58,24 @@
                          int64_t* long_rows, int64_t* chunk_ptr, void* workspace,
                          int64_t workspace_bytes, int idx_dtype, void* stream);
 
+int b200mp_slot_class(const void* ptr, const void* col, int64_t n_slots, uint8_t* cls, int idx_dtype, void* stream);
+int b200mp_class_histogram(const void* ptr, int64_t n_rows, int64_t* hist_dev, int idx_dtype, void* stream);
+
 int b200mp_spmm_csr(const void* rowptr, const void* col, const float* val, const void* x,
                     void* out, int64_t n_rows, int64_t n_cols, int64_t feat, int reduce,
                     const int64_t* long_rows, const int64_t* chunk_ptr, int64_t n_long_rows,
                     int64_t n_chunks, int64_t chunk, float* partials, const float* bias,
                     const void* x_halo, int64_t n_local_cols, int flags, const void* peer_ptrs,
                     int64_t peer_rows, const void* relu_mask, int idx_dtype, int val_dtype, void* stream);
+
+typedef struct b200mp_spmm_csr_args {
+    const void* rowptr; const void* col; const float* val; const void* x; void* out;
+    int64_t n_rows; int64_t n_cols; int64_t feat; int reduce;
+    const int64_t* long_rows; const int64_t* chunk_ptr; int64_t n_long_rows; int64_t n_chunks; int64_t chunk;
+    float* partials; const float* bias; const void* x_halo; int64_t n_local_cols; int flags;
+    const void* peer_ptrs; int64_t peer_rows; const void* relu_mask; int idx_dtype; int val_dtype; void* stream;
+} b200mp_spmm_csr_args;
+int b200mp_spmm_csr_hinted(const b200mp_spmm_csr_args* a, const uint8_t* row_class, int class_min);
 
 int b200mp_segment_csr(const void* ptr, const void* src, void* out, int64_t n_rows, int64_t n_src,
                        int64_t feat, int reduce, const int64_t* long_rows, const int64_t* chunk_ptr,
diff --git a/pytorch_geometric_b200/_lib.py b/pytorch_geometric_b200/_lib.py
--- a/pytorch_geometric_b200/_lib.py
+++ b/pytorch_geometric_b200/_lib.py
@@ -33,6 +33,9 @@
     "b200mp_csr_plan_fill": (_INT, [_P, _I64, _I64, _I64, _P, _P, _P, _I64, _INT, _P]),
     "b200mp_spmm_csr": (_INT, [_P, _P, _P, _P, _P, _I64, _I64, _I64, _INT, _P, _P, _I64, _I64, _I64, _P,
                                _P, _P, _I64, _INT, _P, _I64, _P, _INT, _INT, _P]),
+    "b200mp_spmm_csr_hinted": (_INT, [_P, _P, _INT]),
+    "b200mp_slot_class": (_INT, [_P, _P, _I64, _P, _INT, _P]),
+    "b200mp_class_histogram": (_INT, [_P, _I64, _P, _INT, _P]),
     "b200mp_segment_csr": (_INT, [_P, _P, _P, _I64, _I64, _I64, _INT, _P, _P, _I64, _I64, _I64, _P, _INT, _INT, _P]),
     "b200mp_minmax_ties": (_INT, [_P, _P, _P, _P, _P, _P, _I64, _I64, _INT, _INT, _INT, _P]),
     "b200mp_minmax_backward": (_INT, [_P, _P, _P, _P, _P, _P, _P, _P, _I64, _I64, _INT, _INT, _P]),
diff --git a/pytorch_geometric_b200/csrc/common.cuh b/pytorch_geometric_b200/csrc/common.cuh
--- a/pytorch_geometric_b200/csrc/common.cuh
+++ b/pytorch_geometric_b200/csrc/common.cuh
@@ -88,6 +88,43 @@
                  : "l"(p));
     return v;
 }
+__device__ __forceinline__ uint64_t l2_policy_evict_first() {
+    uint64_t pol;
+    asm("createpolicy.fractional.L2::evict_first.b64 %0, 1.0;" : "=l"(pol));
+    return pol;
+}
+__device__ __forceinline__ uint64_t l2_policy_evict_last() {
+    uint64_t pol;
+    asm("createpolicy.fractional.L2::evict_last.b64 %0, 1.0;" : "=l"(pol));
+    return pol;
+}
+__device__ __forceinline__ Vec16 ldg_row16_hint(const void* p, uint64_t pol) {
+    Vec16 v;
+    asm volatile("ld.global.nc.L1::no_allocate.L2::cache_hint.v4.u32 {%0,%1,%2,%3}, [%4], %5;"
+                 : "=r"(v.w[0]), "=r"(v.w[1]), "=r"(v.w[2]), "=r"(v.w[3])
+                 : "l"(p), "l"(pol));
+    return v;
+}
+__device__ __forceinline__ uint32_t ldg_u32_hint(const void* p, uint64_t pol) {
+    uint32_t v;
+    asm volatile("ld.global.nc.L1::no_allocate.L2::cache_hint.u32 %0, [%1], %2;" : "=r"(v) : "l"(p), "l"(pol));
+    return v;
+}
+__device__ __forceinline__ uint64_t ldg_u64_hint(const void* p, uint64_t pol) {
+    uint64_t v;
+    asm volatile("ld.global.nc.L1::no_allocate.L2::cache_hint.u64 %0, [%1], %2;" : "=l"(v) : "l"(p), "l"(pol));
+    return v;
+}
+__device__ __forceinline__ uint32_t ldg_u8_hint(const void* p, uint64_t pol) {
+    uint32_t v;
+    asm volatile("ld.global.nc.L1::no_allocate.L2::cache_hint.u8 %0, [%1], %2;" : "=r"(v) : "l"(p), "l"(pol));
+    return v;
+}
+template <typename I>
+__device__ __forceinline__ I ldg_idx_hint(const I* p, uint64_t pol) {
+    if constexpr (sizeof(I) == 8) return static_cast<I>(ldg_u64_hint(p, pol));
+    else return static_cast<I>(ldg_u32_hint(p, pol));
+}
 __device__ __forceinline__ Vec16 ldg_stream16(const void* p) {
     Vec16 v;
     asm volatile("ld.global.cs.v4.u32 {%0,%1,%2,%3}, [%4];"
diff --git a/pytorch_geometric_b200/csrc/csr_dispatch.cuh b/pytorch_geometric_b200/csrc/csr_dispatch.cuh
--- a/pytorch_geometric_b200/csrc/csr_dispatch.cuh
+++ b/pytorch_geometric_b200/csrc/csr_dispatch.cuh
@@ -10,7 +10,7 @@
 template <typename T, typename I, int RED, bool GATHER>
 int csr_reduce_variant(const I* rowptr, const I* col, const float* val, const T* x, T* out, int64_t n_rows,
                        int64_t feat, bool is_mean, bool inf_to_zero, LongRowPlan plan, const float* bias,
-                       cudaStream_t stream) {
+                       cudaStream_t stream, const uint8_t* row_class, int class_min) {
     if (n_rows == 0 || feat == 0) return B200MP_OK;
     const size_t row_bytes = static_cast<size_t>(feat) * sizeof(T);
     const bool tma_ok = row_bytes % 16 == 0 && row_bytes >= 512 && row_bytes <= 2048 && aligned16(x) &&
@@ -20,22 +20,22 @@
         return csr_tma_launch<T, I, RED, GATHER>(rowptr, col, val, x, out, n_rows, feat, is_mean, inf_to_zero, plan,
                                                  bias, stream);
     return csr_reduce_dispatch<T, I, RED, GATHER>(rowptr, col, val, x, out, n_rows, feat, is_mean, inf_to_zero, plan,
-                                                  bias, stream);
+                                                  bias, stream, row_class, class_min);
 }
 
 template <typename T, typename I, bool GATHER>
 int csr_reduce_auto(const I* rowptr, const I* col, const float* val, const T* x, T* out, int64_t n_rows,
                     int64_t feat, int reduce, bool inf_to_zero, LongRowPlan plan, const float* bias,
-                    cudaStream_t stream) {
+                    cudaStream_t stream, const uint8_t* row_class = nullptr, int class_min = 0) {
     switch (reduce) {
         case B200MP_SUM:
-            return csr_reduce_variant<T, I, B200MP_SUM, GATHER>(rowptr, col, val, x, out, n_rows, feat, false, false, plan, bias, stream);
+            return csr_reduce_variant<T, I, B200MP_SUM, GATHER>(rowptr, col, val, x, out, n_rows, feat, false, false, plan, bias, stream, row_class, class_min);
         case B200MP_MEAN:
-            return csr_reduce_variant<T, I, B200MP_SUM, GATHER>(rowptr, col, val, x, out, n_rows, feat, true, false, plan, bias, stream);
+            return csr_reduce_variant<T, I, B200MP_SUM, GATHER>(rowptr, col, val, x, out, n_rows, feat, true, false, plan, bias, stream, row_class, class_min);
         case B200MP_MIN:
-            return csr_reduce_variant<T, I, B200MP_MIN, GATHER>(rowptr, col, val, x, out, n_rows, feat, false, inf_to_zero, plan, bias, stream);
+            return csr_reduce_variant<T, I, B200MP_MIN, GATHER>(rowptr, col, val, x, out, n_rows, feat, false, inf_to_zero, plan, bias, stream, row_class, class_min);
         case B200MP_MAX:
-            return csr_reduce_variant<T, I, B200MP_MAX, GATHER>(rowptr, col, val, x, out, n_rows, feat, false, inf_to_zero, plan, bias, stream);
+            return csr_reduce_variant<T, I, B200MP_MAX, GATHER>(rowptr, col, val, x, out, n_rows, feat, false, inf_to_zero, plan, bias, stream, row_class, class_min);
         default:
             set_error("csr_reduce: unsupported reduce %d", reduce);
             return B200MP_ERR_UNSUPPORTED;
diff --git a/pytorch_geometric_b200/csrc/csr_reduce.cuh b/pytorch_geometric_b200/csrc/csr_reduce.cuh
--- a/pytorch_geometric_b200/csrc/csr_reduce.cuh
+++ b/pytorch_geometric_b200/csrc/csr_reduce.cuh
@@ -78,12 +78,13 @@
 }
 
 template <typename T, typename I, int G, int VPL, int RED, bool GATHER, int UNR_OVR = 0, int BLOCK = 256,
-          int MINB = 1>
+          int MINB = 1, bool HINT = false>
 __global__ void __launch_bounds__(BLOCK, MINB)
 csr_reduce_kernel(const I* __restrict__ rowptr, const I* __restrict__ col,
                   const float* __restrict__ val, const T* __restrict__ x, T* __restrict__ out,
                   int64_t n_rows, int n_vec, bool is_mean, bool inf_to_zero, LongRowPlan plan,
-                  const float* __restrict__ bias) {
+                  const float* __restrict__ bias, const uint8_t* __restrict__ row_class, int class_min) {
+    static_assert(!HINT || (G == 32 && GATHER), "L2 hints need a warp-uniform gathered row");
     constexpr int EPV = ElemTraits<T>::kPerVec;
     constexpr int UNR = UNR_OVR ? UNR_OVR : (VPL == 1 ? 8 : (VPL == 2 ? 4 : 2));
     const int lig = threadIdx.x & (G - 1);
@@ -110,14 +111,25 @@
         const size_t voff = static_cast<size_t>(vbase + lig) * 16;
 
         if (G == 32) {
+            uint64_t pol_cold = 0, pol_hot = 0;
+            if constexpr (HINT) {
+                pol_cold = l2_policy_evict_first();
+                pol_hot = l2_policy_evict_last();
+            }
             for (int64_t e0 = begin; e0 < end; e0 += 32) {
                 const int n = static_cast<int>(end - e0 < 32 ? end - e0 : 32);
                 int64_t c_l = 0;
                 float w_l = 1.0f;
                 if (lig < n) {
-                    c_l = GATHER ? static_cast<int64_t>(ldg_idx(col + e0 + lig)) : (e0 + lig);
-                    if (val) w_l = __ldg(val + e0 + lig);
+                    if constexpr (HINT) {
+                        c_l = static_cast<int64_t>(ldg_idx_hint(col + e0 + lig, pol_cold));
+                        if (val) w_l = __uint_as_float(ldg_u32_hint(val + e0 + lig, pol_cold));
+                    } else {
+                        c_l = GATHER ? static_cast<int64_t>(ldg_idx(col + e0 + lig)) : (e0 + lig);
+                        if (val) w_l = __ldg(val + e0 + lig);
+                    }
                     c_l = static_cast<int64_t>(reinterpret_cast<uintptr_t>(row_base(plan, xb, xb2, split, row_bytes, c_l)));
+                    if constexpr (HINT) c_l |= static_cast<int>(ldg_u8_hint(row_class + e0 + lig, pol_cold)) >= class_min;
                 }
                 for (int j = 0; j < n; j += UNR) {
                     Vec16 buf[UNR][VPL];
@@ -127,10 +139,18 @@
                         const int64_t c = __shfl_sync(0xffffffffu, c_l, (j + u) & 31);
                         w[u] = __shfl_sync(0xffffffffu, w_l, (j + u) & 31);
                         if (j + u < n) {
-                            const char* p = reinterpret_cast<const char*>(static_cast<uintptr_t>(c)) + voff;
-#pragma unroll
-                            for (int k = 0; k < VPL; ++k)
-                                if (vvalid[k]) buf[u][k] = ldg_row16(p + static_cast<size_t>(k) * G * 16);
+                            if constexpr (HINT) {
+                                const char* p = reinterpret_cast<const char*>(static_cast<uintptr_t>(c & ~int64_t{1})) + voff;
+                                const uint64_t pol = (c & 1) ? pol_hot : pol_cold;
+#pragma unroll
+                                for (int k = 0; k < VPL; ++k)
+                                    if (vvalid[k]) buf[u][k] = ldg_row16_hint(p + static_cast<size_t>(k) * G * 16, pol);
+                            } else {
+                                const char* p = reinterpret_cast<const char*>(static_cast<uintptr_t>(c)) + voff;
+#pragma unroll
+                                for (int k = 0; k < VPL; ++k)
+                                    if (vvalid[k]) buf[u][k] = ldg_row16(p + static_cast<size_t>(k) * G * 16);
+                            }
                         }
                     }
 #pragma unroll
@@ -289,13 +309,22 @@
 template <typename T, typename I, int RED, bool GATHER, int G, int VPL>
 inline void launch_vec(const I* rowptr, const I* col, const float* val, const T* x, T* out,
                        int64_t n_rows, int n_vec, bool is_mean, bool inf_to_zero,
-                       const LongRowPlan& plan, const float* bias, cudaStream_t stream) {
+                       const LongRowPlan& plan, const float* bias, const uint8_t* row_class, int class_min,
+                       cudaStream_t stream) {
     const int64_t items = plan.n_chunks + n_rows;
     if (items == 0) return;
-#define B200MP_LAUNCH_TUNED(UNR_, BLOCK_, MINB_)                                                           \
-    csr_reduce_kernel<T, I, G, VPL, RED, GATHER, UNR_, BLOCK_, MINB_>                                      \
+#define B200MP_LAUNCH_HINTED(UNR_, BLOCK_, MINB_, HINT_)                                                   \
+    csr_reduce_kernel<T, I, G, VPL, RED, GATHER, UNR_, BLOCK_, MINB_, HINT_>                               \
         <<<static_cast<unsigned>(ceil_div(items, BLOCK_ / G)), BLOCK_, 0, stream>>>(                       \
-            rowptr, col, val, x, out, n_rows, n_vec, is_mean, inf_to_zero, plan, bias)
+            rowptr, col, val, x, out, n_rows, n_vec, is_mean, inf_to_zero, plan, bias, row_class, class_min)
+#define B200MP_LAUNCH_TUNED(UNR_, BLOCK_, MINB_) B200MP_LAUNCH_HINTED(UNR_, BLOCK_, MINB_, false)
+    if constexpr (G == 32 && GATHER) {
+        if (row_class) {
+            if (sizeof(T) == 4) B200MP_LAUNCH_HINTED(unroll_for_vpl<VPL>(), 128, 12, true);
+            else B200MP_LAUNCH_HINTED(unroll_for_vpl<VPL>(), 128, 8, true);
+            return;
+        }
+    }
     if (G == 32 && VPL == 2 && RED == B200MP_SUM && GATHER) {
         switch (get_option_spmm_tune()) {
             case 1: B200MP_LAUNCH_TUNED(4, 256, 1); return;
@@ -307,12 +336,14 @@
     if (sizeof(T) == 4) B200MP_LAUNCH_TUNED(unroll_for_vpl<VPL>(), 128, 12);
     else B200MP_LAUNCH_TUNED(unroll_for_vpl<VPL>(), 128, 8);
 #undef B200MP_LAUNCH_TUNED
+#undef B200MP_LAUNCH_HINTED
 }
 
 template <typename T, typename I, int RED, bool GATHER>
 int csr_reduce_dispatch(const I* rowptr, const I* col, const float* val, const T* x, T* out,
                         int64_t n_rows, int64_t feat, bool is_mean, bool inf_to_zero,
-                        LongRowPlan plan, const float* bias, cudaStream_t stream) {
+                        LongRowPlan plan, const float* bias, cudaStream_t stream,
+                        const uint8_t* row_class = nullptr, int class_min = 0) {
     if (n_rows == 0 || feat == 0) return B200MP_OK;
     const size_t row_bytes = static_cast<size_t>(feat) * sizeof(T);
     const bool vec_ok = (row_bytes % 16 == 0) && aligned16(x) && aligned16(out) && aligned16(plan.x2) &&
@@ -321,7 +352,7 @@
         const int n_vec = static_cast<int>(row_bytes / 16);
         lane_group_shape<4>(n_vec, [&](auto G, auto VPL) {
             launch_vec<T, I, RED, GATHER, G(), VPL()>(rowptr, col, val, x, out, n_rows, n_vec, is_mean, inf_to_zero,
-                                                      plan, bias, stream);
+                                                      plan, bias, row_class, class_min, stream);
         });
     } else {
         int g = 1;
diff --git a/pytorch_geometric_b200/csrc/spmm.cu b/pytorch_geometric_b200/csrc/spmm.cu
--- a/pytorch_geometric_b200/csrc/spmm.cu
+++ b/pytorch_geometric_b200/csrc/spmm.cu
@@ -102,16 +102,17 @@
 
 using namespace b200mp;
 
-extern "C" int b200mp_spmm_csr(const void* rowptr, const void* col, const float* val, const void* x,
-                               void* out, int64_t n_rows, int64_t n_cols, int64_t feat, int reduce,
-                               const int64_t* long_rows, const int64_t* chunk_ptr,
-                               int64_t n_long_rows, int64_t n_chunks, int64_t chunk, float* partials,
-                               const float* bias, const void* x_halo, int64_t n_local_cols, int flags,
-                               const void* peer_ptrs, int64_t peer_rows, const void* relu_mask, int idx_dtype,
-                               int val_dtype, void* stream) {
+static int spmm_csr_impl(const void* rowptr, const void* col, const float* val, const void* x,
+                         void* out, int64_t n_rows, int64_t n_cols, int64_t feat, int reduce,
+                         const int64_t* long_rows, const int64_t* chunk_ptr,
+                         int64_t n_long_rows, int64_t n_chunks, int64_t chunk, float* partials,
+                         const float* bias, const void* x_halo, int64_t n_local_cols, int flags,
+                         const void* peer_ptrs, int64_t peer_rows, const void* relu_mask, int idx_dtype,
+                         int val_dtype, void* stream, const uint8_t* row_class, int class_min) {
     B200MP_CHECK_ARG(n_rows >= 0 && n_cols >= 0 && feat >= 0);
     B200MP_CHECK_ARG((flags & ~1) == 0 && (!(flags & 1) || (reduce == B200MP_SUM && !bias)));
     B200MP_CHECK_ARG(!relu_mask || (flags & 1));
+    B200MP_CHECK_ARG(class_min >= 0 && class_min <= 255);
     LongRowPlan plan;
     if (int rc = make_plan(plan, long_rows, chunk_ptr, n_long_rows, n_chunks, chunk, partials, true)) return rc;
     if (n_rows == 0 || feat == 0) return B200MP_OK;
@@ -132,8 +133,28 @@
         using I = decltype(ti);
         return csr_reduce_auto<T, I, true>(static_cast<const I*>(rowptr), static_cast<const I*>(col), val,
                                             static_cast<const T*>(x), static_cast<T*>(out), n_rows, feat, reduce,
-                                            false, plan, bias, static_cast<cudaStream_t>(stream));
-    });
+                                            false, plan, bias, static_cast<cudaStream_t>(stream), row_class, class_min);
+    });
+}
+
+extern "C" int b200mp_spmm_csr(const void* rowptr, const void* col, const float* val, const void* x,
+                               void* out, int64_t n_rows, int64_t n_cols, int64_t feat, int reduce,
+                               const int64_t* long_rows, const int64_t* chunk_ptr,
+                               int64_t n_long_rows, int64_t n_chunks, int64_t chunk, float* partials,
+                               const float* bias, const void* x_halo, int64_t n_local_cols, int flags,
+                               const void* peer_ptrs, int64_t peer_rows, const void* relu_mask, int idx_dtype,
+                               int val_dtype, void* stream) {
+    return spmm_csr_impl(rowptr, col, val, x, out, n_rows, n_cols, feat, reduce, long_rows, chunk_ptr, n_long_rows,
+                         n_chunks, chunk, partials, bias, x_halo, n_local_cols, flags, peer_ptrs, peer_rows, relu_mask,
+                         idx_dtype, val_dtype, stream, nullptr, 0);
+}
+
+extern "C" int b200mp_spmm_csr_hinted(const b200mp_spmm_csr_args* a, const uint8_t* row_class, int class_min) {
+    B200MP_CHECK_ARG(a);
+    return spmm_csr_impl(a->rowptr, a->col, a->val, a->x, a->out, a->n_rows, a->n_cols, a->feat, a->reduce, a->long_rows,
+                         a->chunk_ptr, a->n_long_rows, a->n_chunks, a->chunk, a->partials, a->bias, a->x_halo,
+                         a->n_local_cols, a->flags, a->peer_ptrs, a->peer_rows, a->relu_mask, a->idx_dtype, a->val_dtype,
+                         a->stream, row_class, class_min);
 }
 
 extern "C" int b200mp_minmax_ties(const void* rowptr, const void* col, const float* val, const void* x,
diff --git a/pytorch_geometric_b200/csrc/structure.cu b/pytorch_geometric_b200/csrc/structure.cu
--- a/pytorch_geometric_b200/csrc/structure.cu
+++ b/pytorch_geometric_b200/csrc/structure.cu
@@ -285,6 +285,30 @@
     nchunks[j] = (deg + chunk - 1) / chunk;
 }
 
+__device__ __forceinline__ int degree_class(int64_t deg) { return deg <= 0 ? 0 : 63 - __clzll(deg); }
+
+template <typename I>
+__global__ void slot_class_kernel(const I* __restrict__ ptr, const I* __restrict__ col, int64_t n_slots,
+                                  uint8_t* __restrict__ cls) {
+    const int64_t e = static_cast<int64_t>(blockIdx.x) * blockDim.x + threadIdx.x;
+    if (e >= n_slots) return;
+    const int64_t c = col[e];
+    cls[e] = static_cast<uint8_t>(degree_class(static_cast<int64_t>(ptr[c + 1]) - static_cast<int64_t>(ptr[c])));
+}
+
+template <typename I>
+__global__ void class_histogram_kernel(const I* __restrict__ ptr, int64_t n_rows, unsigned long long* __restrict__ hist) {
+    __shared__ unsigned long long h[64];
+    for (int k = threadIdx.x; k < 64; k += blockDim.x) h[k] = 0;
+    __syncthreads();
+    for (int64_t r = static_cast<int64_t>(blockIdx.x) * blockDim.x + threadIdx.x; r < n_rows;
+         r += static_cast<int64_t>(gridDim.x) * blockDim.x)
+        atomicAdd(&h[degree_class(static_cast<int64_t>(ptr[r + 1]) - static_cast<int64_t>(ptr[r]))], 1ull);
+    __syncthreads();
+    for (int k = threadIdx.x; k < 64; k += blockDim.x)
+        if (h[k]) atomicAdd(hist + k, h[k]);
+}
+
 }
 
 using namespace b200mp;
@@ -526,3 +550,29 @@
     set_error("bad idx_dtype %d", idx_dtype);
     return B200MP_ERR_UNSUPPORTED;
 }
+
+extern "C" int b200mp_slot_class(const void* ptr, const void* col, int64_t n_slots, uint8_t* cls, int idx_dtype,
+                                 void* stream) {
+    B200MP_CHECK_ARG(n_slots >= 0);
+    if (n_slots == 0) return B200MP_OK;
+    B200MP_CHECK_ARG(ptr && col && cls);
+    cudaStream_t s = static_cast<cudaStream_t>(stream);
+    IDX_DISPATCH((slot_class_kernel<int32_t><<<grid_for(n_slots), kThreads, 0, s>>>(static_cast<const int32_t*>(ptr), static_cast<const int32_t*>(col), n_slots, cls)),
+                 (slot_class_kernel<int64_t><<<grid_for(n_slots), kThreads, 0, s>>>(static_cast<const int64_t*>(ptr), static_cast<const int64_t*>(col), n_slots, cls)));
+    B200MP_LAUNCH_CHECK();
+    return B200MP_OK;
+}
+
+extern "C" int b200mp_class_histogram(const void* ptr, int64_t n_rows, int64_t* hist_dev, int idx_dtype, void* stream) {
+    B200MP_CHECK_ARG(n_rows >= 0 && hist_dev);
+    cudaStream_t s = static_cast<cudaStream_t>(stream);
+    B200MP_CUDA(cudaMemsetAsync(hist_dev, 0, 64 * sizeof(int64_t), s));
+    if (n_rows == 0) return B200MP_OK;
+    B200MP_CHECK_ARG(ptr);
+    const unsigned blocks = static_cast<unsigned>(std::min<int64_t>(ceil_div(n_rows, kThreads), 4 * num_sms()));
+    auto* h = reinterpret_cast<unsigned long long*>(hist_dev);
+    IDX_DISPATCH((class_histogram_kernel<int32_t><<<blocks, kThreads, 0, s>>>(static_cast<const int32_t*>(ptr), n_rows, h)),
+                 (class_histogram_kernel<int64_t><<<blocks, kThreads, 0, s>>>(static_cast<const int64_t*>(ptr), n_rows, h)));
+    B200MP_LAUNCH_CHECK();
+    return B200MP_OK;
+}
diff --git a/pytorch_geometric_b200/functional.py b/pytorch_geometric_b200/functional.py
--- a/pytorch_geometric_b200/functional.py
+++ b/pytorch_geometric_b200/functional.py
@@ -15,7 +15,8 @@
         val = graph.val
         if edge_weight is not None:
             val = graph.to_csr_order(edge_weight.detach().float().contiguous().view(-1))
-        out = ops.spmm_csr(graph.rowptr, graph.col, val, x, graph.num_dst, reduce, graph.plan)
+        out = ops.spmm_csr(graph.rowptr, graph.col, val, x, graph.num_dst, reduce, graph.plan,
+                           row_class=graph.row_class, class_hist=graph.class_hist)
         ctx.graph, ctx.reduce = graph, reduce
         ctx.has_ew = edge_weight is not None
         need_x = reduce in ("min", "max") or (ctx.has_ew and edge_weight.requires_grad)
@@ -35,12 +36,14 @@
                 graph.to_csc_order(graph.from_csr_order(val))
         if ctx.needs_input_grad[0]:
             if reduce in ("sum", "add"):
-                gx = ops.spmm_csr(graph.rowptr_t, graph.col_t, val_t, grad_out, graph.num_src, "sum", graph.plan_t)
+                gx = ops.spmm_csr(graph.rowptr_t, graph.col_t, val_t, grad_out, graph.num_src, "sum", graph.plan_t,
+                                  row_class=graph.row_class_t, class_hist=graph.class_hist_t)
             elif reduce == "mean":
                 mv = graph.mean_val_t()
                 if val_t is not None:
                     mv = mv * val_t
-                gx = ops.spmm_csr(graph.rowptr_t, graph.col_t, mv, grad_out, graph.num_src, "sum", graph.plan_t)
+                gx = ops.spmm_csr(graph.rowptr_t, graph.col_t, mv, grad_out, graph.num_src, "sum", graph.plan_t,
+                                  row_class=graph.row_class_t, class_hist=graph.class_hist_t)
             else:
                 ties = ops.minmax_ties(graph.rowptr, graph.col, val, x, out, count_self_zero=True)
                 gx = ops.minmax_backward(graph.rowptr_t, graph.col_t, val_t, x, out, grad_out, ties)
diff --git a/pytorch_geometric_b200/graph.py b/pytorch_geometric_b200/graph.py
--- a/pytorch_geometric_b200/graph.py
+++ b/pytorch_geometric_b200/graph.py
@@ -12,6 +12,8 @@
 
 
 class CSRGraph:
+    row_class = row_class_t = class_hist = class_hist_t = None
+
     def __init__(self, src: Tensor, dst: Tensor, num_src: int, num_dst: int,
                  edge_weight: Optional[Tensor] = None, chunk: int = DEFAULT_CHUNK,
                  idx_dtype: Optional[torch.dtype] = None):
@@ -80,6 +82,7 @@
             g.perm_t = ops.convert_index(perm_t.contiguous(), idx_dtype)
             g.plan_t = ops.LongRowPlan(g.rowptr_t, g.chunk)
             g._t_built = True
+            g._build_classes()
             if g.val is not None:
                 g.val_t = ops.permute(g.val, g.perm_t)
         return g
@@ -93,8 +96,15 @@
         self.col_t = ops.permute(self._dst, self.perm_t)
         self.plan_t = ops.LongRowPlan(self.rowptr_t, self.chunk)
         self._t_built = True
+        self._build_classes()
         if self.val is not None:
             self.val_t = self.to_csc_order(self.from_csr_order(self.val))
+
+    def _build_classes(self) -> None:
+        self.row_class = ops.slot_class(self.rowptr_t, self.col)
+        self.row_class_t = ops.slot_class(self.rowptr, self.col_t)
+        self.class_hist = ops.class_histogram(self.rowptr_t)
+        self.class_hist_t = ops.class_histogram(self.rowptr)
 
     def trim(self, num_dst: int, num_src: int, num_edges: int) -> "CSRGraph":
         if self.perm is not None:
diff --git a/pytorch_geometric_b200/nn/conv.py b/pytorch_geometric_b200/nn/conv.py
--- a/pytorch_geometric_b200/nn/conv.py
+++ b/pytorch_geometric_b200/nn/conv.py
@@ -43,7 +43,8 @@
     @staticmethod
     def forward(ctx, x: Tensor, bias: Tensor, graph: CSRGraph):
         ctx.graph = graph
-        return ops.spmm_csr(graph.rowptr, graph.col, graph.val, x, graph.num_dst, "sum", graph.plan, bias=bias)
+        return ops.spmm_csr(graph.rowptr, graph.col, graph.val, x, graph.num_dst, "sum", graph.plan, bias=bias,
+                            row_class=graph.row_class, class_hist=graph.class_hist)
 
     @staticmethod
     def backward(ctx, grad_out: Tensor):
@@ -52,7 +53,8 @@
         gx = gb = None
         if ctx.needs_input_grad[0]:
             graph.build_transpose()
-            gx = ops.spmm_csr(graph.rowptr_t, graph.col_t, graph.val_t, grad_out, graph.num_src, "sum", graph.plan_t)
+            gx = ops.spmm_csr(graph.rowptr_t, graph.col_t, graph.val_t, grad_out, graph.num_src, "sum", graph.plan_t,
+                              row_class=graph.row_class_t, class_hist=graph.class_hist_t)
         if ctx.needs_input_grad[1]:
             gb = ops.column_sum(grad_out)
         return gx, gb, None
@@ -71,7 +73,8 @@
     def forward(ctx, x: Tensor, w_l: Tensor, b_l: Optional[Tensor], w_r: Tensor, graph: CSRGraph, aggr: str, relu: bool,
                 input_is_relu: bool, grad_masked_by_consumer: bool):
         x = x.contiguous()
-        agg = ops.spmm_csr(graph.rowptr, graph.col, graph.val, x, graph.num_dst, aggr, graph.plan)
+        agg = ops.spmm_csr(graph.rowptr, graph.col, graph.val, x, graph.num_dst, aggr, graph.plan,
+                           row_class=graph.row_class, class_hist=graph.class_hist)
         w_hi, w_lo = dense.split_tf32(torch.cat([w_l.detach(), w_r.detach()], dim=1))
         y, _ = dense.gemm_pair(agg, x, w_hi, w_lo, 0, w_l.size(0), bias=None if b_l is None else b_l.detach(), relu=relu)
         ctx.graph, ctx.aggr, ctx.relu, ctx.has_bias = graph, aggr, relu, b_l is not None
@@ -93,7 +96,8 @@
             graph.build_transpose()
             val_t = graph.mean_val_t() if ctx.aggr == "mean" else graph.val_t
             ops.spmm_csr(graph.rowptr_t, graph.col_t, val_t, ga, graph.num_src, "sum", graph.plan_t, out=gx, accumulate=True,
-                         relu_mask=x if ctx.input_is_relu else None)
+                         relu_mask=x if ctx.input_is_relu else None, row_class=graph.row_class_t,
+                         class_hist=graph.class_hist_t)
         if ctx.needs_input_grad[1]:
             gwl = dense._mm_tn(g, agg)
         if ctx.needs_input_grad[3]:
diff --git a/pytorch_geometric_b200/ops.py b/pytorch_geometric_b200/ops.py
--- a/pytorch_geometric_b200/ops.py
+++ b/pytorch_geometric_b200/ops.py
@@ -240,11 +240,54 @@
         return self._partials
 
 
+def slot_class(ptr: Tensor, col: Tensor) -> Tensor:
+    _cuda(ptr, col)
+    cls = torch.empty(col.numel(), dtype=torch.uint8, device=col.device)
+    check(lib().b200mp_slot_class(_p(ptr), _p(col), col.numel(), _p(cls), _same_idx(ptr, col), _stream()), "slot_class")
+    return cls
+
+
+def class_histogram(ptr: Tensor) -> Tuple[int, ...]:
+    _cuda(ptr)
+    hist = torch.empty(64, dtype=torch.int64, device=ptr.device)
+    check(lib().b200mp_class_histogram(_p(ptr), ptr.numel() - 1, _p(hist), _idt(ptr), _stream()), "class_histogram")
+    return tuple(int(v) for v in hist.tolist())
+
+
+L2_HOT_FRACTION = 0.5
+L2_HOT_MIN_CLASS = 6
+
+
+def hot_class_min(hist: Tuple[int, ...], row_bytes: int, l2_bytes: int) -> Optional[int]:
+    budget = L2_HOT_FRACTION * l2_bytes
+    rows, best = 0, None
+    for k in range(len(hist) - 1, L2_HOT_MIN_CLASS - 1, -1):
+        if (rows + hist[k]) * row_bytes > budget:
+            break
+        rows += hist[k]
+        if rows:
+            best = k
+    return best
+
+
+_L2_BYTES: "dict" = {}
+
+
+def _class_min(hist: Optional[Tuple[int, ...]], row_bytes: int, device) -> Optional[int]:
+    if hist is None:
+        return None
+    idx = device.index if device.index is not None else torch.cuda.current_device()
+    if idx not in _L2_BYTES:
+        _L2_BYTES[idx] = torch.cuda.get_device_properties(idx).L2_cache_size
+    return hot_class_min(hist, row_bytes, _L2_BYTES[idx])
+
+
 def spmm_csr(rowptr: Tensor, col: Tensor, val: Optional[Tensor], x: Tensor, n_rows: int, reduce: str = "sum",
              plan: Optional[LongRowPlan] = None, out: Optional[Tensor] = None,
              bias: Optional[Tensor] = None, x_halo: Optional[Tensor] = None, accumulate: bool = False,
-             peer_ptrs: Optional[int] = None, peer_rows: int = 0, relu_mask: Optional[Tensor] = None) -> Tensor:
-    _cuda(rowptr, col, val, x)
+             peer_ptrs: Optional[int] = None, peer_rows: int = 0, relu_mask: Optional[Tensor] = None,
+             row_class: Optional[Tensor] = None, class_hist: Optional[Tuple[int, ...]] = None) -> Tensor:
+    _cuda(rowptr, col, val, x, row_class)
     if x.dim() != 2:
         raise ValueError("spmm_csr expects a 2-D feature matrix")
     x = x.contiguous()
@@ -275,10 +318,31 @@
         if x_halo.dtype != x.dtype or x_halo.dim() != 2 or x_halo.size(1) != F or not x_halo.is_contiguous():
             raise ValueError("x_halo must be a contiguous [n_halo, F] tensor of x's dtype")
         n_local, n_cols = x.size(0), x.size(0) + x_halo.size(0)
-    _timed("spmm_csr", 2 if args[2] else 1, lib().b200mp_spmm_csr, _p(rowptr), _p(col), _p(val), _p(x), _p(out),
-           n_rows, n_cols, F, REDUCE[reduce], *args, _p(bias), _p(x_halo), n_local, int(bool(accumulate)),
-           peer_ptrs, int(peer_rows), _p(relu_mask), it, _vdt(x), _stream())
+    call = (_p(rowptr), _p(col), _p(val), _p(x), _p(out), n_rows, n_cols, F, REDUCE[reduce], *args, _p(bias),
+            _p(x_halo), n_local, int(bool(accumulate)), peer_ptrs, int(peer_rows), _p(relu_mask), it, _vdt(x), _stream())
+    class_min = None
+    if row_class is not None:
+        if row_class.dtype != torch.uint8 or row_class.numel() != col.numel() or not row_class.is_contiguous():
+            raise ValueError("row_class must be a contiguous uint8 tensor with one entry per CSR slot")
+        class_min = _class_min(class_hist, F * x.element_size(), x.device)
+    if class_min is None:
+        _timed("spmm_csr", 2 if args[2] else 1, lib().b200mp_spmm_csr, *call)
+    else:
+        a = SpmmCsrArgs(*call)
+        _timed("spmm_csr", 2 if args[2] else 1, lib().b200mp_spmm_csr_hinted, ctypes.byref(a), _p(row_class), class_min)
     return out
+
+
+class SpmmCsrArgs(ctypes.Structure):
+    _fields_ = [
+        ("rowptr", ctypes.c_void_p), ("col", ctypes.c_void_p), ("val", ctypes.c_void_p), ("x", ctypes.c_void_p),
+        ("out", ctypes.c_void_p), ("n_rows", ctypes.c_int64), ("n_cols", ctypes.c_int64), ("feat", ctypes.c_int64),
+        ("reduce", ctypes.c_int), ("long_rows", ctypes.c_void_p), ("chunk_ptr", ctypes.c_void_p),
+        ("n_long_rows", ctypes.c_int64), ("n_chunks", ctypes.c_int64), ("chunk", ctypes.c_int64),
+        ("partials", ctypes.c_void_p), ("bias", ctypes.c_void_p), ("x_halo", ctypes.c_void_p),
+        ("n_local_cols", ctypes.c_int64), ("flags", ctypes.c_int), ("peer_ptrs", ctypes.c_void_p),
+        ("peer_rows", ctypes.c_int64), ("relu_mask", ctypes.c_void_p), ("idx_dtype", ctypes.c_int),
+        ("val_dtype", ctypes.c_int), ("stream", ctypes.c_void_p)]
 
 
 SEGMENT_PLAN_MIN_ROWS = 1 << 16
```

Measured after the change: 908.0 million, median of 6. 1.02x the previous value.
